# liuQuan98/GCL

Hardware: AMD Instinct MI355X
Metric: active voxels/sec thru ResUNetBN2C fwd+bwd+GCL loss, KITTI 0.3m (higher is better)
Workload: dtype f32; 1 GPU; configs[2]: GCL training step (finest_contrastive_loss), ResUNetBN2C-32 conv1 k=5, KITTI-shaped ray-cast clouds @0.3 m, bs=4 x 7 clouds per GPU, positive groups 'fixed16'; global_batch=4, parallelism=dp1

## Files before the change

### gcl_amd/MinkowskiEngine/native.py

```python
import ctypes
import os
import threading

import torch
from torch.autograd.function import once_differentiable

from .. import _lib

PLAN_ENABLED = os.environ.get("GCL_PLAN", "1") == "1"
AUX_STREAM = {"0": "", "1": "1", "low": "low", "high": "high"}[os.environ.get("GCL_PLAN_AUX", "low")]


def _addr(t):
    return t.data_ptr() if t is not None else 0


_SIDE_STREAMS = {}


def eval_side_stream(device, n_rows=None):
    if os.environ.get("GCL_EVAL_SPLIT_MAPS", "1") == "0":
        return None
    if n_rows is not None and n_rows < int(os.environ.get("GCL_EVAL_SPLIT_MIN_ROWS", "100000")):
        return None
# ... 253 lines not shown
        plan.covers_all_params = claimed == set(range(len(params)))
        return plan

    def _pointers(self):
        key = tuple(p.data_ptr() for p in self.params)
        if key != self._ptr_key:
            if any(p.dtype != torch.float32 or not p.is_contiguous() for p in self.params):
                raise ValueError("plan parameters must be contiguous fp32 tensors")
            self._ptr_key = key
            self._param_ptrs = (ctypes.c_void_p * len(key))(*key)
            bn = []
            for rm, rv in self.bn_buffers:
                bn += [rm.data_ptr(), rv.data_ptr()]
            self._bn_ptrs = (ctypes.c_void_p * max(1, len(bn)))(*bn)
        return self._param_ptrs, self._bn_ptrs

    def run(self, x_feats, maps):
        lib = _lib.require_gpu()
        if maps.keys != self.spec_keys:
            raise ValueError("the maps were built for a different map specification than the plan")
        self._check_input(x_feats, maps)
        x = x_feats.contiguous()
        dev = x.device
        need = lib.gcl_plan_arena_bytes(self.handle, ctypes.byref(maps.desc))
        if need < 0:
            raise RuntimeError("gcl_plan_arena_bytes: " + lib.gcl_last_error().decode())
        arena = torch.empty(int(need), dtype=torch.uint8, device=dev)
        self._ensure_state(lib, dev)
        pp, bp = self._pointers()
        if AUX_STREAM and self._aux is None:
            lo, _hi = torch.cuda.Stream.priority_range()
            pct = int(os.environ.get("GCL_AUX_CU_PCT", "0"))
            if 0 < pct < 100:
                h = ctypes.c_void_p()
                _lib.check(lib.gcl_stream_create_cu_share(pct, 1, ctypes.byref(h)), "gcl_stream_create_cu_share")
                self._aux = torch.cuda.ExternalStream(h.value, device=dev)
            else:
                self._aux = torch.cuda.Stream(device=dev, priority={"low": lo, "high": _hi}.get(AUX_STREAM, 0))
            lib.gcl_plan_set_aux_stream(self.handle, ctypes.c_void_p(self._aux.cuda_stream))
        if self.profile_next:
            lib.gcl_plan_profile(self.handle, 1)
        y_ptr = ctypes.c_void_p()
        held = None
        if self._touched is not None and not (torch.is_grad_enabled() and self.forward_list_ok()):
            held, cap = self._touched, self._touched_cap
            self.set_touched_rows(None, 0)
        try:
            _lib.check(lib.gcl_plan_forward(self.handle, ctypes.byref(maps.desc), _lib.ptr(x, torch.float32), pp, bp,
                                            _lib.ptr(self._state), _lib.ptr(arena), arena.numel(), ctypes.byref(y_ptr),
                                            _lib.stream()), "gcl_plan_forward")
        finally:
            if held is not None:
                self.set_touched_rows(held, cap)
        for m in self.bn_modules:
            m._pending_batches += 1
            m._train_forwards += 1
        n_out = int(maps.desc.n_rows[self.records[-1]["level_out"]])
        off = y_ptr.value - arena.data_ptr()
        y = arena[off:off + n_out * self.out_channels * 4].view(torch.float32).view(n_out, self.out_channels)
        if not torch.is_grad_enabled():
            lib.gcl_plan_release(self.handle, _lib.ptr(arena))
            return y
        run = _PlanRun()
        run.plan, run.arena, run.maps, run.y, run.x = self, arena, maps, y, x
        run.grad_targets, run.done = self.grad_targets, False
        run.touched = None
        if self._touched is not None and lib.gcl_plan_suffix_fwd_rows_used(self.handle) > 0:
            run.touched, self._touched, self._touched_cap = self._touched, None, 0
        run.segments = self._segments()
        if run.grad_targets is not None:
            if self._anchor is None or self._anchor.device != dev:
                self._anchor = torch.zeros(1, device=dev, requires_grad=True)
            return _PlanFn.apply(run, self._anchor)
        return _PlanFn.apply(run, *self.params)

    def _check_input(self, x_feats, maps):
        r0 = self.records[0]
        if x_feats.dim() != 2 or x_feats.shape[1] != r0["cin"]:
            raise ValueError(f"the plan was recorded for {r0['cin']} input channels, got a tensor of shape {tuple(x_feats.shape)}")
        if x_feats.shape[0] != int(maps.desc.n_rows[r0["level_in"]]):
            raise ValueError("features and coordinate maps differ in length")

    def _ensure_state(self, lib, dev):
        if self._state is None or self._state.device != dev:
            self._state = torch.empty(int(lib.gcl_plan_eval_state_bytes(self.handle)), dtype=torch.uint8, device=dev)
            self._eval_key = None

    def prepare_eval(self, dev):
        from . import ops
        lib = _lib.require_gpu()
        self._ensure_state(lib, dev)
        pp, _ = self._pointers()
        aff, ptrs = [], []
        for m in self.bn_modules:
            scale, shift = m.eval_affine()
            rstd = getattr(m, "_eval_rstd", None)
            if rstd is None or rstd[0] is not scale:
                with torch.no_grad():
                    rstd = m._eval_rstd = (scale, torch.rsqrt(m.bn.running_var.detach() + m.bn.eps).contiguous())
            aff.append((scale, shift, rstd[1]))
            ptrs += [scale.data_ptr(), shift.data_ptr(), m.bn.running_mean.data_ptr(), rstd[1].data_ptr()]
        bn = (ctypes.c_void_p * len(ptrs))(*ptrs)
        key = (tuple(p._version for p in self.params), tuple(p.data_ptr() for p in self.params), ops._AMAX_EPOCH)
        return pp, bn, aff, key, dev

    def run_eval(self, x_feats, maps, prepared=None):
        lib = _lib.require_gpu()
        if maps.keys != self.spec_keys:
            raise ValueError("the maps were built for a different map specification than the plan")
        self._check_input(x_feats, maps)
        x = x_feats.contiguous()
        dev = x.device
        if prepared is None or prepared[4] != dev:
            prepared = self.prepare_eval(dev)
        pp, bn, aff, key, _ = prepared
        need = lib.gcl_plan_eval_arena_bytes(self.handle, ctypes.byref(maps.desc))
        if need < 0:
            raise RuntimeError("gcl_plan_eval_arena_bytes: " + lib.gcl_last_error().decode())
        arena = torch.empty(int(need), dtype=torch.uint8, device=dev)
        repack = int(key != self._eval_key)
        y_ptr = ctypes.c_void_p()
        _lib.check(lib.gcl_plan_forward_eval(self.handle, ctypes.byref(maps.desc), _lib.ptr(x, torch.float32), pp, bn, repack,
                                             _lib.ptr(self._state), _lib.ptr(arena), arena.numel(), ctypes.byref(y_ptr),
                                             _lib.stream()), "gcl_plan_forward_eval")
        self._eval_key = key
        n_out = int(maps.desc.n_rows[self.records[-1]["level_out"]])
        off = y_ptr.value - arena.data_ptr()
        return arena[off:off + n_out * self.out_channels * 4].view(torch.float32).view(n_out, self.out_channels)

    def _segments(self):
        n = len(self.records)
        if self.bucket_of_param is None or self.on_bucket is None:
            return [(0, n, [])]
        lowest = {}
        for i, r in enumerate(self.records):
            for k in ("w", "bias", "bn_w", "bn_b"):
                p = r[k]
                if p >= 0 and p in self.bucket_of_param:
                    b = self.bucket_of_param[p]
                    lowest[b] = min(lowest.get(b, i), i)
        cuts = sorted(set(lowest.values()), reverse=True)
        segs, hi = [], n
        for c in cuts:
            segs.append((c, hi, sorted(b for b, i in lowest.items() if i == c)))
            hi = c
        if hi > 0:
            segs.append((0, hi, []))
        return segs

    def forward_list_ok(self):
        n, s = len(self.records), _lib.load().gcl_plan_touched_suffix(self.handle)
        return all(last <= s or (first <= s and last == n) for first, last, _ in self._segments())

    def output_rows(self, maps):
        return int(maps.desc.n_rows[self.records[-1]["level_out"]])

    def set_touched_rows(self, rows, cap):
        lib = _lib.load()
        self._touched = rows
        self._touched_cap = int(cap)
        _lib.check(lib.gcl_plan_set_touched_rows(self.handle, _lib.ptr(rows, torch.int32), int(cap)),
                   "gcl_plan_set_touched_rows")

    def touch_loss_rows(self, index, goff, sel, rows_a, rows_b, n_rows, cap):
        lib = _lib.load()
        dev = index.device
        scratch = torch.empty(int(lib.gcl_touched_rows_scratch_len(int(n_rows))), dtype=torch.int32, device=dev)
        out = torch.empty(int(cap) + 1, dtype=torch.int32, device=dev)
        rows, count = out[:cap], out[cap:]
        _lib.check(lib.gcl_touched_rows(_lib.ptr(index, torch.int64), index.shape[0], _lib.ptr(goff, torch.int64),
                                        goff.shape[0] - 1, _lib.ptr(sel, torch.int64), sel.shape[0],
                                        _lib.ptr(rows_a, torch.int64), rows_a.shape[0], _lib.ptr(rows_b, torch.int64),
                                        rows_b.shape[0], int(n_rows), _lib.ptr(scratch), _lib.ptr(rows), int(cap),
                                        _lib.ptr(count), _lib.stream()), "gcl_touched_rows")
        self.set_touched_rows(rows, cap)
        return rows, count

    def _backward(self, run, dy):
        lib = _lib.load()
        targets = run.grad_targets
        flat = None
        if targets is None:
            sizes = [p.numel() for p in self.params]
            flat = torch.empty(sum(sizes), dtype=torch.float32, device=dy.device)
            targets, off = [], 0
            for p, s in zip(self.params, sizes):
                targets.append(flat[off:off + s].view_as(p))
                off += s
        gp = (ctypes.c_void_p * len(targets))(*[t.data_ptr() for t in targets])
        st = _lib.stream()
        for first, last, buckets in run.segments:
            _lib.check(lib.gcl_plan_backward(self.handle, _lib.ptr(run.arena), _lib.ptr(dy, torch.float32), gp, first,
                                             last, st), "gcl_plan_backward")
            for b in buckets:
                self.on_bucket(b)
        self._touched = run.touched = None
        if self.profile_next:
            self.profile_next = False
            self._profile_pending = True
            lib.gcl_plan_profile(self.handle, 0)
        run.done = True
        run.arena = run.maps = run.y = run.x = None
        return None if flat is None else targets

    def profile_records(self):
        lib = _lib.load()
        buf = (ctypes.c_double * (8 * 1024))()
        n = lib.gcl_plan_profile_read(self.handle, buf, 1024)
        return [tuple(buf[8 * i + j] for j in range(8)) for i in range(max(0, n))]
```

### gcl_amd/_lib.py

```python
import ctypes
import os
import subprocess

import torch

_HERE = os.path.dirname(os.path.abspath(__file__))
CSRC = os.path.join(_HERE, "csrc")
LIB_PATH = os.environ.get("GCL_LIB_PATH", os.path.join(CSRC, "libgcl_hip.so"))
SOURCES = ["coords.hip", "conv.hip", "norm.hip", "loss.hip", "pairloss.hip", "data.hip", "sc2pcr.hip", "plan.hip", "match.hip", "ransac.hip", "regstats.hip", "fpfh.hip",
           "valpose.hip", "pairmatch.hip", "icp.hip", "instnorm.hip"]
HEADER = os.path.join(os.path.dirname(_HERE), "include", "gcl_amd.h")

_vp, _i32, _i64, _f32 = ctypes.c_void_p, ctypes.c_int32, ctypes.c_int64, ctypes.c_float
_f64 = ctypes.c_double

MAX_LEVELS, MAX_MAPS = 8, 16
MAPS_PINNED_BYTES = 512 * (MAX_MAPS + 1)
ERR_ARENA = -4


class MapSpec(ctypes.Structure):
    _fields_ = [("t_in", _i32), ("kernel_size", _i32), ("stride", _i32), ("tables", _i32), ("pairs", _i32)]


class MapDesc(ctypes.Structure):
    _fields_ = [("t_in", _i32), ("kernel_size", _i32), ("stride", _i32), ("K", _i32), ("level_in", _i32),
                ("level_out", _i32), ("n_in", _i64), ("n_out", _i64), ("n_pairs", _i64),
                ("nbr", _vp), ("nbr_t", _vp), ("counts", _vp),
                ("tbl_n", _vp), ("order_n", _vp), ("mask_n", _vp), ("tbl_t", _vp), ("order_t", _vp), ("mask_t", _vp),
                ("pair_in", _vp), ("pair_out", _vp), ("presence", _vp), ("dw_bounds", _vp), ("seg_off", _i64 * 128),
                ("counts_host", _i32 * 128)]


class MapsDesc(ctypes.Structure):
    _fields_ = [("n_levels", _i32), ("n_maps", _i32), ("n_rows", _i64 * MAX_LEVELS), ("coords", _vp * MAX_LEVELS),
                ("table", _vp * MAX_LEVELS), ("cap", _i64 * MAX_LEVELS), ("status", _i32 * 4), ("arena_used", _i64),
                ("ready_event", _vp), ("late_mask", _i32), ("reserved", _i32), ("maps", MapDesc * MAX_MAPS)]


class NnSearch(ctypes.Structure):
    _fields_ = [("a", _vp), ("rows_a", _vp), ("b", _vp), ("rows_b", _vp), ("dmin", _vp), ("argmin", _vp), ("pts_a", _vp),
                ("pts_b", _vp), ("src", _vp), ("tgt", _vp), ("bi_off", _i64), ("part_off", _i64), ("ma", _i32), ("mb", _i32)]


class MutualJob(ctypes.Structure):
    _fields_ = [("nn01", _vp), ("nn10", _vp), ("xyz0", _vp), ("xyz1", _vp), ("T", _vp), ("pairs", _vp), ("src", _vp),
                ("tgt", _vp), ("count", _vp), ("m0", _i32), ("m1", _i32)]


class PlanOp(ctypes.Structure):
    _fields_ = [("kind", _i32), ("x", _i32), ("x2", _i32), ("y", _i32), ("level_in", _i32), ("level_out", _i32),
                ("cin", _i32), ("cout", _i32), ("map", _i32), ("transpose", _i32), ("K", _i32), ("w", _i32),
                ("bias", _i32), ("bn_w", _i32), ("bn_b", _i32), ("bn", _i32), ("relu", _i32), ("momentum", _f32),
                ("eps", _f32)]


OP_CONVBN, OP_CONV, OP_RELU, OP_CAT, OP_ROWNORM = 1, 2, 3, 4, 5

SIGNATURES = {
    "gcl_last_error": (ctypes.c_char_p, []),
    "gcl_version": (_i32, []),
    "gcl_device_count": (_i32, []),
    "gcl_coords_insert": (_i32, [_vp, _i64, _vp, _i64, _vp, _vp]),
    "gcl_scan_scratch_len": (_i64, [_i64]),
    "gcl_stride_map": (_i32, [_vp, _i64, _vp, _i32, _vp, _i64, _vp, _vp, _vp, _vp, _vp]),
    "gcl_exclusive_scan_i32": (_i32, [_vp, _i64, _vp, _vp, _vp]),
    "gcl_voxel_coords": (_i32, [_vp, _i64, _f32, _i32, _vp, _vp]),
    "gcl_unique_coords": (_i32, [_vp, _i64, _vp, _i64, _vp, _vp, _vp, _vp, _vp, _vp]),
    "gcl_colocation_hits": (_i32, [_vp, _vp, _i64, _i32, ctypes.POINTER(ctypes.c_double), _vp, _i64, _f32,
                                    ctypes.c_double, _i32, _vp, _vp, _vp, _vp]),
    "gcl_colocation_emit": (_i32, [_vp, _vp, _vp, _i64, _i32, _i32, _vp, _vp, _vp, _vp, _vp, _vp]),
    "gcl_voxel_coords_multi": (_i32, [_vp, _i64, ctypes.POINTER(_i64), _i32, _f32, _vp, _vp]),
    "gcl_cloud_row_starts": (_i32, [_vp, _i64, _vp, _i32, _vp, _vp]),
    "gcl_loader_points": (_i32, [_vp, _vp, _vp, _i64, _vp, _vp, _vp, _vp, _vp]),
    "gcl_colocation_hits_at": (_i32, [_vp, _vp, _i64, _i64, _i32, _i32, ctypes.POINTER(ctypes.c_double), _vp, _i64, _f32,
                                       ctypes.c_double, _i32, _vp, _vp, _vp, _vp]),
    "gcl_cloud_centroids_scratch_len": (_i64, [_i64, _i32]),
    "gcl_cloud_centroids": (_i32, [_vp, _i64, ctypes.POINTER(_i64), _i32, _vp, _vp, _vp]),
    "gcl_cloud_affines": (_i32, [_vp, _vp, _i32, _vp, _vp]),
    "gcl_voxel_coords_aug": (_i32, [_vp, _i64, ctypes.POINTER(_i64), _i32, _f64, _vp, _vp, _i32, _vp, _vp]),
    "gcl_loader_points_aug": (_i32, [_vp, _vp, _vp, _i64, _vp, _vp, _vp, _vp, _i32, _vp, _vp, _vp]),
    "gcl_host_legacy_choice":(_i32, [_vp, _vp, _i64, _i64, _vp, _vp]),
    "gcl_kernel_map_bitmap_len": (_i64, []),
    "gcl_kernel_map_scratch_len": (_i64, [_i32, _i64]),
    "gcl_kernel_map": (_i32, [_vp, _i64, _vp, _i64, _i32, _i32, _i32, _vp, _vp, _vp, _vp, _i64, _vp, _vp]),
    "gcl_kernel_map_pairs": (_i32, [_vp, _i32, _i64, ctypes.POINTER(_i64), _vp, _vp, _vp, _vp]),
    "gcl_map_launch_shape": (_i32, [_i64, _i32, _i32, ctypes.POINTER(_i32)]),
    "gcl_pack_weights_bytes": (_i64, [_i32, _i32, _i32, _i32]),
    "gcl_amax": (_i32, [_vp, _i64, _vp, _i32, _vp]),
    "gcl_amax_multi": (_i32, [_vp, _vp, _i32, _vp, _vp]),
    "gcl_pack_weights_multi": (_i32, [_vp, _i32, _i64, _i32, _vp, _vp, _vp]),
    "gcl_conv_fwd_nb": (_i32, [_i64, _i32, _i32]),
    "gcl_pack_weights": (_i32, [_vp, _i32, _i32, _i32, _i32, _i32, _vp, _vp, _vp]),
    "gcl_table_sort_scratch_len": (_i64, [_i64]),
    "gcl_table_sort": (_i32, [_vp, _i32, _i64, _vp, _vp, _vp, _vp, _vp]),
    "gcl_table_sort_multi": (_i32, [_vp, _i32, _vp]),
    "gcl_conv_fwd_groups_scratch_len": (_i64, [_i64, _i32, _i32, _i32]),
    "gcl_conv_fwd_launch_shape": (_i32, [_i64, _i32, _i32, _i32, _i32, _i32, _i32, _i32, _i32, _i32, ctypes.POINTER(_i32)]),
    "gcl_conv_fwd_fused": (_i32, [_vp, _i64, _i32, _vp, _i32, _vp, _vp, _vp, _vp, _vp, _i64, _i32, _i32, _i32, _vp, _vp, _vp,
                                  _i32, _vp, _vp, _vp, _i32, _vp]),
    "gcl_conv_fwd_fused_ld": (_i32, [_vp, _i64, _i32, _vp, _i32, _vp, _vp, _vp, _vp, _vp, _i64, _i32, _i32, _i32, _vp, _vp, _vp,
                                     _i32, _i32, _vp, _vp, _vp, _i32, _vp]),
    "gcl_split_planes": (_i32, [_vp, _i64, _i32, _vp, _vp, _vp]),
    "gcl_conv_fwd": (_i32, [_vp, _i64, _i32, _vp, _i32, _vp, _vp, _vp, _vp, _vp, _i64, _i32, _i32, _i32, _vp, _vp, _vp, _i32,
                            _vp]),
    "gcl_conv_bwd_weight_scratch_len": (_i64, [_i32, _i32, _i32, _i64, _i64]),
    "gcl_conv_bwd_weight": (_i32, [_vp, _i64, _vp, _i64, _i32, _i32, _vp, _vp, ctypes.POINTER(_i64), _i32, _i32, _i32, _i32, _vp,
                                   _vp, _vp, _vp, _vp]),
    "gcl_conv_bwd_weight_bounds_len": (_i64, [_i32, _i64]),
    "gcl_conv_bwd_weight_bounds": (_i32, [_vp, ctypes.POINTER(_i64), _i32, _i64, _vp, _vp]),
    "gcl_conv_bwd_weight_rg": (_i32, [_vp, _i64, _vp, _i64, _i32, _i32, _vp, _vp, ctypes.POINTER(_i64), _i32, _i32, _i32, _i32, _vp,
                                      _vp, _vp, _vp, _vp, _vp]),
    "gcl_conv_bwd_weight_launch_shape": (_i32, [_i32, _i32, _i32, _i32, _i32, _i32, _i64, _i64, ctypes.POINTER(_i32)]),
    "gcl_conv_bwd_weight_rows_scratch_len": (_i64, [_i32, _i32, _i32, _i64]),
    "gcl_conv_bwd_weight_rows": (_i32, [_vp, _vp, _i64, _i32, _i32, _i32, _vp, _vp, _vp, _vp, _vp]),
    "gcl_presence_bits": (_i32, [_vp, _i32, _i64, _vp, _vp]),
    "gcl_kernel_map_3_from_5": (_i32, [_vp, _vp, _i64, _vp, _vp, _vp]),
    "gcl_not_ones_rows": (_i32, [_vp, _i32, _vp, _i64, _vp, _i32, _vp, _vp]),
    "gcl_stem_fwd": (_i32, [_vp, _vp, _vp, _i64, _i32, _i32, _i32, _vp, _vp, _vp, _vp]),
    "gcl_stem_bwd_weight_scratch_len": (_i64, [_i32, _i32, _i32, _i64]),
    "gcl_stem_bwd_weight": (_i32, [_vp, _vp, _vp, _i64, _i32, _i32, _i32, _vp, _vp, _vp, _vp, _vp]),
    "gcl_bn_scratch_len": (_i64, [_i64, _i32]),
    "gcl_bn_stats": (_i32, [_vp, _i64, _i32, _f32, _f32, _vp, _vp, _vp, _vp, _vp, _vp]),
    "gcl_bn_tiles_scratch_len": (_i64, [_i64, _i32]),
    "gcl_bn_stats_from_tiles_range": (_i32, [_vp, _i64, _i64, _i32, _f32, _f32, _vp, _vp, _vp, _vp, _vp, _vp, _vp, _i32, _vp, _vp, _vp,
                                             _vp]),
    "gcl_bn_apply_planes": (_i32, [_vp, _i64, _i32, _vp, _vp, _vp, _vp, _vp, _i32, _vp, _i32, _vp, _vp, _vp, _vp]),
    "gcl_bn_bwd_reduce_range": (_i32, [_vp, _vp, _i32, _vp, _vp, _i64, _i32, _vp, _vp, _i32, _vp, _vp, _vp, _vp, _vp, _vp, _vp]),
    "gcl_bn_bwd_apply_planes": (_i32, [_vp, _vp, _i32, _vp, _vp, _i64, _i32, _vp, _vp, _vp, _vp, _vp, _i32, _vp, _vp, _vp, _vp, _vp]),
    "gcl_bn_bwd_reduce_rows": (_i32, [_vp, _vp, _i32, _vp, _vp, _i64, _i32, _vp, _vp, _i32, _vp, _vp, _vp, _vp, _vp, _vp, _vp]),
    "gcl_bn_bwd_apply_rows": (_i32, [_vp, _vp, _i32, _vp, _vp, _i64, _i32, _vp, _vp, _vp, _vp, _vp, _i32, _vp, _vp, _vp, _vp, _vp]),
    "gcl_bn_stats_from_tiles": (_i32, [_vp, _i64, _i64, _i32, _f32, _f32, _vp, _vp, _vp, _vp, _vp, _vp]),
    "gcl_bn_apply": (_i32, [_vp, _i64, _i32, _vp, _vp, _vp, _vp, _vp, _i32, _vp, _vp, _vp, _vp]),
    "gcl_bn_apply_ld": (_i32, [_vp, _i64, _i32, _vp, _vp, _vp, _vp, _vp, _i32, _vp, _i32, _vp, _vp, _vp]),
    "gcl_bn_mask_len": (_i64, [_i64, _i32]),
    "gcl_bn_bwd_reduce": (_i32, [_vp, _vp, _vp, _vp, _i64, _i32, _vp, _vp, _i32, _vp, _vp, _vp, _vp]),
    "gcl_bn_bwd_apply": (_i32, [_vp, _vp, _vp, _vp, _i64, _i32, _vp, _vp, _vp, _vp, _vp, _i32, _vp, _vp, _vp, _vp]),
    "gcl_bn_bwd_reduce_ld": (_i32, [_vp, _vp, _i32, _vp, _vp, _i64, _i32, _vp, _vp, _i32, _vp, _vp, _vp, _vp]),
    "gcl_bn_bwd_apply_ld": (_i32, [_vp, _vp, _i32, _vp, _vp, _i64, _i32, _vp, _vp, _vp, _vp, _vp, _i32, _vp, _vp, _vp, _vp]),
    "gcl_in_scratch_len": (_i64, [_i64, _i32, _i32]),
    "gcl_in_fwd": (_i32, [_vp, _i64, _i32, _vp, _vp, _vp, _i32, _f32, _vp, _vp, _vp, _i32, _vp, _vp, _vp, _vp, _vp, _vp, _vp]),
    "gcl_in_bwd": (_i32, [_vp, _vp, _i64, _i32, _vp, _vp, _vp, _i32, _vp, _vp, _vp, _i32, _vp, _vp, _vp, _vp, _vp, _vp, _vp,
                          _vp]),
    "gcl_row_normalize_fwd": (_i32, [_vp, _i64, _i32, _vp, _vp, _vp]),
    "gcl_row_normalize_bwd": (_i32, [_vp, _vp, _vp, _i64, _i32, _vp, _vp, _vp]),
    "gcl_sgd_multi": (_i32, [_vp, _vp, _i32, _f32, _f32, _f32, _i32, _vp]),
    "gcl_col_sum": (_i32, [_vp, _i64, _i32, _vp, _vp, _vp]),
    "gcl_maps_arena_bytes": (_i64, [_i64, _vp, _i32, _i32]),
    "gcl_maps_build": (_i32, [_vp, _i64, _vp, _i32, _i32, _vp, _i64, _vp, _vp, _vp]),
    "gcl_maps_build_split": (_i32, [_vp, _i64, _vp, _i32, _i32, _vp, _i64, _vp, _vp, _vp, _vp]),
    "gcl_plan_create": (_vp, [_vp, _i32, _i32, _i32, _vp, _i32, _i32]),
    "gcl_plan_destroy": (None, [_vp]),
    "gcl_plan_state_bytes": (_i64, [_vp]),
    "gcl_plan_arena_bytes": (_i64, [_vp, _vp]),
    "gcl_plan_forward": (_i32, [_vp, _vp, _vp, _vp, _vp, _vp, _vp, _i64, _vp, _vp]),
    "gcl_plan_eval_state_bytes": (_i64, [_vp]),
    "gcl_plan_eval_arena_bytes": (_i64, [_vp, _vp]),
    "gcl_plan_forward_eval": (_i32, [_vp, _vp, _vp, _vp, _vp, _i32, _vp, _vp, _i64, _vp, _vp]),
    "gcl_plan_backward": (_i32, [_vp, _vp, _vp, _vp, _i32, _i32, _vp]),
    "gcl_plan_release": (_i32, [_vp, _vp]),
    "gcl_plan_set_aux_stream": (_i32, [_vp, _vp]),
    "gcl_plan_touched_suffix": (_i32, [_vp]),
    "gcl_plan_set_touched_rows": (_i32, [_vp, _vp, _i64]),
    "gcl_plan_suffix_rows_used": (_i64, [_vp]),
    "gcl_plan_suffix_fwd_rows_used": (_i64, [_vp]),
    "gcl_gather_rows": (_i32, [_vp, _i32, _i64, _vp, _i64, _i32, _f32, _vp, _vp]),
    "gcl_scatter_rows": (_i32, [_vp, _vp, _i64, _i32, _i64, _vp, _i32, _vp]),
    "gcl_scatter_add_rows": (_i32, [_vp, _i32, _vp, _i64, _i32, _i64, _vp, _i32, _vp]),
    "gcl_row_slots": (_i32, [_vp, _i64, _i64, _vp, _vp]),
    "gcl_touched_rows_scratch_len": (_i64, [_i64]),
    "gcl_touched_rows": (_i32, [_vp, _i64, _vp, _i64, _vp, _i32, _vp, _i32, _vp, _i32, _i64, _vp, _vp, _i64, _vp, _vp]),
    "gcl_stream_create_cu_share": (_i32, [_i32, _i32, ctypes.POINTER(ctypes.c_void_p)]),
    "gcl_stream_destroy": (_i32, [_vp]),
    "gcl_plan_profile": (_i32, [_vp, _i32]),
    "gcl_plan_profile_read": (_i32, [_vp, _vp, _i32]),
    "gcl_sc2_chunks": (_i32, []),
    "gcl_sc2_refine_partial_len": (_i32, []),
    "gcl_sc2_confidence": (_i32, [_vp, _vp, _i32, _f32, _i32, _vp, _vp, _vp, _vp]),
    "gcl_sc2_confidence_scratch_bytes": (_i64, [_i32]),
    "gcl_sc2_confidence_sparse": (_i32, [_vp, _vp, _i32, _f32, _i32, _vp, _vp, _vp, _vp, _vp]),
    "gcl_sc2_register_scratch_bytes": (_i64, [_i32]),
    "gcl_sc2_register": (_i32, [_vp, _vp, _i32, _f32, _i32, _f32, _i32, _i32, _i32, _f32, _f32, _i32, _vp, _vp, _vp, _vp, _vp,
                                _vp, _vp, _vp, _vp, _vp]),
    "gcl_sc2_register_batch_scratch_bytes": (_i64, [_i32, _i32]),
    "gcl_sc2_register_batch": (_i32, [_vp, _vp, _i32, _i32, _vp, _vp, _f32, _i32, _f32, _i32, _i32, _f32, _f32, _i32, _vp, _vp,
                                      _vp, _vp, _vp, _vp, _vp, _vp, _vp, _vp]),
    "gcl_sc2_local_max": (_i32, [_vp, _vp, _i32, _f32, _vp, _vp]),
    "gcl_sc2_seed_knn": (_i32, [_vp, _vp, _i32, _vp, _i32, _f32, _i32, _vp, _vp, _vp]),
    "gcl_sc2_seed_trans": (_i32, [_vp, _vp, _i32, _vp, _i32, _i32, _i32, _f32, _i32, _f32, _vp, _vp, _vp]),
    "gcl_sc2_refine": (_i32, [_vp, _vp, _i32, _f32, _i32, _vp, _vp, _vp, _vp]),
    "gcl_ransac_scratch_bytes": (_i64, [_i32, _i32]),
    "gcl_ransac_default_chunk": (_i32, []),
    "gcl_ransac_register": (_i32, [_vp, _vp, _i32, _i32, _f32, _f32, _f32, _i32, _f32, ctypes.c_uint64, _i32, _vp, _vp, _vp, _vp,
                                   _vp, _vp, _vp]),
    "gcl_ransac_batch_scratch_bytes": (_i64, [_i32, _i32, _i32]),
    "gcl_ransac_register_batch": (_i32, [_vp, _vp, _i32, _i32, _vp, _i32, _f32, _f32, _f32, _i32, _f32, _vp, _i32, _vp, _vp,
                                         _vp, _vp, _vp, _vp, _vp]),
    "gcl_registration_stats": (_i32, [_vp, _vp, _i32, _i32, _vp, _vp, _vp, _f32, _f32, _f32, _vp, _vp, _vp, _vp]),
    "gcl_group_loss_fwd": (_i32, [_vp, _i32, _vp, _vp, _vp, _vp, _i32, _f32, _f32, _i32, _vp, _vp, _vp, _vp]),
    "gcl_group_loss_bwd": (_i32, [_vp, _i32, _vp, _vp, _vp, _vp, _i32, _f32, _f32, _i32, _vp, _vp, _vp, _vp, _vp]),
    "gcl_circle_group_fwd": (_i32, [_vp, _i32, _vp, _vp, _vp, _vp, _i32, _f32, _f32, _f32, _i32, _vp, _vp, _vp, _vp, _vp]),
    "gcl_circle_group_bwd": (_i32, [_vp, _i32, _vp, _vp, _vp, _vp, _i32, _f32, _f32, _f32, _i32, _vp, _vp, _vp, _vp, _vp,
                                    _vp]),
    "gcl_nn_rowmin_scratch_len": (_i64, [_i32, _i32]),
    "gcl_nn_rowmin": (_i32, [_vp, _vp, _i32, _vp, _vp, _i32, _i32, _i32, _vp, _vp, _vp, _vp]),
    "gcl_nn_rowmin_any_scratch_len": (_i64, [_i32, _i32, _i32]),
    "gcl_nn_rowmin_any": (_i32, [_vp, _vp, _i32, _vp, _vp, _i32, _i32, _i32, _vp, _vp, _vp, _vp]),
    "gcl_nn3_scratch_len": (_i64, [_i32, _i32]),
    "gcl_nn3_rowmin": (_i32, [_vp, _i32, _vp, _i32, _vp, _i32, _vp, _vp, _vp, _vp, _vp]),
    "gcl_nn_rowmin_batch_scratch_len": (_i64, [_vp, _i32, _i32]),
    "gcl_nn_rowmin_batch": (_i32, [_vp, _vp, _i32, _i32, _i32, _vp, _vp]),
    "gcl_mutual_match_batch": (_i32, [_vp, _vp, _i32, _f32, _vp]),
    "gcl_mutual_correspondences_batch": (_i32, [_vp, _vp, _i32, _i32, _vp]),
    "gcl_mutual_match": (_i32, [_vp, _i32, _vp, _i32, _vp, _vp, _vp, _f32, _vp, _vp, _vp]),
    "gcl_mutual_correspondences": (_i32, [_vp, _i32, _vp, _i32, _vp, _vp, _i32, _vp, _vp, _vp, _vp]),
    "gcl_neg_mask": (_i32, [_vp, _vp, _vp, _i32, _vp, _vp, _i64, _i64, _vp, _i64, _vp, _vp]),
    "gcl_neg_loss_fwd": (_i32, [_vp, _vp, _i32, _f32, _vp, _vp]),
    "gcl_neg_loss_bwd": (_i32, [_vp, _i32, _vp, _vp, _vp, _vp, _vp, _i32, _f32, _vp, _vp, _vp, _vp]),
    "gcl_loss_combine": (_i32, [_vp, _vp, _i32, _vp, _f32, _f32, _f32, _vp, _vp]),
    "gcl_loss_seed": (_i32, [_vp, _f32, _f32, _f32, _i32, _vp, _vp, _vp, _vp]),
    "gcl_pair_key_table": (_i32, [_vp, _i64, _i64, _vp, _i64, _vp]),
    "gcl_pair_key_mask": (_i32, [_vp, _i32, _vp, _vp, _i64, _i32, _i64, _vp, _i64, _vp, _vp, _vp]),
    "gcl_triplet_scratch_len": (_i64, [_i32]),
    "gcl_triplet_fwd": (_i32, [_vp, _i64, _vp, _i64, _i32, _vp, _vp, _vp, _vp, _i32, _f32, _vp, _vp, _vp]),
    "gcl_triplet_bwd": (_i32, [_vp, _i64, _vp, _i64, _i32, _vp, _vp, _vp, _vp, _i32, _vp, _vp, _vp, _vp, _vp, _vp]),
    "gcl_pair_terms_scratch_len": (_i64, [_i32]),
    "gcl_pair_terms_fwd": (_i32, [_vp, _i64, _vp, _i64, _i32, _vp, _vp, _i32, _i32, _f32, _f32, _vp, _vp, _vp]),
    "gcl_pair_terms_bwd": (_i32, [_vp, _i64, _vp, _i64, _i32, _vp, _vp, _i32, _i32, _f32, _f32, _vp, _vp, _vp, _vp, _vp,
                                  _vp]),
    "gcl_fpfh_cell_keys": (_i32, [_vp, _i64, _vp, _i32, _f32, _vp, _vp]),
    "gcl_fpfh_neighbours": (_i32, [_vp, _i64, _vp, _i32, _vp, _vp, _f32, _i32, _vp, _vp, _vp]),
    "gcl_fpfh_normals": (_i32, [_vp, _i64, _vp, _vp, _i32, _vp, _vp, _i32, _vp, _vp]),
    "gcl_fpfh_spfh": (_i32, [_vp, _vp, _i64, _vp, _vp, _i32, _vp, _vp]),
    "gcl_fpfh_combine": (_i32, [_vp, _vp, _i64, _vp, _vp, _i32, _i32, _vp, _vp]),
    "gcl_irls_pose_scratch_len": (_i64, [_i64]),
    "gcl_irls_pose_batch": (_i32, [_vp, _vp, _i64, _vp, _i32, _vp, _i32, _f64, _i32, _vp, _vp, _vp, _vp]),
    "gcl_val_stats_batch": (_i32, [_vp, _vp, _i64, _vp, _vp, _i64, _vp, _i32, _vp, _vp, _vp, _f64, _f64, _vp, _vp]),
    "gcl_pair_matches_scratch_len": (_i64, [_i64]),
    "gcl_pair_matches_count": (_i32, [_vp, _i64, _vp, _vp, _i64, _vp, _vp, _i32, _vp, _i64, _i32, _i32, _f32, _vp, _vp, _f64, _i32,
                                       _vp, _vp, _vp, _vp]),
    "gcl_pair_matches_emit": (_i32, [_vp, _i64, _vp, _vp, _i64, _vp, _vp, _i32, _vp, _i64, _i32, _i32, _f32, _vp, _vp, _f64, _i32,
                                      _i32, _vp, _vp, _vp, _i64, _vp]),
    "gcl_icp_scratch_bytes": (_i64, [_i64, _i64, _i32]),
    "gcl_icp_register_batch": (_i32, [_vp, ctypes.POINTER(_i64), _vp, _vp, ctypes.POINTER(_i64), _vp, _i32, _vp, _vp, _f64, _vp,
                                      _i32, _f64, _f64, _vp, _vp, _vp, _vp, _vp, _vp]),
}

PAIR_CHUNK = 128
TRIPLET_OUT = 20
PAIR_SQ, PAIR_SQ_POS, PAIR_NEG, PAIR_DIST = 0, 1, 2, 3
FPFH_MAX_NN, FPFH_MAX_CLOUDS, FPFH_BINS = 128, 32767, 33

_lib = None


TRAINING_STEP_SOURCES = ("coords.hip", "conv.hip", "norm.hip", "plan.hip")


def source_hash():
    import hashlib
    h = hashlib.sha256()
    for path in [os.path.join(CSRC, s) for s in TRAINING_STEP_SOURCES] + [os.path.join(CSRC, "common.h")]:
        with open(path, "rb") as fh:
            h.update(fh.read())
    return h.hexdigest()[:16]


def build(force=False, verbose=False):
    srcs = [os.path.join(CSRC, s) for s in SOURCES]
    hdrs = [os.path.join(CSRC, "common.h"), os.path.join(CSRC, "kabsch.h"), os.path.join(CSRC, "fpgrid.h"), HEADER]
    deps = srcs + hdrs
    if not force and os.path.exists(LIB_PATH) and all(os.path.getmtime(LIB_PATH) >= os.path.getmtime(d) for d in deps):
        return LIB_PATH
    hdr_time = max(os.path.getmtime(h) for h in hdrs)
    objs, jobs = [], []
    for s in srcs:
        o = s[:-4] + ".o"
        objs.append(o)
        if force or not os.path.exists(o) or os.path.getmtime(o) < max(os.path.getmtime(s), hdr_time):
            cmd = ["hipcc", "--offload-arch=gfx950", "-O3", "-std=c++17", "-fPIC", "-c", s, "-o", o]
            if verbose:
                print(" ".join(cmd))
            jobs.append((cmd, subprocess.Popen(cmd)))
    for cmd, p in jobs:
        if p.wait() != 0:
            raise subprocess.CalledProcessError(p.returncode, cmd)
    cmd = ["hipcc", "--offload-arch=gfx950", "-fPIC", "-shared", "-o", LIB_PATH] + objs
    if verbose:
        print(" ".join(cmd))
    subprocess.run(cmd, check=True)
    return LIB_PATH


def load():
    global _lib
    if _lib is not None:
        return _lib
    if not os.path.exists(LIB_PATH):
        raise RuntimeError(
            f"{LIB_PATH} is missing: run `python -c 'import __graft_entry__ as g; g.build()'` "
            "(gcl_amd has no CPU fallback; the HIP library is the only product path)")
    lib = ctypes.CDLL(LIB_PATH)
    for name, (res, args) in SIGNATURES.items():
        fn = getattr(lib, name)
        fn.restype = res
        fn.argtypes = args
    _lib = lib
    return lib


_gpu_ok = False


def require_gpu():
# ... 39 lines not shown
```

### gcl_amd/csrc/norm.hip

```cpp
#include "common.h"

namespace gcl {

static inline int bn_rows_per_wg(long long n, int c) {
  int rows = 1024;
  while (rows > 64 && n / rows < 1024) rows >>= 1;
  (void)c;
  return rows;
}

__device__ __forceinline__ float4 mask_as_y(const unsigned long long* __restrict__ mask, long long e) {
  const unsigned long long* m = mask + (e >> 6) * 4;
  const int b = (int)(e & 63);
  return make_float4((float)((m[0] >> b) & 1), (float)((m[1] >> b) & 1), (float)((m[2] >> b) & 1),
                     (float)((m[3] >> b) & 1));
}

__device__ __forceinline__ void relu_gate(float4& g, const float4& yv) {
  g.x = yv.x > 0.f ? g.x : 0.f; g.y = yv.y > 0.f ? g.y : 0.f;
  g.z = yv.z > 0.f ? g.z : 0.f; g.w = yv.w > 0.f ? g.w : 0.f;
}

__device__ __forceinline__ void bn_reduce_partials(double (&red)[2][256][4], const double (&s0)[4], const double (&s1)[4],
                                                   const float (&gm)[4], int c, bool gmax, double* partial) {
// ... 243 lines not shown
};
__global__ void __launch_bounds__(256) k_bn_stats_direct(const float* __restrict__ partial, int n_part, long long n, int c,
                                                         float eps, float momentum, float* running_mean,
                                                         float* running_var, float* mean, float* rstd, BnRange rg) {
  const int ch = blockIdx.x;
  double s, ss;
  reduce_runs(partial + (long long)ch * n_part, partial + ((long long)c + ch) * n_part, n_part, s, ss);
  float xlo = 0.f, xhi = 0.f;
  if (rg.y_amax)
    reduce_min_max(partial + ((long long)2 * c + ch) * n_part, partial + ((long long)3 * c + ch) * n_part, n_part, xlo, xhi);
  if (threadIdx.x != 0) return;
  double m = s / (double)n;
  double var = ss / (double)n - m * m;
  if (var < 0) var = 0;
  const float mu = (float)m, rs = (float)(1.0 / sqrt(var + (double)eps));
  mean[ch] = mu;
  rstd[ch] = rs;
  if (running_mean) {
    double unb = (n > 1) ? var * (double)n / (double)(n - 1) : var;
    running_mean[ch] = (float)((1.0 - momentum) * running_mean[ch] + momentum * m);
    running_var[ch] = (float)((1.0 - momentum) * running_var[ch] + momentum * unb);
  }
  if (rg.y_amax) {
    if (rg.xrange) {
      rg.xrange[ch] = xlo;
      rg.xrange[c + ch] = xhi;
    }
    const float w = rg.weight[ch], b = rg.bias[ch];
    const float f_lo = (xlo - mu) * rs * w + b, f_hi = (xhi - mu) * rs * w + b;
    float bound = rg.relu ? fmaxf(fmaxf(f_lo, f_hi), 0.f) : fmaxf(fabsf(f_lo), fabsf(f_hi));
    if (rg.add_amax) bound += __int_as_float(amax_slot_bits(rg.add_amax));
    if (rg.max_with) bound = fmaxf(bound, __int_as_float(amax_slot_bits(rg.max_with)));
    amax_slot_publish(rg.y_amax, __float_as_int(bound), (unsigned)ch);
  }
}

struct BnBwdRange {
  const float* xrange;
  const float* mean;
  const float* rstd;
  const float* weight;
  long long n;
  int* dx_amax;
};
__global__ void __launch_bounds__(256) k_bn_bwd_final(const double* __restrict__ partial, int nwg, int c,
                                                      float* sum_g, float* sum_gx, BnBwdRange rg) {
  const int ch = blockIdx.x;
  double s, ss;
  reduce_runs(partial + (long long)ch * nwg, partial + ((long long)c + ch) * nwg, nwg, s, ss);
  double gmax = 0;
  if (rg.dx_amax) {
    __shared__ double gm[256];
    double a = 0;
    const double* p3 = partial + ((long long)2 * c + ch) * nwg;
    for (int w = threadIdx.x; w < nwg; w += 256) a = fmax(a, p3[w]);
    gm[threadIdx.x] = a;
    __syncthreads();
    for (int o = 128; o > 0; o >>= 1) {
      if ((int)threadIdx.x < o) gm[threadIdx.x] = fmax(gm[threadIdx.x], gm[threadIdx.x + o]);
      __syncthreads();
    }
    gmax = gm[0];
  }
  if (threadIdx.x != 0) return;
  sum_g[ch] = (float)s;
  sum_gx[ch] = (float)ss;
  if (rg.dx_amax) {
    const float mu = rg.mean[ch], rs = rg.rstd[ch], inv_n = 1.0f / (float)rg.n;
    const float xh = fmaxf(fabsf(rg.xrange[ch] - mu), fabsf(rg.xrange[c + ch] - mu)) * rs;
    const float bound = fabsf(rg.weight[ch] * rs) * ((float)gmax + fabsf((float)s) * inv_n + xh * fabsf((float)ss) * inv_n);
    amax_slot_publish(rg.dx_amax, __float_as_int(bound * 1.0000153f), (unsigned)ch);
  }
}

__device__ __forceinline__ void publish_amax(float m, int* amax_bits) {
#pragma unroll
  for (int o = 32; o > 0; o >>= 1) m = fmaxf(m, __shfl_xor(m, o));
  __shared__ float wm[4];
  if ((threadIdx.x & 63) == 0) wm[threadIdx.x >> 6] = m;
  __syncthreads();
  if (threadIdx.x == 0) {
    amax_slot_publish(amax_bits, __float_as_int(fmaxf(fmaxf(wm[0], wm[1]), fmaxf(wm[2], wm[3]))), blockIdx.x);
  }
}
__device__ __forceinline__ float amax4(float m, const float4& v) {
  return fmaxf(m, fmaxf(fmaxf(fabsf(v.x), fabsf(v.y)), fmaxf(fabsf(v.z), fabsf(v.w))));
}

struct BnFwdC { float4 mu, rs, wv, bv; };
__device__ __forceinline__ BnFwdC bn_fwd_c(const float* mean, const float* rstd, const float* weight, const float* bias, int cq) {
  BnFwdC k;
  k.mu = reinterpret_cast<const float4*>(mean)[cq]; k.rs = reinterpret_cast<const float4*>(rstd)[cq];
  k.wv = reinterpret_cast<const float4*>(weight)[cq]; k.bv = reinterpret_cast<const float4*>(bias)[cq];
  return k;
}
__device__ __forceinline__ float4 bn_fwd_one(const float4& xv, const float4& rv, bool has_res, int relu, const BnFwdC& k) {
  float4 o;
  o.x = (xv.x - k.mu.x) * k.rs.x * k.wv.x + k.bv.x;
  o.y = (xv.y - k.mu.y) * k.rs.y * k.wv.y + k.bv.y;
  o.z = (xv.z - k.mu.z) * k.rs.z * k.wv.z + k.bv.z;
  o.w = (xv.w - k.mu.w) * k.rs.w * k.wv.w + k.bv.w;
  if (has_res) { o.x += rv.x; o.y += rv.y; o.z += rv.z; o.w += rv.w; }
  if (relu) { o.x = fmaxf(o.x, 0.f); o.y = fmaxf(o.y, 0.f); o.z = fmaxf(o.z, 0.f); o.w = fmaxf(o.w, 0.f); }
  return o;
}
__device__ __forceinline__ void bn_mask_store(unsigned long long* __restrict__ mask, long long e, const float4& o, bool ok) {
  unsigned long long b0 = __ballot(ok && o.x > 0.f), b1 = __ballot(ok && o.y > 0.f), b2 = __ballot(ok && o.z > 0.f),
                     b3 = __ballot(ok && o.w > 0.f);
  if (ok && (threadIdx.x & 63) == 0) {
    unsigned long long* m = mask + (e >> 6) * 4;
    m[0] = b0; m[1] = b1; m[2] = b2; m[3] = b3;
  }
}

template <bool HOIST>
__global__ void __launch_bounds__(256) k_bn_apply(const float* __restrict__ x, long long total4, int c,
                                                  const float* __restrict__ mean, const float* __restrict__ rstd,
                                                  const float* __restrict__ weight, const float* __restrict__ bias,
                                                  const float* __restrict__ residual, int relu,
                                                  float* __restrict__ y, unsigned long long* __restrict__ mask,
                                                  int* amax_bits, int y_ld = 0, unsigned short* __restrict__ planes = nullptr,
                                                  const int* __restrict__ planes_amax = nullptr) {
  const float pscale = planes ? amax_scale(planes_amax) : 1.f;
  const int cq_n = c >> 2;
  const long long S = (long long)gridDim.x * blockDim.x;
  const long long e0 = (long long)blockIdx.x * blockDim.x + threadIdx.x;
  const long long yld4 = (y_ld ? y_ld : c) >> 2;
  const long long rstep = HOIST ? S / cq_n : 0;
  long long row_e = e0 / cq_n;
  const int q0 = (int)(e0 % cq_n);
#define BN_Y(E, ROW) (y_ld ? (HOIST ? reinterpret_cast<float4*>(y)[(ROW)*yld4 + q0]                        \
                                    : reinterpret_cast<float4*>(y)[((E) / cq_n) * yld4 + ((E) % cq_n)])   \
                           : reinterpret_cast<float4*>(y)[E])
  const float4 z4 = make_float4(0, 0, 0, 0);
  float am = 0.f;
  BnFwdC ka, kb;
  if (HOIST) ka = kb = bn_fwd_c(mean, rstd, weight, bias, (int)(e0 % cq_n));
  for (long long e = e0; e - (threadIdx.x & 63) < total4; e += 2 * S) {
    const long long f = e + S;
    const bool oka = e < total4, okb = f < total4;
    if (!HOIST) {
      ka = bn_fwd_c(mean, rstd, weight, bias, (int)((oka ? e : 0) % cq_n));
      kb = bn_fwd_c(mean, rstd, weight, bias, (int)((okb ? f : 0) % cq_n));
    }
    float4 xa = z4, xb = z4, ra = z4, rb = z4;
    if (oka) xa = reinterpret_cast<const float4*>(x)[e];
    if (okb) xb = reinterpret_cast<const float4*>(x)[f];
    if (residual) {
      if (oka) ra = reinterpret_cast<const float4*>(residual)[e];
      if (okb) rb = reinterpret_cast<const float4*>(residual)[f];
    }
    const float4 oa = bn_fwd_one(xa, ra, residual != nullptr, relu, ka);
    const float4 ob = bn_fwd_one(xb, rb, residual != nullptr, relu, kb);
    if (oka) { BN_Y(e, row_e) = oa; am = amax4(am, oa); }
    if (okb) { BN_Y(f, row_e + rstep) = ob; am = amax4(am, ob); }
    if (planes) {
      const long long pld = yld4 * 4;
      if (oka) store_planes4(planes, HOIST ? row_e : e / cq_n, pld, HOIST ? q0 * 4 : (int)(e % cq_n) * 4, oa, pscale);
      if (okb) store_planes4(planes, HOIST ? row_e + rstep : f / cq_n, pld, HOIST ? q0 * 4 : (int)(f % cq_n) * 4, ob, pscale);
    }
    row_e += 2 * rstep;
    if (mask) {
      bn_mask_store(mask, e, oa, oka);
      if (f - (threadIdx.x & 63) < total4) bn_mask_store(mask, f, ob, okb);
    }
  }
#undef BN_Y
  if (amax_bits && !planes) publish_amax(am, amax_bits);
}

struct BnBwdC { float4 mu, rs, wv, sg, sx; };
__device__ __forceinline__ BnBwdC bn_bwd_c(const float* mean, const float* rstd, const float* weight, const float* sum_g,
                                           const float* sum_gx, int cq) {
  BnBwdC k;
  k.mu = reinterpret_cast<const float4*>(mean)[cq]; k.rs = reinterpret_cast<const float4*>(rstd)[cq];
  k.wv = reinterpret_cast<const float4*>(weight)[cq];
  k.sg = reinterpret_cast<const float4*>(sum_g)[cq]; k.sx = reinterpret_cast<const float4*>(sum_gx)[cq];
  return k;
}
__device__ __forceinline__ float4 bn_bwd_one(const float4& xv, const float4& g, float inv_n, const BnBwdC& k) {
  float4 o;
  o.x = k.wv.x * k.rs.x * (g.x - k.sg.x * inv_n - (xv.x - k.mu.x) * k.rs.x * k.sx.x * inv_n);
  o.y = k.wv.y * k.rs.y * (g.y - k.sg.y * inv_n - (xv.y - k.mu.y) * k.rs.y * k.sx.y * inv_n);
  o.z = k.wv.z * k.rs.z * (g.z - k.sg.z * inv_n - (xv.z - k.mu.z) * k.rs.z * k.sx.z * inv_n);
  o.w = k.wv.w * k.rs.w * (g.w - k.sg.w * inv_n - (xv.w - k.mu.w) * k.rs.w * k.sx.w * inv_n);
  return o;
}

template <bool HOIST, bool ROWS>
__global__ void __launch_bounds__(256) k_bn_bwd_apply(const float* __restrict__ x, const float* __restrict__ dy,
                                                      const float* __restrict__ y, long long total4, int c,
                                                      float inv_n, const float* __restrict__ mean,
                                                      const float* __restrict__ rstd,
                                                      const float* __restrict__ weight,
                                                      const float* __restrict__ sum_g,
                                                      const float* __restrict__ sum_gx, int relu,
                                                      const unsigned long long* __restrict__ mask,
                                                      float* __restrict__ dx, float* __restrict__ dres,
                                                      int* amax_bits, int dy_ld = 0,
                                                      unsigned short* __restrict__ planes = nullptr,
                                                      const int* __restrict__ planes_amax = nullptr,
                                                      const int* __restrict__ slots = nullptr) {
  const float pscale = planes ? amax_scale(planes_amax) : 1.f;
  const int cq_n = c >> 2;
  const long long S = (long long)gridDim.x * blockDim.x;
  const long long e0 = (long long)blockIdx.x * blockDim.x + threadIdx.x;
  const long long gld4 = (dy_ld ? dy_ld : c) >> 2;
  const long long rstep = HOIST ? S / cq_n : 0;
  long long row_e = e0 / cq_n;
  const int q0 = (int)(e0 % cq_n);
#define BN_DY(E, ROW) (dy_ld ? (HOIST ? reinterpret_cast<const float4*>(dy)[(ROW)*gld4 + q0]                       \
                                      : reinterpret_cast<const float4*>(dy)[((E) / cq_n) * gld4 + ((E) % cq_n)])  \
                             : reinterpret_cast<const float4*>(dy)[E])
#define BN_SLOT(E, ROW) slots[HOIST ? (ROW) : (E) / cq_n]
#define BN_DY_ROWS(G, E, SLOT) \
  if ((SLOT) >= 0) G = reinterpret_cast<const float4*>(dy)[(SLOT)*gld4 + (HOIST ? q0 : (int)((E) % cq_n))];
#define BN_DRES(E, SLOT, G)                                                                                       \
  if (dres) {                                                                                                     \
    if (!ROWS) reinterpret_cast<float4*>(dres)[E] = G;                                                            \
    else if ((SLOT) >= 0) reinterpret_cast<float4*>(dres)[(SLOT)*cq_n + (HOIST ? q0 : (int)((E) % cq_n))] = G;    \
  }
  const float4 z4 = make_float4(0, 0, 0, 0);
  float am = 0.f;
  BnBwdC ka, kb;
  if (HOIST) ka = kb = bn_bwd_c(mean, rstd, weight, sum_g, sum_gx, (int)(e0 % cq_n));
  for (long long e = e0; e < total4; e += 2 * S) {
    const long long f = e + S;
    const bool okb = f < total4;
    if (!HOIST) {
      ka = bn_bwd_c(mean, rstd, weight, sum_g, sum_gx, (int)(e % cq_n));
      kb = bn_bwd_c(mean, rstd, weight, sum_g, sum_gx, (int)((okb ? f : 0) % cq_n));
    }
    long long sa = -1, sb = -1;
    if (ROWS) {
      sa = BN_SLOT(e, row_e);
      if (okb) sb = BN_SLOT(f, row_e + rstep);
    }
    float4 xa = reinterpret_cast<const float4*>(x)[e], ga = z4;
    if (ROWS) { BN_DY_ROWS(ga, e, sa) } else ga = BN_DY(e, row_e);
    float4 xb = z4, gb = z4, ya = z4, yb = z4;
    if (okb) {
      xb = reinterpret_cast<const float4*>(x)[f];
      if (ROWS) { BN_DY_ROWS(gb, f, sb) } else gb = BN_DY(f, row_e + rstep);
    }
    row_e += 2 * rstep;
    if (relu) {
      ya = mask ? mask_as_y(mask, e) : reinterpret_cast<const float4*>(y)[e];
      if (okb) yb = mask ? mask_as_y(mask, f) : reinterpret_cast<const float4*>(y)[f];
      relu_gate(ga, ya);
      relu_gate(gb, yb);
    }
    const float4 oa = bn_bwd_one(xa, ga, inv_n, ka);
    reinterpret_cast<float4*>(dx)[e] = oa;
    am = amax4(am, oa);
    if (planes) store_planes4(planes, e / cq_n, c, (int)(e % cq_n) * 4, oa, pscale);
    BN_DRES(e, sa, ga)
    if (okb) {
      const float4 ob = bn_bwd_one(xb, gb, inv_n, kb);
      reinterpret_cast<float4*>(dx)[f] = ob;
      am = amax4(am, ob);
      if (planes) store_planes4(planes, f / cq_n, c, (int)(f % cq_n) * 4, ob, pscale);
      BN_DRES(f, sb, gb)
    }
  }
#undef BN_DY
#undef BN_SLOT
#undef BN_DY_ROWS
#undef BN_DRES
  if (amax_bits && !planes) publish_amax(am, amax_bits);
}

template <bool BWD>
__global__ void __launch_bounds__(256) k_row_normalize(const float* __restrict__ a, const float* __restrict__ dy,
                                                       const float* __restrict__ norm_in, long long n, int c,
                                                       float* __restrict__ out, float* __restrict__ norm_out,
                                                       int* out_amax) {
  const int lpr = c >> 2;
  const long long e = (long long)blockIdx.x * blockDim.x + threadIdx.x;
  const long long row = e / lpr;
  const bool ok = row < n;
  float4 v = make_float4(0, 0, 0, 0), g = make_float4(0, 0, 0, 0);
  if (ok) {
    v = reinterpret_cast<const float4*>(a)[e];
    if (BWD) g = reinterpret_cast<const float4*>(dy)[e];
  }
  float s = BWD ? (v.x * g.x + v.y * g.y + v.z * g.z + v.w * g.w) : (v.x * v.x + v.y * v.y + v.z * v.z + v.w * v.w);
  for (int o = 1; o < lpr; o <<= 1) s += __shfl_xor(s, o);
  float m = 0.f;
  if (ok) {
    float4 o4;
    if (!BWD) {
      const float nr = sqrtf(s);
      o4 = make_float4(v.x / nr, v.y / nr, v.z / nr, v.w / nr);
      if ((e % lpr) == 0) norm_out[row] = nr;
    } else {
      const float nr = norm_in[row];
      o4 = make_float4((g.x - v.x * s) / nr, (g.y - v.y * s) / nr, (g.z - v.z * s) / nr, (g.w - v.w * s) / nr);
    }
    reinterpret_cast<float4*>(out)[e] = o4;
    m = amax4(m, o4);
  }
  if (out_amax) publish_amax(m, out_amax);
}

struct SgdPtrs { float* p; const float* g; float* buf; };
__global__ void __launch_bounds__(256) k_sgd_multi(const SgdPtrs* __restrict__ table, const long long* __restrict__ sizes,
                                                   float lr, float momentum, float wd, int first) {
  const SgdPtrs t = table[blockIdx.y];
  const long long n = sizes[blockIdx.y];
  const bool vec = ((((unsigned long long)t.p) | ((unsigned long long)t.g) | ((unsigned long long)t.buf)) & 15ull) == 0;
  const long long n4 = vec ? n / 4 : 0;
  for (long long e = (long long)blockIdx.x * blockDim.x + threadIdx.x; e < n4; e += (long long)gridDim.x * blockDim.x) {
    float4 p = reinterpret_cast<const float4*>(t.p)[e];
    const float4 g = reinterpret_cast<const float4*>(t.g)[e];
    float4 b = make_float4(0, 0, 0, 0);
    if (!first) b = reinterpret_cast<const float4*>(t.buf)[e];
    const float d0 = g.x + wd * p.x, d1 = g.y + wd * p.y, d2 = g.z + wd * p.z, d3 = g.w + wd * p.w;
    b.x = first ? d0 : momentum * b.x + d0;
    b.y = first ? d1 : momentum * b.y + d1;
    b.z = first ? d2 : momentum * b.z + d2;
    b.w = first ? d3 : momentum * b.w + d3;
    reinterpret_cast<float4*>(t.buf)[e] = b;
    p.x -= lr * b.x;
    p.y -= lr * b.y;
    p.z -= lr * b.z;
    p.w -= lr * b.w;
    reinterpret_cast<float4*>(t.p)[e] = p;
  }
  for (long long e = n4 * 4 + (long long)blockIdx.x * blockDim.x + threadIdx.x; e < n; e += (long long)gridDim.x * blockDim.x) {
    const float p = t.p[e];
    const float d = t.g[e] + wd * p;
    const float b = first ? d : momentum * t.buf[e] + d;
    t.buf[e] = b;
    t.p[e] = p - lr * b;
  }
}

static bool bn_c_ok(int c) { return c >= 4 && c % 4 == 0 && (256 % (c / 4)) == 0; }

__global__ void __launch_bounds__(256) k_col_sum_final(const double* __restrict__ partial, int nwg, int c, float* out) {
  const int ch = blockIdx.x;
  double s, ss;
  reduce_runs(partial + (long long)ch * nwg, partial + ((long long)c + ch) * nwg, nwg, s, ss);
  if (threadIdx.x != 0) return;
  out[ch] = (float)s;
}

}

using namespace gcl;

extern "C" {

int64_t gcl_bn_scratch_len(int64_t n, int32_t c) { return cdiv(n, bn_rows_per_wg(n, c)) * 3 * c; }

int gcl_bn_stats(const float* x, int64_t n, int32_t c, float eps, float momentum, float* running_mean,
                 float* running_var, double* scratch, float* mean, float* rstd, void* stream) {
  GCL_CHECK_ARG(x && scratch && mean && rstd, "gcl_bn_stats: null pointer");
  GCL_CHECK_ARG(n > 0 && bn_c_ok(c), "gcl_bn_stats: unsupported shape n=%lld c=%d (c/4 must divide 256)", (long long)n, c);
  hipStream_t st = (hipStream_t)stream;
  const int rows = bn_rows_per_wg(n, c);
  int nwg = (int)cdiv(n, rows);
  hipLaunchKernelGGL(k_bn_reduce<false>, dim3(nwg), dim3(256), 0, st, x, (const float*)nullptr,
                     (const float*)nullptr, (long long)n, c, (const float*)nullptr, (const float*)nullptr, 0,
                     (const unsigned long long*)nullptr, rows, scratch);
  hipLaunchKernelGGL(k_bn_stats_final, dim3((unsigned)c), dim3(256), 0, st, (const double*)scratch, nwg,
                     (long long)n, c, eps, momentum, running_mean, running_var, mean, rstd);
  GCL_CHECK_LAUNCH();
  return GCL_OK;
}

int64_t gcl_bn_tiles_scratch_len(int64_t n_tiles, int32_t c) { (void)n_tiles; return 2 * (int64_t)c; }

int gcl_bn_stats_from_tiles(const float* partial, int64_t n_tiles, int64_t n, int32_t c, float eps, float momentum,
                            float* running_mean, float* running_var, double* scratch, float* mean, float* rstd,
                            void* stream) {
  (void)scratch;
  return gcl_bn_stats_from_tiles_range(partial, n_tiles, n, c, eps, momentum, running_mean, running_var, mean, rstd, nullptr,
                                       nullptr, nullptr, 0, nullptr, nullptr, nullptr, stream);
}

int gcl_bn_stats_from_tiles_range(const float* partial, int64_t n_tiles, int64_t n, int32_t c, float eps, float momentum,
                                  float* running_mean, float* running_var, float* mean, float* rstd, float* xrange,
                                  const float* weight, const float* bias, int32_t relu, const int32_t* add_amax,
                                  const int32_t* max_with, int32_t* y_amax, void* stream) {
  GCL_CHECK_ARG(partial && mean && rstd, "gcl_bn_stats_from_tiles: null pointer");
  GCL_CHECK_ARG(n > 0 && n_tiles > 0 && n_tiles <= BN_DIRECT_MAX && c > 0, "gcl_bn_stats_from_tiles: bad sizes");
  GCL_CHECK_ARG(!y_amax || (weight && bias), "gcl_bn_stats_from_tiles_range: the bound of max|y| needs the BatchNorm's weight and bias");
  const BnRange rg{xrange, weight, bias, relu, (const int*)add_amax, (const int*)max_with, (int*)y_amax};
  hipLaunchKernelGGL(k_bn_stats_direct, dim3((unsigned)c), dim3(256), 0, (hipStream_t)stream, partial, (int)n_tiles,
                     (long long)n, c, eps, momentum, running_mean, running_var, mean, rstd, rg);
  GCL_CHECK_LAUNCH();
  return GCL_OK;
}

int gcl_bn_apply(const float* x, int64_t n, int32_t c, const float* mean, const float* rstd, const float* weight,
                 const float* bias, const float* residual, int32_t relu, float* y, uint64_t* relu_mask,
                 int32_t* y_amax, void* stream) {
  return gcl_bn_apply_ld(x, n, c, mean, rstd, weight, bias, residual, relu, y, 0, relu_mask, y_amax, stream);
}

int gcl_bn_apply_ld(const float* x, int64_t n, int32_t c, const float* mean, const float* rstd, const float* weight,
                    const float* bias, const float* residual, int32_t relu, float* y, int32_t y_ld, uint64_t* relu_mask,
                    int32_t* y_amax, void* stream) {
  return gcl_bn_apply_planes(x, n, c, mean, rstd, weight, bias, residual, relu, y, y_ld, relu_mask, y_amax, nullptr, stream);
}

int gcl_bn_apply_planes(const float* x, int64_t n, int32_t c, const float* mean, const float* rstd, const float* weight,
                        const float* bias, const float* residual, int32_t relu, float* y, int32_t y_ld, uint64_t* relu_mask,
                        int32_t* y_amax, void* planes, void* stream) {
  GCL_CHECK_ARG(x && mean && rstd && weight && bias && y, "gcl_bn_apply: null pointer");
  GCL_CHECK_ARG(n > 0 && c >= 4 && c % 4 == 0, "gcl_bn_apply: unsupported shape");
  GCL_CHECK_ARG(y_ld == 0 || (y_ld >= c && y_ld % 4 == 0), "gcl_bn_apply_ld: y_ld must be 0 or a multiple of 4 >= c");
  GCL_CHECK_ARG(!planes || (y_amax && c % 32 == 0 && (y_ld % 32) == 0),
                "gcl_bn_apply_planes: a plane image needs the slot that holds the bound of max|y| and widths that are multiples of 32");
  long long total4 = n * (c / 4);
  long long g = cdiv(total4, 256);
  if (g > 4096) g = 4096;
  if ((g * 256) % (c / 4) == 0)
    hipLaunchKernelGGL(k_bn_apply<true>, dim3((unsigned)g), dim3(256), 0, (hipStream_t)stream, x, total4, c, mean, rstd,
                       weight, bias, residual, relu, y, (unsigned long long*)(relu ? relu_mask : nullptr), y_amax, y_ld,
                       (unsigned short*)planes, (const int*)y_amax);
  else
    hipLaunchKernelGGL(k_bn_apply<false>, dim3((unsigned)g), dim3(256), 0, (hipStream_t)stream, x, total4, c, mean, rstd,
                       weight, bias, residual, relu, y, (unsigned long long*)(relu ? relu_mask : nullptr), y_amax, y_ld,
                       (unsigned short*)planes, (const int*)y_amax);
  GCL_CHECK_LAUNCH();
  return GCL_OK;
}

int64_t gcl_bn_mask_len(int64_t n, int32_t c) { return cdiv(n * (c / 4), 64) * 4; }

int gcl_bn_bwd_reduce(const float* x, const float* dy, const float* y, const uint64_t* relu_mask, int64_t n,
                      int32_t c, const float* mean, const float* rstd, int32_t relu, double* scratch, float* sum_g,
                      float* sum_gx, void* stream) {
  return gcl_bn_bwd_reduce_ld(x, dy, 0, y, relu_mask, n, c, mean, rstd, relu, scratch, sum_g, sum_gx, stream);
}

int gcl_bn_bwd_reduce_ld(const float* x, const float* dy, int32_t dy_ld, const float* y, const uint64_t* relu_mask, int64_t n,
                         int32_t c, const float* mean, const float* rstd, int32_t relu, double* scratch, float* sum_g,
                         float* sum_gx, void* stream) {
  return gcl_bn_bwd_reduce_range(x, dy, dy_ld, y, relu_mask, n, c, mean, rstd, relu, scratch, sum_g, sum_gx, nullptr, nullptr,
                                 nullptr, stream);
}

int gcl_bn_bwd_reduce_range(const float* x, const float* dy, int32_t dy_ld, const float* y, const uint64_t* relu_mask,
                            int64_t n, int32_t c, const float* mean, const float* rstd, int32_t relu, double* scratch,
                            float* sum_g, float* sum_gx, const float* xrange, const float* weight, int32_t* dx_amax,
                            void* stream) {
  GCL_CHECK_ARG(dy_ld == 0 || (dy_ld >= c && dy_ld % 4 == 0), "gcl_bn_bwd_reduce: dy_ld must be 0 or a multiple of 4 >= c");
  GCL_CHECK_ARG(x && dy && mean && rstd && scratch && sum_g && sum_gx, "gcl_bn_bwd_reduce: null pointer");
  GCL_CHECK_ARG(!relu || y || relu_mask, "gcl_bn_bwd_reduce: y or relu_mask is required when relu is set");
  GCL_CHECK_ARG(n > 0 && bn_c_ok(c), "gcl_bn_bwd_reduce: unsupported shape n=%lld c=%d", (long long)n, c);
  GCL_CHECK_ARG(!dx_amax || (xrange && weight), "gcl_bn_bwd_reduce_range: the bound of max|dx| needs xrange (forward pass) and the weight");
  hipStream_t st = (hipStream_t)stream;
  const int rows = bn_rows_per_wg(n, c);
  int nwg = (int)cdiv(n, rows);
  hipLaunchKernelGGL(k_bn_reduce<true>, dim3(nwg), dim3(256), 0, st, x, dy, y, (long long)n, c, mean, rstd, relu,
                     (const unsigned long long*)relu_mask, rows, scratch, dy_ld, dx_amax ? 1 : 0);
  const BnBwdRange rg{xrange, mean, rstd, weight, (long long)n, (int*)dx_amax};
  hipLaunchKernelGGL(k_bn_bwd_final, dim3((unsigned)c), dim3(256), 0, st, (const double*)scratch, nwg, c,
                     sum_g, sum_gx, rg);
  GCL_CHECK_LAUNCH();
  return GCL_OK;
}

int gcl_bn_bwd_apply(const float* x, const float* dy, const float* y, const uint64_t* relu_mask, int64_t n, int32_t c,
                     const float* mean, const float* rstd, const float* weight, const float* sum_g,
                     const float* sum_gx, int32_t relu, float* dx, float* dres, int32_t* dx_amax, void* stream) {
  return gcl_bn_bwd_apply_ld(x, dy, 0, y, relu_mask, n, c, mean, rstd, weight, sum_g, sum_gx, relu, dx, dres, dx_amax, stream);
}

int gcl_bn_bwd_apply_ld(const float* x, const float* dy, int32_t dy_ld, const float* y, const uint64_t* relu_mask, int64_t n,
                        int32_t c, const float* mean, const float* rstd, const float* weight, const float* sum_g,
                        const float* sum_gx, int32_t relu, float* dx, float* dres, int32_t* dx_amax, void* stream) {
  return gcl_bn_bwd_apply_planes(x, dy, dy_ld, y, relu_mask, n, c, mean, rstd, weight, sum_g, sum_gx, relu, dx, dres, dx_amax,
                                 nullptr, stream);
}

int gcl_bn_bwd_apply_planes(const float* x, const float* dy, int32_t dy_ld, const float* y, const uint64_t* relu_mask, int64_t n,
                            int32_t c, const float* mean, const float* rstd, const float* weight, const float* sum_g,
                            const float* sum_gx, int32_t relu, float* dx, float* dres, int32_t* dx_amax, void* planes,
                            void* stream) {
  GCL_CHECK_ARG(dy_ld == 0 || (dy_ld >= c && dy_ld % 4 == 0), "gcl_bn_bwd_apply: dy_ld must be 0 or a multiple of 4 >= c");
  GCL_CHECK_ARG(x && dy && mean && rstd && weight && sum_g && sum_gx && dx, "gcl_bn_bwd_apply: null pointer");
  GCL_CHECK_ARG(!relu || y || relu_mask, "gcl_bn_bwd_apply: y or relu_mask is required when relu is set");
  GCL_CHECK_ARG(n > 0 && c >= 4 && c % 4 == 0, "gcl_bn_bwd_apply: unsupported shape");
  GCL_CHECK_ARG(!planes || (dx_amax && c % 32 == 0),
                "gcl_bn_bwd_apply_planes: a plane image needs the slot that holds the bound of max|dx| and c a multiple of 32");
  long long total4 = n * (c / 4);
  long long g = cdiv(total4, 256);
  if (g > 4096) g = 4096;
  if ((g * 256) % (c / 4) == 0)
    hipLaunchKernelGGL((k_bn_bwd_apply<true, false>), dim3((unsigned)g), dim3(256), 0, (hipStream_t)stream, x, dy, y, total4, c,
                       1.0f / (float)n, mean, rstd, weight, sum_g, sum_gx, relu, (const unsigned long long*)relu_mask, dx,
                       dres, dx_amax, dy_ld, (unsigned short*)planes, (const int*)dx_amax);
  else
    hipLaunchKernelGGL((k_bn_bwd_apply<false, false>), dim3((unsigned)g), dim3(256), 0, (hipStream_t)stream, x, dy, y, total4, c,
                       1.0f / (float)n, mean, rstd, weight, sum_g, sum_gx, relu, (const unsigned long long*)relu_mask, dx,
                       dres, dx_amax, dy_ld, (unsigned short*)planes, (const int*)dx_amax);
  GCL_CHECK_LAUNCH();
  return GCL_OK;
}

int gcl_bn_bwd_reduce_rows(const float* x, const float* g, int32_t g_ld, const int32_t* slots, const uint64_t* relu_mask,
                           int64_t n, int32_t c, const float* mean, const float* rstd, int32_t relu, double* scratch,
                           float* sum_g, float* sum_gx, const float* xrange, const float* weight, int32_t* dx_amax,
                           void* stream) {
  GCL_CHECK_ARG(g_ld == 0 || (g_ld >= c && g_ld % 4 == 0), "gcl_bn_bwd_reduce_rows: g_ld must be 0 or a multiple of 4 >= c");
  GCL_CHECK_ARG(x && g && slots && mean && rstd && scratch && sum_g && sum_gx, "gcl_bn_bwd_reduce_rows: null pointer");
  GCL_CHECK_ARG(!relu || relu_mask, "gcl_bn_bwd_reduce_rows: relu_mask is required when relu is set");
  GCL_CHECK_ARG(n > 0 && bn_c_ok(c), "gcl_bn_bwd_reduce_rows: unsupported shape n=%lld c=%d", (long long)n, c);
  GCL_CHECK_ARG(!dx_amax || (xrange && weight), "gcl_bn_bwd_reduce_rows: the bound of max|dx| needs xrange (forward pass) and the weight");
  hipStream_t st = (hipStream_t)stream;
  const int per_wg = bn_rows_per_wg(n, c);
  const int nwg = (int)cdiv(n, per_wg);
  hipLaunchKernelGGL(k_bn_reduce_rows, dim3(nwg), dim3(256), 0, st, x, g, (const int*)slots, (long long)n, c, mean, rstd,
                     (const unsigned long long*)(relu ? relu_mask : nullptr), per_wg, scratch, g_ld, dx_amax ? 1 : 0);
  const BnBwdRange rg{xrange, mean, rstd, weight, (long long)n, (int*)dx_amax};
  hipLaunchKernelGGL(k_bn_bwd_final, dim3((unsigned)c), dim3(256), 0, st, (const double*)scratch, nwg, c, sum_g, sum_gx, rg);
  GCL_CHECK_LAUNCH();
  return GCL_OK;
}

int gcl_bn_bwd_apply_rows(const float* x, const float* g, int32_t g_ld, const int32_t* slots, const uint64_t* relu_mask,
                          int64_t n, int32_t c, const float* mean, const float* rstd, const float* weight, const float* sum_g,
                          const float* sum_gx, int32_t relu, float* dx, float* dres, int32_t* dx_amax, void* planes,
                          void* stream) {
  GCL_CHECK_ARG(g_ld == 0 || (g_ld >= c && g_ld % 4 == 0), "gcl_bn_bwd_apply_rows: g_ld must be 0 or a multiple of 4 >= c");
  GCL_CHECK_ARG(x && g && slots && mean && rstd && weight && sum_g && sum_gx && dx, "gcl_bn_bwd_apply_rows: null pointer");
  GCL_CHECK_ARG(!relu || relu_mask, "gcl_bn_bwd_apply_rows: relu_mask is required when relu is set");
  GCL_CHECK_ARG(n > 0 && c >= 4 && c % 4 == 0, "gcl_bn_bwd_apply_rows: unsupported shape");
  GCL_CHECK_ARG(!planes || (dx_amax && c % 32 == 0),
                "gcl_bn_bwd_apply_rows: a plane image needs the slot that holds the bound of max|dx| and c a multiple of 32");
  long long total4 = n * (c / 4);
  long long grid = cdiv(total4, 256);
  if (grid > 4096) grid = 4096;
  if ((grid * 256) % (c / 4) == 0)
    hipLaunchKernelGGL((k_bn_bwd_apply<true, true>), dim3((unsigned)grid), dim3(256), 0, (hipStream_t)stream, x, g,
                       (const float*)nullptr, total4, c, 1.0f / (float)n, mean, rstd, weight, sum_g, sum_gx, relu,
                       (const unsigned long long*)relu_mask, dx, dres, dx_amax, g_ld, (unsigned short*)planes,
                       (const int*)dx_amax, (const int*)slots);
  else
    hipLaunchKernelGGL((k_bn_bwd_apply<false, true>), dim3((unsigned)grid), dim3(256), 0, (hipStream_t)stream, x, g,
                       (const float*)nullptr, total4, c, 1.0f / (float)n, mean, rstd, weight, sum_g, sum_gx, relu,
                       (const unsigned long long*)relu_mask, dx, dres, dx_amax, g_ld, (unsigned short*)planes,
                       (const int*)dx_amax, (const int*)slots);
  GCL_CHECK_LAUNCH();
  return GCL_OK;
}

static bool rownorm_c_ok(int c) { return c >= 4 && c <= 256 && (c & (c - 1)) == 0; }

int gcl_row_normalize_fwd(const float* x, int64_t n, int32_t c, float* y, float* norm, void* stream) {
  GCL_CHECK_ARG(x && y && norm, "gcl_row_normalize_fwd: null pointer");
  GCL_CHECK_ARG(n > 0 && rownorm_c_ok(c), "gcl_row_normalize_fwd: c must be a power of two in [4, 256] (got %d)", c);
  long long total = n * (c / 4);
  hipLaunchKernelGGL(k_row_normalize<false>, dim3((unsigned)cdiv(total, 256)), dim3(256), 0, (hipStream_t)stream, x,
                     (const float*)nullptr, (const float*)nullptr, (long long)n, c, y, norm, (int*)nullptr);
  GCL_CHECK_LAUNCH();
  return GCL_OK;
}

int gcl_row_normalize_bwd(const float* y, const float* dy, const float* norm, int64_t n, int32_t c, float* dx,
                          int32_t* dx_amax, void* stream) {
  GCL_CHECK_ARG(y && dy && norm && dx, "gcl_row_normalize_bwd: null pointer");
  GCL_CHECK_ARG(n > 0 && rownorm_c_ok(c), "gcl_row_normalize_bwd: c must be a power of two in [4, 256] (got %d)", c);
  long long total = n * (c / 4);
  hipLaunchKernelGGL(k_row_normalize<true>, dim3((unsigned)cdiv(total, 256)), dim3(256), 0, (hipStream_t)stream, y, dy,
                     norm, (long long)n, c, dx, (float*)nullptr, dx_amax);
  GCL_CHECK_LAUNCH();
  return GCL_OK;
}

int gcl_col_sum(const float* x, int64_t n, int32_t c, double* scratch, float* out, void* stream) {
  GCL_CHECK_ARG(x && scratch && out, "gcl_col_sum: null pointer");
  GCL_CHECK_ARG(n > 0 && bn_c_ok(c), "gcl_col_sum: unsupported shape n=%lld c=%d (c/4 must divide 256)", (long long)n, c);
  hipStream_t st = (hipStream_t)stream;
  const int rows = bn_rows_per_wg(n, c);
  int nwg = (int)cdiv(n, rows);
  hipLaunchKernelGGL(k_bn_reduce<false>, dim3(nwg), dim3(256), 0, st, x, (const float*)nullptr,
                     (const float*)nullptr, (long long)n, c, (const float*)nullptr, (const float*)nullptr, 0,
                     (const unsigned long long*)nullptr, rows, scratch);
  hipLaunchKernelGGL(k_col_sum_final, dim3((unsigned)c), dim3(256), 0, st, (const double*)scratch, nwg, c, out);
  GCL_CHECK_LAUNCH();
  return GCL_OK;
}

int gcl_sgd_multi(const void* table, const int64_t* sizes, int32_t n_tensors, float lr, float momentum,
                  float weight_decay, int32_t first, void* stream) {
  GCL_CHECK_ARG(table && sizes && n_tensors > 0 && n_tensors <= 65535, "gcl_sgd_multi: bad argument");
  hipLaunchKernelGGL(k_sgd_multi, dim3(128, (unsigned)n_tensors), dim3(256), 0, (hipStream_t)stream,
                     (const SgdPtrs*)table, (const long long*)sizes, lr, momentum, weight_decay, first);
  GCL_CHECK_LAUNCH();
  return GCL_OK;
}

}
```

### gcl_amd/csrc/plan.hip

```cpp
#include "common.h"

#include <string.h>

#include <new>
#include <utility>
#include <vector>

namespace gcl {

__device__ __forceinline__ float amax4p(float m, const float4& v) {
  return fmaxf(m, fmaxf(fmaxf(fabsf(v.x), fabsf(v.y)), fmaxf(fabsf(v.z), fabsf(v.w))));
}
__device__ __forceinline__ void publish_amax_wg(float m, int* slot) {
#pragma unroll
  for (int o = 32; o > 0; o >>= 1) m = fmaxf(m, __shfl_xor(m, o));
  __shared__ float wm[4];
  if ((threadIdx.x & 63) == 0) wm[threadIdx.x >> 6] = m;
  __syncthreads();
  if (threadIdx.x == 0)
    amax_slot_publish(slot, __float_as_int(fmaxf(fmaxf(wm[0], wm[1]), fmaxf(wm[2], wm[3]))), blockIdx.x);
}

__global__ void __launch_bounds__(256) k_relu_fwd(const float4* __restrict__ x, long long n4, float4* __restrict__ y,
                                                  int* amax) {
// ... 283 lines not shown
  for (int s = 0; s < n_specs; ++s) any_pairs = any_pairs || (specs[s].pairs != 0 && specs[s].kernel_size > 1);
  const bool split = (side != nullptr || A.dry) && !any_pairs;
  auto on_side = [&](const gcl_map_spec& sp) { return split && !(sp.t_in == 1 && sp.stride == 1); };
  struct MapLaunch { int s, src5, flags; int32_t *bitmap, *scratch; void* stream; };
  MapLaunch launches[GCL_MAX_MAPS];
  int n_launches = 0;
  const MapShape mshape = map_launch_shape(n, 1, 0);
  const bool prefill = !A.dry && !side && mshape.prefill;
  char* fill_lo = nullptr;
  for (int s = 0; s < n_specs; ++s) {
    const gcl_map_spec& sp = specs[s];
    gcl_map_desc& d = out->maps[s];
    d.t_in = sp.t_in;
    d.kernel_size = sp.kernel_size;
    d.stride = sp.stride;
    d.K = sp.kernel_size * sp.kernel_size * sp.kernel_size;
    d.level_in = level_of(sp.t_in);
    d.level_out = level_of(sp.t_in * sp.stride);
    GCL_CHECK_ARG(d.level_in >= 0 && d.level_out >= 0 && d.level_out < n_levels && (sp.stride == 1 || sp.stride == 2),
                  "gcl_maps_build: map %d (t_in %d, stride %d) is outside the %d levels built", s, sp.t_in, sp.stride, n_levels);
    GCL_CHECK_ARG(sp.kernel_size == 1 || sp.kernel_size == 3 || sp.kernel_size == 5, "gcl_maps_build: kernel size 1, 3 or 5");
    d.n_in = out->n_rows[d.level_in];
    d.n_out = out->n_rows[d.level_out];
    if (sp.kernel_size == 1) {
      GCL_CHECK_ARG(sp.stride == 1, "gcl_maps_build: kernel_size 1 with stride > 1");
      continue;
    }
    const int sd = on_side(sp) ? 1 : 0;
    void* mstream = (sd && side) ? (void*)side : stream;
    if (sd) out->late_mask |= 1 << s;
    d.nbr = A.take_n<int32_t>((long long)d.K * d.n_out);
    if (!fill_lo) fill_lo = (char*)d.nbr;
    const bool same = sp.stride == 1;
    d.nbr_t = same ? nullptr : A.take_n<int32_t>((long long)d.K * d.n_in);
    d.counts = counts_all + 128 * s;
    int src5 = -1;
    for (int q = 0; q < s && same && sp.kernel_size == 3; ++q)
      if (specs[q].t_in == sp.t_in && specs[q].kernel_size == 5 && specs[q].stride == 1 && out->maps[q].nbr) src5 = q;
    if (src5 >= 0) {
      launches[n_launches++] = MapLaunch{s, src5, 0, nullptr, nullptr, mstream};
      continue;
    }
    const bool use_bitmap = A.dry || mshape.use_bitmap;
    const bool bitmap_valid = use_bitmap && bitmap[sd][d.level_in] != nullptr;
    if (use_bitmap && !bitmap_valid) bitmap[sd][d.level_in] = A.take_n<int32_t>(gcl_kernel_map_bitmap_len());
    int32_t* scratch = A.take_n<int32_t>(gcl_kernel_map_scratch_len(sp.kernel_size, d.n_out));
    launches[n_launches++] = MapLaunch{s, -1, (same ? 1 : 0) | (bitmap_valid ? 2 : 0) | 4 | (prefill ? 8 : 0),
                                       use_bitmap ? bitmap[sd][d.level_in] : nullptr, scratch, mstream};
  }
  if (prefill && fill_lo) fill32(fill_lo, (long long)((A.base + A.off) - fill_lo) / 4, 0xFFFFFFFFu, st);
  for (int q = 0; q < n_launches; ++q) {
    const MapLaunch& L = launches[q];
    const gcl_map_spec& sp = specs[L.s];
    gcl_map_desc& d = out->maps[L.s];
    if (L.src5 >= 0)
      PLAN_CALL(gcl_kernel_map_3_from_5(out->maps[L.src5].nbr, out->maps[L.src5].counts, d.n_out, d.nbr, d.counts, L.stream));
    else
      PLAN_CALL(gcl_kernel_map(out->coords[d.level_out], d.n_out, out->table[d.level_in], out->cap[d.level_in],
                               sp.kernel_size, sp.t_in, L.flags, L.bitmap, L.scratch, d.nbr, d.nbr_t, d.n_in, d.counts, L.stream));
    if (!A.dry && any_pairs)
      GCL_CHECK_HIP(hipMemcpyAsync(pinned + 128 * (L.s + 1), d.counts, sizeof(int32_t) * d.K, hipMemcpyDeviceToHost, st));
  }
  gcl_sort_job jobs[2][2 * GCL_MAX_MAPS];
  int n_jobs[2] = {0, 0};
  for (int s = 0; s < n_specs; ++s) {
    const gcl_map_spec& sp = specs[s];
    gcl_map_desc& d = out->maps[s];
    if (sp.kernel_size == 1) continue;
    for (int tr = 0; tr < 2; ++tr) {
      if (!(sp.tables & (1 << tr))) continue;
      const int32_t* tbl = tr ? d.nbr_t : d.nbr;
      GCL_CHECK_ARG(tbl, "gcl_maps_build: map %d has no transposed table (stride 1)", s);
      const long long rows = tr ? d.n_in : d.n_out;
      GCL_CHECK_ARG(d.K == 27, "gcl_maps_build: sorted tables are built for 3^3 kernels");
      int32_t* scratch = A.take_n<int32_t>(gcl_table_sort_scratch_len(rows));
      int32_t* order = A.take_n<int32_t>(rows);
      int32_t* sorted = A.take_n<int32_t>((long long)d.K * rows);
      int32_t* mask = A.take_n<int32_t>(cdiv(rows, 32));
      const int sd = on_side(sp) ? 1 : 0;
      jobs[sd][n_jobs[sd]++] = gcl_sort_job{tbl, d.K, rows, scratch, order, sorted, mask, d.counts};
      if (tr) { d.tbl_t = sorted; d.order_t = order; d.mask_t = mask; }
      else { d.tbl_n = sorted; d.order_n = order; d.mask_n = mask; }
    }
  }
  for (int s = 0; s < n_specs; ++s) {
    if (!(specs[s].tables & 4) || specs[s].kernel_size == 1) continue;
    gcl_map_desc& d = out->maps[s];
    d.presence = A.take_n<uint32_t>(d.n_out * ((d.K + 31) / 32));
    PLAN_CALL(gcl_presence_bits(d.nbr, d.K, d.n_out, d.presence, (on_side(specs[s]) && side) ? (void*)side : stream));
  }
  for (int sd = 0; sd < 2; ++sd) {
    void* sstream = (sd && side) ? (void*)side : stream;
    if (n_jobs[sd]) PLAN_CALL(gcl_table_sort_multi(jobs[sd], n_jobs[sd], sstream));
  }
  if (!side) out->late_mask = 0;
  if (!A.dry && any_pairs) GCL_CHECK_HIP(hipStreamSynchronize(st));
  for (int s = 0; s < n_specs; ++s) {
    const gcl_map_spec& sp = specs[s];
    gcl_map_desc& d = out->maps[s];
    if (sp.kernel_size == 1) {
      if (!sp.pairs) continue;
      const long long total = cdiv(d.n_in, GCL_PAIR_CHUNK) * GCL_PAIR_CHUNK;
      d.pair_in = d.pair_out = A.take_n<int32_t>(total);
      d.seg_off[0] = 0;
      d.seg_off[1] = total;
      d.n_pairs = d.n_in;
      d.counts_host[0] = (int32_t)d.n_in;
      if (!A.dry) {
        hipLaunchKernelGGL(k_identity_pairs, dim3((unsigned)cdiv(total, 256)), dim3(256), 0, st, d.pair_in, (long long)d.n_in,
                           total);
        GCL_CHECK_LAUNCH();
      }
      continue;
    }
    if (!any_pairs && !A.dry) continue;
    long long total = 0;
    d.seg_off[0] = 0;
    for (int k = 0; k < d.K; ++k) {
      const long long c = A.dry ? d.n_out : (long long)pinned[128 * (s + 1) + k];
      d.counts_host[k] = (int32_t)c;
      d.n_pairs += c;
      total += cdiv(c, GCL_PAIR_CHUNK) * GCL_PAIR_CHUNK;
      d.seg_off[k + 1] = total;
    }
    if (!sp.pairs) continue;
    const long long len = total > 0 ? total : 1;
    int32_t* both = A.take_n<int32_t>(2 * len);
    d.pair_in = both;
    d.pair_out = both + len;
    int32_t* scratch = A.take_n<int32_t>((long long)d.K * cdiv(d.n_out, 1024) + d.K + 1);
    PLAN_CALL(gcl_kernel_map_pairs(d.nbr, d.K, d.n_out, d.seg_off, scratch, d.pair_in, d.pair_out, stream));
    const long long nb = !A.dry ? gcl_conv_bwd_weight_bounds_len(d.K, d.n_out)
                                : (d.n_out >= 32768 && d.K > 1 && d.K <= 27 ? (long long)d.K * (cdiv(d.n_out, 512) + 1) : 0);
    if (nb > 0 && total > 0) {
      d.dw_bounds = A.take_n<int32_t>(nb);
      PLAN_CALL(gcl_conv_bwd_weight_bounds(d.pair_out, d.seg_off, d.K, d.n_out, d.dw_bounds, stream));
    }
  }
  out->arena_used = A.off;
  if (!A.fits()) {
    set_error("gcl_maps_build: arena too small (%lld bytes needed, %lld given)", A.off, A.size);
    return GCL_ERR_ARENA;
  }
  return GCL_OK;
}

struct RowView;
struct TState {
  float* ptr = nullptr;
  RowView* rv = nullptr;
  int32_t* amax = nullptr;
  void* planes = nullptr;
  int ld = 0;
};

struct OpSaved {
  float* conv_out = nullptr;
  unsigned long long* mask = nullptr;
  float *mean = nullptr, *rstd = nullptr;
  float* xrange = nullptr;
  int32_t* x_amax = nullptr;
  float* norm = nullptr;
};

struct ProfRec {
  hipEvent_t e0, e1;
  double kind, pairs, cin, cout, n_in, n_out, K;
};

struct PassState {
  const gcl_maps_desc* maps = nullptr;
  gcl_maps_desc maps_copy;
  std::vector<TState> t, g;
  std::vector<OpSaved> saved;
  std::vector<void*> params;
  Arena A{DRY_BASE, 0, 0, true};
  int32_t* slot_pool = nullptr;
  long long n_slots = 0, next_slot = 0;
  bool slots_exhausted = false;
  int32_t* w_amax = nullptr;
  unsigned char *pack_fwd = nullptr, *pack_bwd = nullptr;
  void* state = nullptr;
  bool forward_done = false, bwd_packed = false;
  std::vector<char> relu_masked;
  hipEvent_t fwd_packs = nullptr;
  bool fwd_packs_pending = false;
  int32_t* not_ones = nullptr;
  void* key = nullptr;
  const int32_t* fwd_rows = nullptr;
  long long fwd_cap = 0;
};

struct Plan : PassState {
  std::vector<PassState*> passes;
  std::vector<gcl_plan_op> ops;
  int n_tensors = 0, n_params = 0, n_bn = 0, presplit = 128;
  std::vector<int> worder;
  std::vector<int> widx;
  std::vector<int> wmode;
  std::vector<long long> wK, wcin, wcout, off_fwd, off_bwd;
  long long bytes_fwd = 0, bytes_bwd = 0, wgs_fwd = 0, wgs_bwd = 0;
  int n_bwd = 0;
  std::vector<char> made;
  std::vector<char> fuse_relu;
  std::vector<int> cat_left;
  std::vector<int> mask_from;
  std::vector<long long> host_tables, uploaded;
  bool eval = false;
  void* const* bn_eval = nullptr;
  bool eval_repack = true;
  hipStream_t aux = nullptr;
  std::vector<hipEvent_t> events;
  size_t events_used = 0;
  bool aux_dirty = false;
  int suffix_first = 0;
  bool suffix_rows_ok = false;
  const int32_t* touched = nullptr;
  long long touched_cap = 0;
  long long suffix_rows_used = 0;
  long long suffix_fwd_rows_used = 0;
  bool profile = false;
  std::vector<ProfRec> prof;
  size_t prof_used = 0;
};

static long long state_words(const Plan& P) { return (long long)P.worder.size() * (2 + 8 + 8); }

static int32_t* new_slot(Plan& P) {
  if (P.next_slot >= P.n_slots) {
    P.slots_exhausted = true;
    return P.slot_pool;
  }
  return P.slot_pool + (P.next_slot++) * GCL_AMAX_WORDS;
}

static int ensure_amax(Plan& P, TState& ts, long long numel, hipStream_t st) {
  Arena& A = P.A;
  if (ts.amax) return GCL_OK;
  ts.amax = new_slot(P);
  PLAN_CALL(gcl_amax(ts.ptr, numel, ts.amax, 1, (void*)st));
  return GCL_OK;
}

static int ensure_planes(Plan& P, TState& ts, long long n, int c, hipStream_t st) {
  Arena& A = P.A;
  if (ts.planes) return GCL_OK;
  ts.planes = A.take(n * c * 4);
  PLAN_CALL(gcl_split_planes(ts.ptr, n, c, ts.amax, ts.planes, (void*)st));
  return GCL_OK;
}

static hipStream_t fork_aux(Plan& P, hipStream_t st) {
  if (!P.aux || P.A.dry) return st;
  if (P.events_used == P.events.size()) {
    hipEvent_t e;
    if (hipEventCreateWithFlags(&e, hipEventDisableTiming) != hipSuccess) return st;
    P.events.push_back(e);
  }
  hipEvent_t e = P.events[P.events_used++];
  if (hipEventRecord(e, st) != hipSuccess || hipStreamWaitEvent(P.aux, e, 0) != hipSuccess) return st;
  P.aux_dirty = true;
  return P.aux;
}

static int join_aux(Plan& P, hipStream_t st) {
  if (!P.aux || !P.aux_dirty || P.A.dry) return GCL_OK;
  if (P.events_used == P.events.size()) {
    hipEvent_t e;
    GCL_CHECK_HIP(hipEventCreateWithFlags(&e, hipEventDisableTiming));
    P.events.push_back(e);
  }
  hipEvent_t e = P.events[P.events_used++];
  GCL_CHECK_HIP(hipEventRecord(e, P.aux));
  GCL_CHECK_HIP(hipStreamWaitEvent(st, e, 0));
  P.aux_dirty = false;
  return GCL_OK;
}

struct ProfScope {
  Plan& P;
  hipStream_t st;
  ProfRec* r = nullptr;
  ProfScope(Plan& P_, hipStream_t st_, int kind, double pairs, int cin, int cout, long long n_in, long long n_out, int K)
      : P(P_), st(st_) {
    if (!P.profile || P.A.dry) return;
    if (P.prof_used == P.prof.size()) {
      ProfRec nr{};
      if (hipEventCreate(&nr.e0) != hipSuccess || hipEventCreate(&nr.e1) != hipSuccess) return;
      P.prof.push_back(nr);
    }
    r = &P.prof[P.prof_used++];
    r->kind = kind; r->pairs = pairs; r->cin = cin; r->cout = cout; r->n_in = (double)n_in; r->n_out = (double)n_out; r->K = K;
    (void)hipEventRecord(r->e0, st);
  }
  ~ProfScope() { if (r) (void)hipEventRecord(r->e1, st); }
};

static bool is_stem(const gcl_plan_op& op, const gcl_map_desc& m) {
  return op.cin <= 4 && (op.cout % 32) == 0 && !op.transpose && m.kernel_size > 1 && op.bias < 0;
}

static int stem_flag(Plan& P, const gcl_plan_op& op, const gcl_map_desc& m, const TState& x, long long n_in, hipStream_t st) {
  Arena& A = P.A;
  if (!m.presence || P.not_ones) return GCL_OK;
  constexpr int CLOUD_FLAGS = 4096;
  int32_t* cloud = A.take_n<int32_t>(CLOUD_FLAGS);
  P.not_ones = A.take_n<int32_t>(n_in);
  PLAN_CALL(gcl_not_ones_rows(x.ptr, op.cin, P.maps->coords[op.level_in], n_in, cloud, CLOUD_FLAGS, P.not_ones, (void*)st));
  return GCL_OK;
}

struct SortedTable {
  const int32_t *tbl = nullptr, *order = nullptr, *mask = nullptr;
};
static SortedTable sorted_table(const gcl_map_desc& m, bool transposed) {
  if (m.kernel_size == 1) return SortedTable();
  return transposed ? SortedTable{m.tbl_t, m.order_t, m.mask_t} : SortedTable{m.tbl_n, m.order_n, m.mask_n};
}

static int conv_forward(Plan& P, int i, float** y_out, float** stats_out, hipStream_t st, int32_t** relu_amax_out,
                        long long rows = 0) {
  Arena& A = P.A;
  const gcl_plan_op& op = P.ops[i];
  const gcl_maps_desc& M = *P.maps;
  const gcl_map_desc& m = M.maps[op.map];
  const long long n_in = rows > 0 ? rows : M.n_rows[op.level_in], n_out = rows > 0 ? rows : M.n_rows[op.level_out];
  TState& x = P.t[op.x];
  float* y = A.take_n<float>(n_out * op.cout);
  *y_out = y;
  *stats_out = nullptr;
  *relu_amax_out = nullptr;
  const float* W = (const float*)P.params[op.w];
  if (is_stem(op, m)) {
    int rcs = stem_flag(P, op, m, x, n_in, st);
    if (rcs) return rcs;
    PLAN_CALL(gcl_stem_fwd(x.ptr, W, m.nbr, n_out, op.K, op.cin, op.cout, y, m.presence, m.presence ? P.not_ones : nullptr,
                           (void*)st));
    return GCL_OK;
  }
  const int wi = P.widx[op.w];
  if (P.fwd_packs_pending && !A.dry) {
    GCL_CHECK_HIP(hipStreamWaitEvent(st, P.fwd_packs, 0));
    P.fwd_packs_pending = false;
  }
  int rc = ensure_amax(P, x, n_in * op.cin, st);
  if (rc) return rc;
  P.saved[i].x_amax = x.amax;
  const bool pl = op.cin >= P.presplit;
  if (pl && (rc = ensure_planes(P, x, n_in, op.cin, st))) return rc;
  float* stats = nullptr;
  if (op.kind == GCL_OP_CONVBN) stats = A.take_n<float>(cdiv(n_out, 128) * 4 * op.cout);
  *stats_out = stats;
  const SortedTable T = sorted_table(m, op.transpose);
  GCL_CHECK_ARG(A.dry || m.kernel_size == 1 || T.tbl, "gcl_plan_forward: record %d needs a sorted table the maps do not carry", i);
  const float* bias = op.bias >= 0 ? (const float*)P.params[op.bias] : nullptr;
  ProfScope ps(P, st, 0, (double)(m.kernel_size > 1 ? m.n_pairs : n_out), op.cin, op.cout, n_in, n_out, op.K);
  int32_t* relu_amax = (op.kind == GCL_OP_CONV && P.fuse_relu[i]) ? new_slot(P) : nullptr;
  *relu_amax_out = relu_amax;
  PLAN_CALL(gcl_conv_fwd_fused(pl ? (const float*)x.planes : x.ptr, n_in, pl ? 1 : 0, P.pack_fwd + P.off_fwd[wi], 4, x.amax,
                               P.w_amax + (long long)wi * GCL_AMAX_WORDS, T.tbl, T.order, T.mask, n_out, op.K, op.cin, op.cout,
                               bias, nullptr, nullptr, relu_amax ? 1 : 0, relu_amax, y, stats, 0, (void*)st));
  return GCL_OK;
}

static int upload_tables(Plan& P, hipStream_t st) {
  const size_t n = P.worder.size();
  std::vector<long long>& h = P.host_tables;
  h.assign((size_t)state_words(P), 0);
  long long wg = 0;
  for (size_t q = 0; q < n; ++q) {
    h[q] = (long long)(uintptr_t)P.params[P.worder[q]];
    h[n + q] = P.wK[q] * P.wcin[q] * P.wcout[q];
    long long* d = &h[2 * n + 8 * q];
    d[0] = h[q]; d[1] = P.wK[q]; d[2] = P.wcin[q]; d[3] = P.wcout[q]; d[4] = 0; d[5] = (long long)q; d[6] = P.off_fwd[q]; d[7] = wg;
    wg += cdiv(h[n + q], 256);
  }
  P.wgs_fwd = wg;
  wg = 0;
  size_t row = 0;
  for (size_t q = 0; q < n; ++q) {
    if (!P.wmode[q]) continue;
    long long* d = &h[2 * n + 8 * n + 8 * row++];
    d[0] = h[q]; d[1] = P.wK[q]; d[2] = P.wcin[q]; d[3] = P.wcout[q]; d[4] = P.wmode[q]; d[5] = (long long)q; d[6] = P.off_bwd[q]; d[7] = wg;
    wg += cdiv(h[n + q], 256);
  }
  P.wgs_bwd = wg;
  if (h != P.uploaded) {
    GCL_CHECK_HIP(hipMemcpyAsync(P.state, h.data(), h.size() * sizeof(long long), hipMemcpyHostToDevice, st));
    GCL_CHECK_HIP(hipStreamSynchronize(st));
    P.uploaded = h;
  }
  return GCL_OK;
}

static int spread_rows(Plan& P, float* src, float* norm, const int32_t* rows, long long cap, int c, long long n, float** out,
                       hipStream_t st) {
  Arena& A = P.A;
  float* dst = A.take_n<float>(n * c);
  *out = dst;
  if (A.dry) return GCL_OK;
  GCL_CHECK_HIP(hipMemsetAsync(dst, 0, (size_t)(n * c) * sizeof(float), st));
  if (!norm) return gcl_scatter_rows(src, rows, cap, c, n, dst, c, (void*)st);
  hipLaunchKernelGGL(k_scatter_rows_inert, dim3(grid_for(cap * c / 4)), dim3(256), 0, st, (float4*)src, norm, (const int*)rows,
                     cap, c / 4, n, dst, c);
  GCL_CHECK_LAUNCH();
  return GCL_OK;
}

static int plan_forward(Plan& P, const float* x_in, void* const* bn_stats, float** y_out, hipStream_t st) {
  Arena& A = P.A;
  const gcl_maps_desc& M = *P.maps;
  const size_t nw = P.worder.size();
  P.t.assign(P.n_tensors, TState());
  P.g.assign(P.n_tensors, TState());
  P.saved.assign(P.ops.size(), OpSaved());
  if (P.profile && !A.dry) P.prof_used = 0;
  if (!A.dry) P.events_used = 0;
  P.n_slots = 4 * (long long)P.n_tensors + 2 * (long long)P.ops.size() + 16;
  P.next_slot = 0;
  P.slots_exhausted = false;
  P.not_ones = nullptr;
  P.fwd_packs_pending = false;
  P.slot_pool = A.take_n<int32_t>(P.n_slots * GCL_AMAX_WORDS);
  if (!A.dry) GCL_CHECK_HIP(hipMemsetAsync(P.slot_pool, 0, (size_t)P.n_slots * GCL_AMAX_WORDS * sizeof(int32_t), st));
  if (P.eval) {
    char* base = (char*)P.state + ((state_words(P) * 8 + 255) & ~255ll);
    P.w_amax = (int32_t*)base;
    P.pack_fwd = (unsigned char*)(base + (((long long)nw * GCL_AMAX_WORDS * 4 + 255) & ~255ll));
  } else {
    P.w_amax = A.take_n<int32_t>((long long)nw * GCL_AMAX_WORDS);
    P.pack_fwd = (unsigned char*)A.take(P.bytes_fwd);
  }
  P.bwd_packed = false;
  if (nw && !A.dry) {
    int rc = upload_tables(P, st);
    if (rc) return rc;
    if (!P.eval || P.eval_repack) {
      const long long* tab = (const long long*)P.state;
      hipStream_t ps = st;
      if (!P.eval && P.aux && P.n_bwd) ps = fork_aux(P, st);
      PLAN_CALL(gcl_amax_multi((const float* const*)tab, (const int64_t*)(tab + nw), (int32_t)nw, P.w_amax, (void*)ps));
      PLAN_CALL(gcl_pack_weights_multi((const int64_t*)(tab + 2 * nw), (int32_t)nw, P.wgs_fwd, 4, P.w_amax, P.pack_fwd, (void*)ps));
      if (ps != st) {
        if (P.events_used == P.events.size()) {
          hipEvent_t e;
          GCL_CHECK_HIP(hipEventCreateWithFlags(&e, hipEventDisableTiming));
          P.events.push_back(e);
        }
        P.fwd_packs = P.events[P.events_used++];
        GCL_CHECK_HIP(hipEventRecord(P.fwd_packs, ps));
        P.fwd_packs_pending = true;
      }
    }
  }
  if (!P.eval && P.aux && P.n_bwd) {
    P.pack_bwd = (unsigned char*)A.take(P.bytes_bwd);
    if (!A.dry) {
      hipStream_t ws = fork_aux(P, st);
      const long long* tab = (const long long*)P.state;
      PLAN_CALL(gcl_pack_weights_multi((const int64_t*)(tab + 2 * nw + 8 * nw), P.n_bwd, P.wgs_bwd, 4, P.w_amax, P.pack_bwd,
                                       (void*)ws));
    }
    P.bwd_packed = true;
  }
  P.t[0].ptr = (float*)x_in;
  bool late_pending = !A.dry && M.ready_event && M.late_mask;
  for (size_t i = 0; i < P.ops.size(); ++i) {
    const gcl_plan_op& op = P.ops[i];
    const bool compact = P.fwd_cap > 0 && (int)i >= P.suffix_first;
    const long long n_out = compact ? P.fwd_cap : M.n_rows[op.level_out];
    if (compact && (int)i == P.suffix_first) {
      TState& xs = P.t[op.x];
      float* cx = A.take_n<float>(P.fwd_cap * op.cin);
      PLAN_CALL(gcl_gather_rows(xs.ptr, xs.ld ? xs.ld : op.cin, M.n_rows[op.level_in], P.fwd_rows, P.fwd_cap, op.cin, 0.f, cx,
                                (void*)st));
      int32_t* slot = xs.amax;
      xs = TState();
      xs.ptr = cx;
      xs.amax = slot;
    }
    if (late_pending && (op.kind == GCL_OP_CONVBN || op.kind == GCL_OP_CONV) && ((M.late_mask >> op.map) & 1)) {
      GCL_CHECK_HIP(hipStreamWaitEvent(st, (hipEvent_t)M.ready_event, 0));
      late_pending = false;
    }
    TState& y = P.t[op.y];
    int rc;
    switch (op.kind) {
      case GCL_OP_CONVBN: {
        if (P.eval) {
          const gcl_map_desc& m = M.maps[op.map];
          const long long n_in = M.n_rows[op.level_in];
          TState& x = P.t[op.x];
          const int c = op.cout;
          const float* res = op.x2 >= 0 ? P.t[op.x2].ptr : nullptr;
          y.ptr = A.take_n<float>(n_out * c);
          y.amax = new_slot(P);
          void* const* be = P.bn_eval ? P.bn_eval + 4 * op.bn : nullptr;
          if (is_stem(op, m)) {
            float* cy = A.take_n<float>(n_out * c);
            unsigned long long* mask = op.relu ? A.take_n<unsigned long long>(gcl_bn_mask_len(n_out, c)) : nullptr;
            if ((rc = stem_flag(P, op, m, x, n_in, st))) return rc;
            PLAN_CALL(gcl_stem_fwd(x.ptr, (const float*)P.params[op.w], m.nbr, n_out, op.K, op.cin, c, cy, m.presence,
                                   m.presence ? P.not_ones : nullptr, (void*)st));
            PLAN_CALL(gcl_bn_apply(cy, n_out, c, (const float*)be[2], (const float*)be[3], (const float*)P.params[op.bn_w],
                                   (const float*)P.params[op.bn_b], res, op.relu, y.ptr, (uint64_t*)mask, y.amax, (void*)st));
            break;
          }
          const int wi = P.widx[op.w];
          if ((rc = ensure_amax(P, x, n_in * op.cin, st))) return rc;
          const SortedTable T = sorted_table(m, op.transpose);
          GCL_CHECK_ARG(A.dry || m.kernel_size == 1 || T.tbl,
                        "gcl_plan_forward_eval: record %d needs a sorted table the maps do not carry", (int)i);
          const long long gs_len = T.tbl ? gcl_conv_fwd_groups_scratch_len(n_out, op.K, op.cin, c) : 0;
          float* gscratch = gs_len > 0 ? A.take_n<float>(gs_len) : nullptr;
          ProfScope ps(P, st, 0, (double)(m.kernel_size > 1 ? m.n_pairs : n_out), op.cin, c, n_in, n_out, op.K);
          PLAN_CALL(gcl_conv_fwd_fused(x.ptr, n_in, 0, P.pack_fwd + P.off_fwd[wi], 4, x.amax,
                                       P.w_amax + (long long)wi * GCL_AMAX_WORDS, T.tbl, T.order, T.mask, n_out, op.K, op.cin, c,
                                       (const float*)be[1], (const float*)be[0], res, op.relu, y.amax, y.ptr, gscratch,
                                       GCL_CONV_TALL, (void*)st));
          break;
        }
        float *cy, *stats;
        int32_t* unused_slot;
        if ((rc = conv_forward(P, (int)i, &cy, &stats, st, &unused_slot))) return rc;
        OpSaved& sv = P.saved[i];
        sv.conv_out = cy;
        const int c = op.cout;
        float* mr = A.take_n<float>(2 * c);
        sv.mean = mr;
        sv.rstd = mr + c;
        float* rm = (float*)bn_stats[2 * op.bn];
        float* rv = (float*)bn_stats[2 * op.bn + 1];
        const int32_t* res_amax = op.x2 >= 0 ? P.t[op.x2].amax : nullptr;
        const int32_t* cat_amax = P.cat_left[i] >= 0 ? P.t[P.ops[P.cat_left[i]].x2].amax : nullptr;
        const bool bound = stats && c >= P.presplit && (c % 32) == 0 && (op.x2 < 0 || res_amax) &&
                           (P.cat_left[i] < 0 || (cat_amax && (P.ops[P.cat_left[i]].cout % 32) == 0));
        int32_t* bound_slot = bound ? new_slot(P) : nullptr;
        if (stats) {
          const long long nt = cdiv(n_out, 128);
          if (bound) sv.xrange = A.take_n<float>(2 * c);
          PLAN_CALL(gcl_bn_stats_from_tiles_range(stats, nt, n_out, c, op.eps, op.momentum, rm, rv, sv.mean, sv.rstd, sv.xrange,
                                                  (const float*)P.params[op.bn_w], (const float*)P.params[op.bn_b], op.relu,
                                                  res_amax, cat_amax, bound_slot, (void*)st));
        } else {
          double* scratch = A.take_n<double>(gcl_bn_scratch_len(n_out, c));
          PLAN_CALL(gcl_bn_stats(cy, n_out, c, op.eps, op.momentum, rm, rv, scratch, sv.mean, sv.rstd, (void*)st));
        }
        if (P.cat_left[i] >= 0) {
          const gcl_plan_op& cat = P.ops[P.cat_left[i]];
          TState& cty = P.t[cat.y];
          cty = TState();
          cty.ptr = A.take_n<float>(n_out * cat.cout);
          cty.amax = bound ? bound_slot : new_slot(P);
          if (bound) cty.planes = A.take(n_out * cat.cout * 4);
          y.ptr = cty.ptr;
          y.ld = cat.cout;
          y.amax = cty.amax;
          y.planes = nullptr;
        } else {
          y.ptr = A.take_n<float>(n_out * c);
          y.ld = 0;
          y.amax = bound ? bound_slot : new_slot(P);
          if (bound) y.planes = A.take(n_out * c * 4);
        }
        if (op.relu) sv.mask = A.take_n<unsigned long long>(gcl_bn_mask_len(n_out, c));
        const float* res = op.x2 >= 0 ? P.t[op.x2].ptr : nullptr;
        void* img = !bound ? nullptr : (P.cat_left[i] >= 0 ? P.t[P.ops[P.cat_left[i]].y].planes : y.planes);
        PLAN_CALL(gcl_bn_apply_planes(cy, n_out, c, sv.mean, sv.rstd, (const float*)P.params[op.bn_w],
                                      (const float*)P.params[op.bn_b], res, op.relu, y.ptr, y.ld, (uint64_t*)sv.mask, y.amax,
                                      img, (void*)st));
        break;
      }
      case GCL_OP_CONV: {
        float *cy, *stats;
        int32_t* relu_amax;
        if ((rc = conv_forward(P, (int)i, &cy, &stats, st, &relu_amax, compact ? P.fwd_cap : 0))) return rc;
        y.ptr = cy;
        if (relu_amax) {
          y.amax = relu_amax;
          P.t[P.ops[i + 1].y] = y;
        }
        break;
      }
      case GCL_OP_RELU: {
        if (i > 0 && P.fuse_relu[i - 1]) {
          if (compact) y = P.t[op.x];
          break;
        }
        const long long n4 = n_out * op.cout / 4;
        y.ptr = A.take_n<float>(n_out * op.cout);
        y.amax = new_slot(P);
        if (!A.dry) {
          hipLaunchKernelGGL(k_relu_fwd, dim3(grid_for(n4)), dim3(256), 0, st, (const float4*)P.t[op.x].ptr, n4, (float4*)y.ptr,
                             y.amax);
          GCL_CHECK_LAUNCH();
        }
        break;
      }
      case GCL_OP_CAT: {
        const int ca = op.cin, cb = op.cout - op.cin;
        if (P.t[op.x].ld == op.cout && P.t[op.x].ptr == y.ptr && y.ptr) {
          if (!A.dry) {
            hipLaunchKernelGGL(k_cat_right, dim3(grid_for(n_out * cb / 4)), dim3(256), 0, st, (const float4*)P.t[op.x2].ptr,
                               cb / 4, n_out, ca / 4, (float4*)y.ptr, y.amax, (unsigned short*)y.planes);
            GCL_CHECK_LAUNCH();
          }
          break;
        }
        y.ptr = A.take_n<float>(n_out * op.cout);
        y.amax = new_slot(P);
        const int32_t *sa = P.t[op.x].amax, *sb = P.t[op.x2].amax;
        if (!A.dry) {
          const bool both = sa && sb;
          hipLaunchKernelGGL(k_cat2, dim3(grid_for(n_out * op.cout / 4)), dim3(256), 0, st, (const float4*)P.t[op.x].ptr, ca / 4,
                             (const float4*)P.t[op.x2].ptr, cb / 4, n_out, (float4*)y.ptr, y.amax, both ? (const int*)sa : nullptr,
                             both ? (const int*)sb : nullptr);
          GCL_CHECK_LAUNCH();
        }
        break;
      }
      case GCL_OP_ROWNORM: {
        y.ptr = A.take_n<float>(n_out * op.cout);
        P.saved[i].norm = A.take_n<float>(n_out);
        PLAN_CALL(gcl_row_normalize_fwd(P.t[op.x].ptr, n_out, op.cout, y.ptr, P.saved[i].norm, (void*)st));
        break;
      }
      default:
        set_error("gcl_plan_forward: unknown record kind %d", op.kind);
        return GCL_ERR_ARG;
    }
  }
  if (late_pending) GCL_CHECK_HIP(hipStreamWaitEvent(st, (hipEvent_t)M.ready_event, 0));
  *y_out = P.t[P.ops.back().y].ptr;
  if (P.fwd_cap > 0) {
    const gcl_plan_op& last = P.ops.back();
    return spread_rows(P, *y_out, last.kind == GCL_OP_ROWNORM ? P.saved[P.ops.size() - 1].norm : nullptr, P.fwd_rows, P.fwd_cap,
                       last.cout, M.n_rows[last.level_out], y_out, st);
  }
  return GCL_OK;
}

struct RowView {
  const int32_t* rows = nullptr;
  long long cap = 0, n = 0;
  bool parked = false;
  std::vector<std::pair<const float*, float*>> gathered;
  int32_t* slots = nullptr;
  long long n_rows(const gcl_maps_desc& M, int level) const { return cap > 0 ? cap : M.n_rows[level]; }
};

static int contiguous(Plan& P, TState& g, long long rows, int c, hipStream_t st);

static int densify(Plan& P, TState& g, int c, hipStream_t st) {
  if (!g.rv || !g.ptr) return GCL_OK;
  const RowView& V = *g.rv;
  int rc;
  if ((rc = contiguous(P, g, V.cap, c, st))) return rc;
  float* dense;
  if ((rc = spread_rows(P, g.ptr, nullptr, V.rows, V.cap, c, V.n, &dense, st))) return rc;
  g = TState();
  g.ptr = dense;
  return GCL_OK;
}

static int give(Plan& P, int tensor, float* gptr, long long numel, hipStream_t st, int32_t* amax = nullptr, int ld = 0,
                int c = 0, RowView* rv = nullptr) {
  Arena& A = P.A;
  if (tensor < 0 || !P.made[tensor] || !gptr) return GCL_OK;
  TState& g = P.g[tensor];
  if (!g.ptr) {
    g = TState();
    g.ptr = gptr;
    g.ld = ld;
    g.rv = rv;
    g.amax = amax;
    return GCL_OK;
  }
  if (g.rv || rv) {
    GCL_CHECK_ARG(c > 0 && c % 4 == 0, "gcl_plan_backward: a compact gradient needs its channel count");
    TState in;
    in.ptr = gptr;
    in.ld = ld;
    in.rv = rv;
    numel = (g.rv ? g.rv : rv)->n * c;
    int rc;
    if ((rc = densify(P, g, c, st)) || (rc = densify(P, in, c, st))) return rc;
    gptr = in.ptr;
    ld = in.ld;
  }
  float* sum = A.take_n<float>(numel);
  if (!A.dry) {
    if (g.ld || ld) {
      GCL_CHECK_ARG(c > 0 && c % 4 == 0, "gcl_plan_backward: a sliced gradient needs its channel count");
      hipLaunchKernelGGL(k_add2_ld, dim3(grid_for(numel / 4)), dim3(256), 0, st, (const float*)g.ptr, g.ld ? g.ld : c,
                         (const float*)gptr, ld ? ld : c, numel / c, c / 4, (float4*)sum);
    } else {
      hipLaunchKernelGGL(k_add2, dim3(grid_for(numel / 4)), dim3(256), 0, st, (const float4*)g.ptr, (const float4*)gptr,
                         numel / 4, (float4*)sum);
    }
    GCL_CHECK_LAUNCH();
  }
  g = TState();
  g.ptr = sum;
  return GCL_OK;
}

static int contiguous(Plan& P, TState& g, long long rows, int c, hipStream_t st) {
  if (!g.ld || !g.ptr) return GCL_OK;
  Arena& A = P.A;
  float* out = A.take_n<float>(rows * c);
  if (!A.dry) {
    hipLaunchKernelGGL(k_add2_ld, dim3(grid_for(rows * c / 4)), dim3(256), 0, st, (const float*)g.ptr, g.ld, (const float*)nullptr,
                       0, rows, c / 4, (float4*)out);
    GCL_CHECK_LAUNCH();
  }
  g = TState();
  g.ptr = out;
  return GCL_OK;
}

static int saved_rows(Plan& P, RowView& V, const float* src, int ld, int c, float pad, hipStream_t st, const float** out) {
  Arena& A = P.A;
  *out = src;
  if (V.cap <= 0 || V.parked) return GCL_OK;
  for (auto& e : V.gathered)
    if (e.first == src) {
      *out = e.second;
      return GCL_OK;
    }
  float* rows = A.take_n<float>(V.cap * c);
  PLAN_CALL(gcl_gather_rows(src, ld, V.n, V.rows, V.cap, c, pad, rows, (void*)st));
  V.gathered.push_back({src, rows});
  *out = rows;
  return GCL_OK;
}
static int saved_rows(Plan& P, RowView& V, const TState& t, int c, hipStream_t st, const float** out) {
  return saved_rows(P, V, t.ptr, t.ld ? t.ld : c, c, 0.f, st, out);
}

static int row_slots(Plan& P, RowView& V, hipStream_t st) {
  Arena& A = P.A;
  if (V.slots) return GCL_OK;
  V.slots = A.take_n<int32_t>(V.n);
  PLAN_CALL(gcl_row_slots(V.rows, V.cap, V.n, V.slots, (void*)st));
  return GCL_OK;
}

static int conv_backward(Plan& P, int i, TState dy, RowView& V, void* const* grads, hipStream_t st) {
  Arena& A = P.A;
  const gcl_plan_op& op = P.ops[i];
  const gcl_maps_desc& M = *P.maps;
  const gcl_map_desc& m = M.maps[op.map];
  const long long n_in = V.n_rows(M, op.level_in), n_out = V.n_rows(M, op.level_out);
  TState& x = P.t[op.x];
  float* dW = (float*)grads[op.w];
  int rc;
  if (is_stem(op, m)) {
    float* scratch = A.take_n<float>(gcl_stem_bwd_weight_scratch_len(op.K, op.cin, op.cout, n_out));
    hipStream_t ws = fork_aux(P, st);
    ProfScope ps(P, ws, 2, (double)m.n_pairs, op.cin, op.cout, n_in, n_out, op.K);
    PLAN_CALL(gcl_stem_bwd_weight(x.ptr, dy.ptr, m.nbr, n_out, op.K, op.cin, op.cout, scratch, dW, m.presence,
                                  m.presence ? P.not_ones : nullptr, (void*)ws));
    return GCL_OK;
  }
  const int wi = P.widx[op.w];
  if ((rc = ensure_amax(P, dy, n_out * op.cout, st))) return rc;
  const int32_t* w_amax = P.w_amax + (long long)wi * GCL_AMAX_WORDS;
  const double pairs = (double)(m.kernel_size > 1 ? m.n_pairs : n_out);
  const long long rows_len = m.kernel_size == 1 ? gcl_conv_bwd_weight_rows_scratch_len(op.cin, op.cout, 4, n_in) : 0;
  const bool pl_w = rows_len <= 0 && op.cin >= P.presplit && op.cout >= P.presplit;
  const bool pl_x = op.cout >= P.presplit;
  if ((pl_w || (pl_x && P.made[op.x])) && (rc = ensure_planes(P, dy, n_out, op.cout, st))) return rc;
  if (pl_w) {
    x.amax = P.saved[i].x_amax;
    if ((rc = ensure_planes(P, x, n_in, op.cin, st))) return rc;
  }
  const float* xr;
  if ((rc = saved_rows(P, V, x, op.cin, st, &xr))) return rc;
  hipStream_t ws = fork_aux(P, st);
  if (P.made[op.x]) {
    const int mode = (m.kernel_size > 1 && !op.transpose && m.stride == 1) ? 2 : 1;
    const SortedTable T = sorted_table(m, !op.transpose && m.stride != 1);
    const int32_t *tbl = T.tbl, *order = T.order, *mask = T.mask;
    GCL_CHECK_ARG(mode == P.wmode[wi], "gcl_plan_backward: record %d: input-gradient pack mode mismatch", i);
    GCL_CHECK_ARG(A.dry || m.kernel_size == 1 || tbl, "gcl_plan_backward: record %d needs a sorted table the maps do not carry", i);
    const bool pl = pl_x;
    float* acc = P.g[op.x].ptr;
    const int acc_ld = P.g[op.x].ld;
    const RowView* acc_rows = P.g[op.x].rv;
    GCL_CHECK_ARG(!acc_rows || (V.cap <= 0 && acc_rows->n == n_in && op.cin % 4 == 0),
                  "gcl_plan_backward: record %d: a compact gradient waits at an input of another shape", i);
    float* dx = A.take_n<float>(n_in * op.cin);
    int32_t* dx_amax = nullptr;
    {
      ProfScope ps(P, st, acc && !acc_rows ? 1 : 0, pairs, op.cout, op.cin, n_out, n_in, op.K);
      if (acc && !acc_rows)
        PLAN_CALL(gcl_conv_fwd_fused_ld(pl ? (const float*)dy.planes : dy.ptr, n_out, pl ? 1 : 0, P.pack_bwd + P.off_bwd[wi], 4,
                                        dy.amax, w_amax, tbl, order, mask, n_in, op.K, op.cout, op.cin, nullptr, nullptr, acc,
                                        acc_ld, 0, nullptr, dx, nullptr, 0, (void*)st));
      else if (!acc && P.mask_from[i] >= 0) {
        dx_amax = new_slot(P);
        PLAN_CALL(gcl_conv_fwd_fused(pl ? (const float*)dy.planes : dy.ptr, n_out, pl ? 1 : 0, P.pack_bwd + P.off_bwd[wi], 4,
                                     dy.amax, w_amax, tbl, order, mask, n_in, op.K, op.cout, op.cin, nullptr, nullptr, xr, 2,
                                     dx_amax, dx, nullptr, 0, (void*)st));
        if (P.relu_masked.size() != P.ops.size()) P.relu_masked.assign(P.ops.size(), 0);
        P.relu_masked[P.mask_from[i]] = 1;
      } else
        PLAN_CALL(gcl_conv_fwd(pl ? (const float*)dy.planes : dy.ptr, n_out, pl ? 1 : 0, P.pack_bwd + P.off_bwd[wi], 4, dy.amax,
                               w_amax, tbl, order, mask, n_in, op.K, op.cout, op.cin, nullptr, dx, nullptr, 0, (void*)st));
    }
    if (acc_rows)
      PLAN_CALL(gcl_scatter_add_rows(acc, acc_ld ? acc_ld : op.cin, acc_rows->rows, acc_rows->cap, op.cin, n_in, dx, op.cin,
                                     (void*)st));
    P.g[op.x] = TState();
    P.g[op.x].ptr = dx;
    P.g[op.x].amax = dx_amax;
  }
  if (rows_len > 0) {
    float* scratch = A.take_n<float>(rows_len);
    ProfScope ps(P, ws, 3, pairs, op.cin, op.cout, n_in, n_out, op.K);
    PLAN_CALL(gcl_conv_bwd_weight_rows(xr, dy.ptr, n_in, op.cin, op.cout, 4, P.saved[i].x_amax, dy.amax, scratch, dW,
                                       (void*)ws));
  } else {
    GCL_CHECK_ARG(V.cap <= 0, "gcl_plan_backward: record %d: the pair-list weight gradient does not run on a row list", i);
    const int32_t *pa = m.pair_in, *pb = m.pair_out;
    if (op.transpose) { pa = m.pair_out; pb = m.pair_in; }
    GCL_CHECK_ARG(A.dry || (pa && pb), "gcl_plan_backward: record %d needs pair lists the maps do not carry", i);
    const int sorted_side = m.kernel_size == 1 ? 0 : (op.transpose ? 1 : 2);
    const long long n_sorted = sorted_side == 1 ? n_in : (sorted_side == 2 ? n_out : 0);
    float* scratch = A.take_n<float>(gcl_conv_bwd_weight_scratch_len(op.K, op.cin, op.cout, m.seg_off[op.K], n_sorted));
    const bool pl = pl_w;
    ProfScope ps(P, ws, 2, pairs, op.cin, op.cout, n_in, n_out, op.K);
    const int32_t* rgb = (sorted_side != 0 && n_sorted == m.n_out) ? m.dw_bounds : nullptr;
    PLAN_CALL(gcl_conv_bwd_weight_rg(pl ? (const float*)x.planes : x.ptr, n_in, pl ? (const float*)dy.planes : dy.ptr, n_out,
                                     pl ? 1 : 0, sorted_side, pa, pb, m.seg_off, op.K, op.cin, op.cout, 4, P.saved[i].x_amax,
                                     dy.amax, scratch, dW, rgb, (void*)ws));
  }
  if (op.bias >= 0) {
    double* scratch = A.take_n<double>(gcl_bn_scratch_len(n_out, op.cout));
    PLAN_CALL(gcl_col_sum(dy.ptr, n_out, op.cout, scratch, (float*)grads[op.bias], (void*)ws));
  }
  return GCL_OK;
}

static int backward_record(Plan& P, int i, RowView& V, void* const* grads, hipStream_t st) {
  Arena& A = P.A;
  const gcl_maps_desc& M = *P.maps;
  const gcl_plan_op& op = P.ops[i];
  const long long n_out = V.n_rows(M, op.level_out), n_in = V.n_rows(M, op.level_in);
  TState g = P.g[op.y];
  P.g[op.y] = TState();
  if (!g.ptr) return GCL_OK;
  int rc;
  const bool rows_ok = g.rv && V.cap <= 0 && g.rv->n == n_out &&
                       (op.kind == GCL_OP_CAT || (op.kind == GCL_OP_CONVBN && (!op.relu || P.saved[i].mask)));
  if (g.rv && !rows_ok && (rc = densify(P, g, op.cout, st))) return rc;
  RowView* const rv = g.rv;
  switch (op.kind) {
    case GCL_OP_CONVBN: {
      const OpSaved& sv = P.saved[i];
      const int c = op.cout;
      float* sum_g = (float*)grads[op.bn_b];
      float* sum_gx = (float*)grads[op.bn_w];
      double* scratch = A.take_n<double>(gcl_bn_scratch_len(n_out, c));
      const bool bound = sv.xrange && c >= P.presplit && !is_stem(op, M.maps[op.map]);
      TState d;
      d.ptr = A.take_n<float>(n_out * c);
      d.amax = new_slot(P);
      if (rv) {
        if ((rc = row_slots(P, *rv, st))) return rc;
        PLAN_CALL(gcl_bn_bwd_reduce_rows(sv.conv_out, g.ptr, g.ld, rv->slots, (const uint64_t*)sv.mask, n_out, c, sv.mean, sv.rstd,
                                         op.relu, scratch, sum_g, sum_gx, sv.xrange, (const float*)P.params[op.bn_w],
                                         bound ? d.amax : nullptr, (void*)st));
      } else {
        PLAN_CALL(gcl_bn_bwd_reduce_range(sv.conv_out, g.ptr, g.ld, nullptr, (const uint64_t*)sv.mask, n_out, c, sv.mean, sv.rstd,
                                          op.relu, scratch, sum_g, sum_gx, sv.xrange, (const float*)P.params[op.bn_w],
                                          bound ? d.amax : nullptr, (void*)st));
      }
      if (bound) d.planes = A.take(n_out * c * 4);
      const long long res_rows = rv ? rv->cap : n_out;
      float* dres = op.x2 >= 0 ? A.take_n<float>(res_rows * c) : nullptr;
      if (rv)
        PLAN_CALL(gcl_bn_bwd_apply_rows(sv.conv_out, g.ptr, g.ld, rv->slots, (const uint64_t*)sv.mask, n_out, c, sv.mean, sv.rstd,
                                        (const float*)P.params[op.bn_w], sum_g, sum_gx, op.relu, d.ptr, dres, d.amax, d.planes,
                                        (void*)st));
      else
        PLAN_CALL(gcl_bn_bwd_apply_planes(sv.conv_out, g.ptr, g.ld, nullptr, (const uint64_t*)sv.mask, n_out, c, sv.mean,
                                          sv.rstd, (const float*)P.params[op.bn_w], sum_g, sum_gx, op.relu, d.ptr, dres,
                                          d.amax, d.planes, (void*)st));
      if ((rc = conv_backward(P, i, d, V, grads, st))) return rc;
      return give(P, op.x2, dres, res_rows * c, st, nullptr, 0, c, rv);
    }
    case GCL_OP_CONV:
      if ((rc = contiguous(P, g, n_out, op.cout, st))) return rc;
      return conv_backward(P, i, g, V, grads, st);
    case GCL_OP_RELU: {
      if ((size_t)i < P.relu_masked.size() && P.relu_masked[i]) {
        P.relu_masked[i] = 0;
        return give(P, op.x, g.ptr, n_out * op.cout, st, g.amax, g.ld, op.cout);
      }
      if ((rc = contiguous(P, g, n_out, op.cout, st))) return rc;
      const float* y;
      if ((rc = saved_rows(P, V, P.t[op.y], op.cout, st, &y))) return rc;
      const long long numel = n_out * op.cout;
      float* gx = A.take_n<float>(numel);
      int32_t* slot = new_slot(P);
      if (!A.dry) {
        hipLaunchKernelGGL(k_relu_bwd, dim3(grid_for(numel / 4)), dim3(256), 0, st, (const float4*)g.ptr, (const float4*)y,
                           numel / 4, (float4*)gx, slot);
        GCL_CHECK_LAUNCH();
      }
      return give(P, op.x, gx, numel, st, slot, 0, op.cout);
    }
    case GCL_OP_CAT: {
      const int ca = op.cin, cb = op.cout - op.cin;
      const long long rows = rv ? rv->cap : n_out;
      if ((rc = contiguous(P, g, rows, op.cout, st))) return rc;
      if ((rc = give(P, op.x, g.ptr, rows * ca, st, nullptr, op.cout, ca, rv))) return rc;
      return give(P, op.x2, g.ptr + ca, rows * cb, st, nullptr, op.cout, cb, rv);
    }
    case GCL_OP_ROWNORM: {
      if ((rc = contiguous(P, g, n_out, op.cout, st))) return rc;
      const float *y, *norm;
      if ((rc = saved_rows(P, V, P.t[op.y], op.cout, st, &y))) return rc;
      if ((rc = saved_rows(P, V, P.saved[i].norm, 1, 1, 1.f, st, &norm))) return rc;
      float* dx = A.take_n<float>(n_in * op.cin);
      int32_t* slot = new_slot(P);
      PLAN_CALL(gcl_row_normalize_bwd(y, g.ptr, norm, n_out, op.cout, dx, slot, (void*)st));
      return give(P, op.x, dx, n_in * op.cin, st, slot, 0, op.cin);
    }
    default:
      set_error("gcl_plan_backward: unknown record kind %d", op.kind);
      return GCL_ERR_ARG;
  }
}

static int suffix_backward(Plan& P, const float* dy, void* const* grads, RowView& V, hipStream_t st) {
  Arena& A = P.A;
  const gcl_plan_op &head = P.ops[P.suffix_first], &tail = P.ops.back();
  V.n = P.maps->n_rows[head.level_in];
  V.parked = P.fwd_cap > 0;
  float* dyc = A.take_n<float>(V.cap * tail.cout);
  PLAN_CALL(gcl_gather_rows(dy, tail.cout, V.n, V.rows, V.cap, tail.cout, 0.f, dyc, (void*)st));
  P.g[tail.y] = TState();
  P.g[tail.y].ptr = dyc;
  int rc;
  for (int i = (int)P.ops.size() - 1; i >= P.suffix_first; --i)
    if ((rc = backward_record(P, i, V, grads, st))) return rc;
  const TState g = P.g[head.x];
  P.g[head.x] = TState();
  A.take_n<float>(V.n * head.cin);
  if (!g.ptr) return GCL_OK;
  return give(P, head.x, g.ptr, V.cap * head.cin, st, nullptr, 0, head.cin, &V);
}

static int tensor_width(const Plan& P, int tensor) {
  for (const gcl_plan_op& op : P.ops)
    if (op.y == tensor) return op.cout;
  return 0;
}

static int plan_backward(Plan& P, const float* dy, void* const* grads, int first, int last, hipStream_t st,
                         const int32_t* rows = nullptr, long long cap = 0) {
  Arena& A = P.A;
  const gcl_maps_desc& M = *P.maps;
  const size_t nw = P.worder.size();
  const int n_ops = (int)P.ops.size();
  if (last == (int)P.ops.size()) {
    P.g[P.ops.back().y] = TState();
    P.g[P.ops.back().y].ptr = (float*)dy;
  }
  if (P.bwd_packed && last == (int)P.ops.size()) {
    int rcj = join_aux(P, st);
    if (rcj) return rcj;
  }
  if (!P.bwd_packed) {
    P.pack_bwd = (unsigned char*)A.take(P.bytes_bwd);
    if (P.n_bwd && !A.dry) {
      const long long* tab = (const long long*)P.state;
      PLAN_CALL(gcl_pack_weights_multi((const int64_t*)(tab + 2 * nw + 8 * nw), P.n_bwd, P.wgs_bwd, 4, P.w_amax, P.pack_bwd,
                                       (void*)st));
    }
    P.bwd_packed = true;
  }
  int top = last - 1, rc;
  long long reserve_to = 0;
  RowView list;
  if (last == n_ops && !A.dry) P.suffix_rows_used = 0;
  if (last == n_ops && P.suffix_first < n_ops && P.suffix_rows_ok && first <= P.suffix_first) {
    const long long n = M.n_rows[P.ops[P.suffix_first].level_in];
    auto run = [&](const int32_t* r, long long c, bool counted, long long* end) {
      RowView scratch_view;
      RowView& V = counted ? scratch_view : list;
      V.rows = r;
      V.cap = c;
      const Arena a0 = A;
      const long long slot0 = P.next_slot;
      std::vector<TState> g0;
      std::vector<char> masked0;
      if (counted) {
        g0 = P.g;
        masked0 = P.relu_masked;
        A.dry = true;
      }
      const int rcs = suffix_backward(P, dy, grads, V, st);
      *end = A.off;
      if (counted) {
        A = a0;
        P.next_slot = slot0;
        P.g = g0;
        P.relu_masked = masked0;
      }
      return rcs;
    };
    long long end = 0;
    if (P.fwd_cap > 0) {
      rows = P.fwd_rows;
      cap = P.fwd_cap;
    } else if (A.dry) {
      cap = 0;
      if ((n - 1) / 2 > 0 && (rc = run(nullptr, (n - 1) / 2, true, &reserve_to))) return rc;
    } else if (!rows || cap <= 0 || 2 * cap >= n || run(rows, cap, true, &end) != GCL_OK || end > A.size) {
      cap = 0;
    }
    if (cap > 0) {
      if ((rc = run(rows, cap, false, &end))) return rc;
      top = P.suffix_first - 1;
      if (!A.dry) P.suffix_rows_used = cap;
    }
  }
  RowView dense;
  for (int i = top; i >= first; --i) {
    if (reserve_to && i == P.suffix_first - 1 && A.off < reserve_to) A.off = reserve_to;
    if ((rc = backward_record(P, i, dense, grads, st))) return rc;
  }
  if (reserve_to && A.off < reserve_to) A.off = reserve_to;
  for (size_t t = 0; t < P.g.size(); ++t)
    if (P.g[t].rv && (rc = densify(P, P.g[t], tensor_width(P, (int)t), st))) return rc;
  return join_aux(P, st);
}

static int check_maps(const Plan& P, const gcl_maps_desc* M) {
  GCL_CHECK_ARG(M && M->n_levels >= 1 && M->n_levels <= GCL_MAX_LEVELS && M->n_maps >= 0 && M->n_maps <= GCL_MAX_MAPS,
                "gcl_plan: bad maps descriptor");
  for (size_t i = 0; i < P.ops.size(); ++i) {
    const gcl_plan_op& op = P.ops[i];
    GCL_CHECK_ARG(op.level_in < M->n_levels && op.level_out < M->n_levels, "gcl_plan: record %d uses a level the maps lack", (int)i);
    if (op.kind == GCL_OP_CONVBN || op.kind == GCL_OP_CONV) {
      GCL_CHECK_ARG(op.map >= 0 && op.map < M->n_maps, "gcl_plan: record %d names map %d of %d", (int)i, op.map, M->n_maps);
      const gcl_map_desc& m = M->maps[op.map];
      GCL_CHECK_ARG(m.K == op.K, "gcl_plan: record %d expects K = %d, map %d has %d", (int)i, op.K, op.map, m.K);
      const int lin = op.transpose ? m.level_out : m.level_in, lout = op.transpose ? m.level_in : m.level_out;
      GCL_CHECK_ARG(lin == op.level_in && lout == op.level_out, "gcl_plan: record %d and map %d disagree on the levels", (int)i, op.map);
    }
  }
  return GCL_OK;
}

}

using namespace gcl;

extern "C" {

static int dry_pass(Plan& P, const float* x, void* const* bn_stats, bool backward, long long* need) {
  std::vector<void*> nulls(2 * (P.n_bn > 0 ? P.n_bn : 1), nullptr), gn(P.n_params, nullptr);
  const Arena real = P.A;
  const bool prof = P.profile;
  P.A = Arena{DRY_BASE, 0, 0, true};
  P.profile = false;
  float* y = nullptr;
  int rc = plan_forward(P, x, bn_stats ? bn_stats : nulls.data(), &y, nullptr);
  if (rc == GCL_OK && backward) rc = plan_backward(P, (const float*)DRY_BASE, gn.data(), 0, (int)P.ops.size(), nullptr);
  *need = P.A.off;
  P.A = real;
  P.profile = prof;
  P.relu_masked.clear();
  return rc;
}

static void park(Plan& P, PassState* slot) {
  *slot = std::move(static_cast<PassState&>(P));
  slot->maps = &slot->maps_copy;
  static_cast<PassState&>(P) = PassState();
}
static void unpark(Plan& P, PassState* slot) {
  static_cast<PassState&>(P) = std::move(*slot);
  P.maps = &P.maps_copy;
}

int64_t gcl_maps_arena_bytes(int64_t n, const gcl_map_spec* specs_host, int32_t n_specs, int32_t n_levels) {
  if (n <= 0 || !specs_host || n_specs < 0 || n_specs > GCL_MAX_MAPS || n_levels < 1 || n_levels > GCL_MAX_LEVELS) return -1;
  Arena A{DRY_BASE, 0, 0, true};
  gcl_maps_desc d;
  if (maps_build(nullptr, n, specs_host, n_specs, n_levels, A, nullptr, &d, nullptr) != GCL_OK) return -1;
  return A.off + 4096;
}

int gcl_maps_build_split(const int32_t* coords, int64_t n, const gcl_map_spec* specs_host, int32_t n_specs, int32_t n_levels,
                         void* arena, int64_t arena_bytes, void* pinned_host, gcl_maps_desc* out_host, void* stream,
                         void* side_stream) {
  GCL_CHECK_ARG(coords && specs_host && arena && pinned_host && out_host, "gcl_maps_build: null pointer");
  GCL_CHECK_ARG(side_stream != stream || !side_stream, "gcl_maps_build_split: the side stream must differ from the stream");
  GCL_CHECK_ARG(n > 0, "gcl_maps_build: empty SparseTensor");
  GCL_CHECK_ARG(n_specs >= 0 && n_specs <= GCL_MAX_MAPS && n_levels >= 1 && n_levels <= GCL_MAX_LEVELS,
                "gcl_maps_build: at most %d maps and %d levels", GCL_MAX_MAPS, GCL_MAX_LEVELS);
  const int64_t need = gcl_maps_arena_bytes(n, specs_host, n_specs, n_levels);
  GCL_CHECK_ARG(need >= 0, "gcl_maps_build: bad map specification");
  if (arena_bytes < need) {
    set_error("gcl_maps_build: arena too small (%lld bytes needed, %lld given)", (long long)need, (long long)arena_bytes);
    return GCL_ERR_ARENA;
  }
  Arena A{(char*)arena, arena_bytes, 0, false};
  return maps_build(coords, n, specs_host, n_specs, n_levels, A, (int32_t*)pinned_host, out_host, (hipStream_t)stream,
                    (hipStream_t)side_stream);
}

int gcl_maps_build(const int32_t* coords, int64_t n, const gcl_map_spec* specs_host, int32_t n_specs, int32_t n_levels,
                   void* arena, int64_t arena_bytes, void* pinned_host, gcl_maps_desc* out_host, void* stream) {
  return gcl_maps_build_split(coords, n, specs_host, n_specs, n_levels, arena, arena_bytes, pinned_host, out_host, stream, nullptr);
}

void* gcl_plan_create(const gcl_plan_op* ops_host, int32_t n_ops, int32_t n_tensors, int32_t n_params,
                      const int32_t* weight_order_host, int32_t n_weights, int32_t presplit_min_c) {
  if (!ops_host || n_ops <= 0 || n_tensors <= 1 || n_params <= 0 || n_weights < 0 || (n_weights && !weight_order_host)) {
    set_error("gcl_plan_create: bad argument");
    return nullptr;
  }
  Plan* P = new (std::nothrow) Plan();
  if (!P) {
    set_error("gcl_plan_create: out of host memory");
    return nullptr;
  }
  P->ops.assign(ops_host, ops_host + n_ops);
  P->n_tensors = n_tensors;
  P->n_params = n_params;
  P->presplit = presplit_min_c > 0 ? presplit_min_c : 128;
  P->worder.assign(weight_order_host, weight_order_host + n_weights);
  P->widx.assign(n_params, -1);
  P->made.assign(n_tensors, 0);
  const size_t nw = (size_t)n_weights;
  P->wmode.assign(nw, 0);
  P->wK.assign(nw, 0);
  P->wcin.assign(nw, 0);
  P->wcout.assign(nw, 0);
  P->off_fwd.assign(nw, 0);
  P->off_bwd.assign(nw, 0);
  bool ok = true;
  for (int q = 0; q < n_weights && ok; ++q) {
    const int p = weight_order_host[q];
    ok = p >= 0 && p < n_params && P->widx[p] < 0;
    if (ok) P->widx[p] = q;
  }
  std::vector<char> seen_param(n_params, 0);
  for (int i = 0; i < n_ops && ok; ++i) {
    const gcl_plan_op& op = P->ops[i];
    auto tensor_ok = [&](int t) { return t >= 0 && t < n_tensors; };
    ok = tensor_ok(op.x) && tensor_ok(op.y) && op.y != 0 && !P->made[op.y] && (op.x == 0 || P->made[op.x]) &&
         op.level_in >= 0 && op.level_in < GCL_MAX_LEVELS && op.level_out >= 0 && op.level_out < GCL_MAX_LEVELS &&
         op.cin > 0 && op.cout > 0;
    if (!ok) break;
    if (op.x2 >= 0) ok = tensor_ok(op.x2) && P->made[op.x2];
    if (!ok) break;
    auto claim = [&](int p) {
      if (p < 0 || p >= n_params || seen_param[p]) return false;
      seen_param[p] = 1;
      return true;
    };
    if (op.kind == GCL_OP_CONVBN || op.kind == GCL_OP_CONV) {
      ok = claim(op.w) && op.map >= 0 && op.map < GCL_MAX_MAPS && op.K >= 1 && op.K <= 125;
      if (ok && op.bias >= 0) ok = claim(op.bias) && op.kind == GCL_OP_CONV;
      if (ok && op.kind == GCL_OP_CONVBN) ok = claim(op.bn_w) && claim(op.bn_b) && op.bn >= 0 && op.cout % 4 == 0;
      if (ok && op.kind == GCL_OP_CONVBN) P->n_bn = op.bn + 1 > P->n_bn ? op.bn + 1 : P->n_bn;
      if (!ok) break;
      const bool stem_shape = op.cin <= 4 && (op.cout % 32) == 0 && !op.transpose && op.K > 1 && op.bias < 0;
      if (!stem_shape) {
        ok = (op.cin % 32) == 0 && (op.cout % 32) == 0 && op.K <= 27 && P->widx[op.w] >= 0;
        if (!ok) break;
        const int q = P->widx[op.w];
        P->wK[q] = op.K; P->wcin[q] = op.cin; P->wcout[q] = op.cout;
        if (op.x != 0) P->wmode[q] = (op.K > 1 && !op.transpose && op.level_in == op.level_out) ? 2 : 1;
      } else {
        ok = op.x == 0;
      }
    } else if (op.kind == GCL_OP_CAT) {
      ok = op.x2 >= 0 && op.cin % 4 == 0 && (op.cout - op.cin) > 0 && (op.cout - op.cin) % 4 == 0 && op.level_in == op.level_out;
    } else if (op.kind == GCL_OP_RELU || op.kind == GCL_OP_ROWNORM) {
      ok = op.cin == op.cout && op.cout % 4 == 0 && op.level_in == op.level_out;
    } else {
      ok = false;
    }
    P->made[op.y] = 1;
  }
  P->fuse_relu.assign(P->ops.size(), 0);
  for (size_t i = 0; ok && i + 1 < P->ops.size(); ++i) {
    const gcl_plan_op &a = P->ops[i], &b = P->ops[i + 1];
    if (a.kind != GCL_OP_CONV || b.kind != GCL_OP_RELU || b.x != a.y || a.cin <= 4) continue;
    bool other = a.y == P->ops.back().y;
    for (size_t j = 0; j < P->ops.size(); ++j)
      if (j != i + 1 && (P->ops[j].x == a.y || P->ops[j].x2 == a.y)) other = true;
    if (!other) P->fuse_relu[i] = 1;
  }
  P->cat_left.assign(P->ops.size(), -1);
  for (size_t i = 0; ok && i < P->ops.size(); ++i) {
    const gcl_plan_op& a = P->ops[i];
    if (a.kind != GCL_OP_CONVBN || a.cin <= 4 || a.y == P->ops.back().y) continue;
    int cat = -1, consumers = 0;
    for (size_t j = 0; j < P->ops.size(); ++j) {
      if (P->ops[j].kind == GCL_OP_CAT && P->ops[j].x == a.y && P->ops[j].x2 != a.y && j > i) cat = (int)j;
      consumers += (P->ops[j].x == a.y) + (P->ops[j].x2 == a.y);
    }
    if (cat >= 0 && consumers == 1) P->cat_left[i] = cat;
  }
  P->mask_from.assign(P->ops.size(), -1);
  for (size_t i = 0; ok && i < P->ops.size(); ++i) {
    const gcl_plan_op& a = P->ops[i];
    if ((a.kind != GCL_OP_CONV && a.kind != GCL_OP_CONVBN) || a.cin <= 4 || a.x == 0) continue;
    int r = -1, consumers = 0;
    for (size_t j = 0; j < P->ops.size(); ++j) {
      if (P->ops[j].kind == GCL_OP_RELU && P->ops[j].y == a.x) r = (int)j;
      consumers += (P->ops[j].x == a.x) + (P->ops[j].x2 == a.x);
    }
    if (r >= 0 && consumers == 1 && a.x != P->ops.back().y) P->mask_from[i] = r;
  }
  if (!ok) {
    set_error("gcl_plan_create: malformed or unsupported operator records");
    delete P;
    return nullptr;
  }
  {
    auto consumers = [&](int t) {
      int c = 0;
      for (const gcl_plan_op& o : P->ops) c += (o.x == t) + (o.x2 == t);
      return c;
    };
    auto row_local = [](const gcl_plan_op& o) {
      return o.kind == GCL_OP_ROWNORM || o.kind == GCL_OP_RELU ||
             (o.kind == GCL_OP_CONV && o.K == 1 && !o.transpose && o.level_in == o.level_out && o.cin > 4);
    };
    int s = n_ops;
    while (s > 0 && row_local(P->ops[s - 1]) &&
           (s == n_ops || (P->ops[s].x == P->ops[s - 1].y && consumers(P->ops[s - 1].y) == 1)))
      --s;
    while (s < n_ops && consumers(P->ops[s].x) != 1) ++s;
    P->suffix_first = s;
    P->suffix_rows_ok = true;
    for (int i = s; i < n_ops; ++i)
      if (P->ops[i].kind == GCL_OP_CONV && gcl_conv_bwd_weight_rows_scratch_len(P->ops[i].cin, P->ops[i].cout, 4, 128) <= 0)
        P->suffix_rows_ok = false;
  }
  for (size_t q = 0; q < nw; ++q) {
    if (!P->wK[q]) {
      set_error("gcl_plan_create: weight_order names a parameter no record uses");
      delete P;
      return nullptr;
    }
    const long long bytes = (gcl_pack_weights_bytes((int)P->wK[q], (int)P->wcin[q], (int)P->wcout[q], 4) + 255) / 256 * 256;
    P->off_fwd[q] = P->bytes_fwd;
    P->bytes_fwd += bytes;
    if (P->wmode[q]) {
      P->off_bwd[q] = P->bytes_bwd;
      P->bytes_bwd += bytes;
      ++P->n_bwd;
    }
  }
  return P;
}

void gcl_plan_destroy(void* plan) {
  Plan* P = (Plan*)plan;
  if (!P) return;
  for (ProfRec& r : P->prof) {
    (void)hipEventDestroy(r.e0);
    (void)hipEventDestroy(r.e1);
  }
  for (PassState* q : P->passes) delete q;
  for (hipEvent_t e : P->events) (void)hipEventDestroy(e);
  delete P;
}

int64_t gcl_plan_state_bytes(const void* plan) {
  if (!plan) return -1;
  return state_words(*(const Plan*)plan) * 8 + 256;
}

int64_t gcl_plan_arena_bytes(void* plan, const gcl_maps_desc* maps_host) {
  Plan* P = (Plan*)plan;
  if (!P || check_maps(*P, maps_host) != GCL_OK) return -1;
  P->maps = maps_host;
  P->params.assign(P->n_params, nullptr);
  long long need = 0;
  const int rc = dry_pass(*P, nullptr, nullptr, true, &need);
  P->forward_done = false;
  return rc == GCL_OK ? need + 4096 : -1;
}

int gcl_plan_forward(void* plan, const gcl_maps_desc* maps_host, const float* x, void* const* params_host,
                     void* const* bn_stats_host, void* state, void* arena, int64_t arena_bytes, float** y_out_host,
                     void* stream) {
  Plan* P = (Plan*)plan;
  GCL_CHECK_ARG(P && maps_host && x && params_host && bn_stats_host && state && arena && y_out_host, "gcl_plan_forward: null pointer");
  int rc = check_maps(*P, maps_host);
  if (rc) return rc;
  P->maps_copy = *maps_host;
  P->maps = &P->maps_copy;
  P->params.assign(params_host, params_host + P->n_params);
  P->state = state;
  P->A = Arena{(char*)arena, arena_bytes, 0, false};
  P->forward_done = false;
  long long need = 0;
  if ((rc = dry_pass(*P, x, bn_stats_host, true, &need))) return rc;
  if (need > arena_bytes) {
    set_error("gcl_plan_forward: arena too small (%lld bytes needed, %lld given)", need, (long long)arena_bytes);
    return GCL_ERR_ARENA;
  }
  const int n_ops = (int)P->ops.size();
  P->suffix_fwd_rows_used = 0;
  if (P->touched && P->touched_cap > 0 && P->suffix_first < n_ops && P->suffix_rows_ok && P->ops.back().cout % 4 == 0 &&
      2 * P->touched_cap < maps_host->n_rows[P->ops[P->suffix_first].level_in]) {
    P->fwd_rows = P->touched;
    P->fwd_cap = P->touched_cap;
    if (dry_pass(*P, x, bn_stats_host, true, &need) != GCL_OK || need > arena_bytes) {
      P->fwd_rows = nullptr;
      P->fwd_cap = 0;
    }
  }
  rc = plan_forward(*P, x, bn_stats_host, y_out_host, (hipStream_t)stream);
  P->forward_done = rc == GCL_OK;
  if (rc != GCL_OK) {
    P->fwd_rows = nullptr;
    P->fwd_cap = 0;
    return rc;
  }
  if (P->fwd_cap > 0) {
    P->suffix_fwd_rows_used = P->fwd_cap;
    P->touched = nullptr;
    P->touched_cap = 0;
  }
  PassState* slot = nullptr;
  for (PassState* q : P->passes)
    if (!q->forward_done || q->key == arena) slot = q;
  if (!slot) {
    slot = new (std::nothrow) PassState();
    GCL_CHECK_ARG(slot, "gcl_plan_forward: out of host memory");
    P->passes.push_back(slot);
  }
  P->key = arena;
  park(*P, slot);
  return GCL_OK;
}

int64_t gcl_plan_eval_state_bytes(const void* plan) {
  if (!plan) return -1;
  const Plan& P = *(const Plan*)plan;
  return ((state_words(P) * 8 + 255) & ~255ll) + (((long long)P.worder.size() * GCL_AMAX_WORDS * 4 + 255) & ~255ll) +
         P.bytes_fwd + 256;
}

int64_t gcl_plan_eval_arena_bytes(void* plan, const gcl_maps_desc* maps_host) {
  Plan* P = (Plan*)plan;
  if (!P || check_maps(*P, maps_host) != GCL_OK) return -1;
  P->maps = maps_host;
  P->params.assign(P->n_params, nullptr);
  P->eval = true;
  P->bn_eval = nullptr;
  P->state = DRY_BASE;
  long long need = 0;
  const int rc = dry_pass(*P, nullptr, nullptr, false, &need);
  P->eval = false;
  P->forward_done = false;
  return rc == GCL_OK ? need + 4096 : -1;
}

int gcl_plan_forward_eval(void* plan, const gcl_maps_desc* maps_host, const float* x, void* const* params_host,
                          void* const* bn_eval_host, int32_t repack, void* state, void* arena, int64_t arena_bytes,
                          float** y_out_host, void* stream) {
  Plan* P = (Plan*)plan;
  GCL_CHECK_ARG(P && maps_host && x && params_host && bn_eval_host && state && arena && y_out_host,
                "gcl_plan_forward_eval: null pointer");
  int rc = check_maps(*P, maps_host);
  if (rc) return rc;
  P->maps_copy = *maps_host;
  P->maps = &P->maps_copy;
  P->params.assign(params_host, params_host + P->n_params);
  P->state = state;
  P->eval = true;
  P->bn_eval = bn_eval_host;
  P->eval_repack = repack != 0;
  std::vector<void*> nulls(2 * (P->n_bn > 0 ? P->n_bn : 1), nullptr);
  long long need = 0;
  rc = dry_pass(*P, x, nulls.data(), false, &need);
  if (rc == GCL_OK && need > arena_bytes) {
    set_error("gcl_plan_forward_eval: arena too small (%lld bytes needed, %lld given)", need, (long long)arena_bytes);
    rc = GCL_ERR_ARENA;
  }
  if (rc == GCL_OK) {
    P->A = Arena{(char*)arena, arena_bytes, 0, false};
    rc = plan_forward(*P, x, nulls.data(), y_out_host, (hipStream_t)stream);
  }
  if (rc == GCL_OK && P->slots_exhausted) {
    set_error("gcl_plan_forward_eval: amax slot pool exhausted");
    rc = GCL_ERR_ARG;
  }
  P->eval = false;
  P->bn_eval = nullptr;
  P->forward_done = false;
  static_cast<PassState&>(*P) = PassState();
  return rc;
}

int gcl_plan_release(void* plan, void* arena) {
  Plan* P = (Plan*)plan;
  GCL_CHECK_ARG(P, "gcl_plan_release: null plan");
  bool found = false;
  for (PassState* q : P->passes)
    if (q->forward_done && q->key == arena) found = true;
  if (found && P->aux && P->aux_dirty) {
    GCL_CHECK_HIP(hipStreamSynchronize(P->aux));
    P->aux_dirty = false;
  }
  for (PassState* q : P->passes)
    if (q->forward_done && q->key == arena) *q = PassState();
  return GCL_OK;
}

int gcl_plan_backward(void* plan, void* arena, const float* dy, void* const* grads_host, int32_t first_op,
                      int32_t last_op, void* stream) {
  Plan* P = (Plan*)plan;
  GCL_CHECK_ARG(P, "gcl_plan_backward: null pointer");
  const int32_t* rows = P->touched;
  const long long cap = P->touched_cap;
  P->touched = nullptr;
  P->touched_cap = 0;
  GCL_CHECK_ARG(grads_host, "gcl_plan_backward: null pointer");
  PassState* slot = nullptr;
  for (PassState* q : P->passes)
    if (q->forward_done && q->key == arena) slot = q;
  GCL_CHECK_ARG(slot, "gcl_plan_backward: no forward pass to differentiate in this arena");
  GCL_CHECK_ARG(first_op >= 0 && first_op < last_op && last_op <= (int)P->ops.size(), "gcl_plan_backward: bad record range");
  GCL_CHECK_ARG(last_op != (int)P->ops.size() || dy, "gcl_plan_backward: the last segment needs dy");
  if (slot->fwd_cap > 0) {
    GCL_CHECK_ARG(!rows || (rows == slot->fwd_rows && cap == slot->fwd_cap),
                  "gcl_plan_backward: the forward pass of this arena ran the touched-row suffix on another list");
    GCL_CHECK_ARG(last_op <= P->suffix_first || (first_op <= P->suffix_first && last_op == (int)P->ops.size()),
                  "gcl_plan_backward: the record range [%d, %d) cuts the touched-row suffix [%d, %d), which the forward pass "
                  "ran on the rows of a list: there are no dense operands to fall back to",
                  (int)first_op, (int)last_op, P->suffix_first, (int)P->ops.size());
  }
  unpark(*P, slot);
  int rc = plan_backward(*P, dy, grads_host, first_op, last_op, (hipStream_t)stream, rows, cap);
  if (rc == GCL_OK && !P->A.fits()) {
    set_error("gcl_plan_backward: arena overrun");
    rc = GCL_ERR_ARENA;
  }
  if (rc == GCL_OK && P->slots_exhausted) {
    set_error("gcl_plan_backward: amax slot pool exhausted");
    rc = GCL_ERR_ARG;
  }
  if (first_op == 0 || rc != GCL_OK) P->forward_done = false;
  park(*P, slot);
  return rc;
}

int gcl_plan_set_aux_stream(void* plan, void* stream) {
  Plan* P = (Plan*)plan;
  GCL_CHECK_ARG(P, "gcl_plan_set_aux_stream: null plan");
  P->aux = (hipStream_t)stream;
  return GCL_OK;
}

int gcl_plan_touched_suffix(const void* plan) {
  if (!plan) return -1;
  return ((const Plan*)plan)->suffix_first;
}

int gcl_gather_rows(const float* src, int32_t ld, int64_t n_src, const int32_t* rows, int64_t cap, int32_t c, float pad,
                    float* out, void* stream) {
  GCL_CHECK_ARG(src && rows && out && n_src > 0 && cap > 0 && c > 0 && ld >= c, "gcl_gather_rows: bad argument");
  const bool vec = c % 4 == 0 && ld % 4 == 0 && (((uintptr_t)src | (uintptr_t)out) & 15) == 0;
  if (vec)
    hipLaunchKernelGGL(k_gather_rows<float4>, dim3(grid_for(cap * c / 4)), dim3(256), 0, (hipStream_t)stream, src, ld,
                       (long long)n_src, (const int*)rows, (long long)cap, c / 4, pad, (float4*)out);
  else
    hipLaunchKernelGGL(k_gather_rows<float>, dim3(grid_for(cap * c)), dim3(256), 0, (hipStream_t)stream, src, ld,
                       (long long)n_src, (const int*)rows, (long long)cap, c, pad, out);
  GCL_CHECK_LAUNCH();
  return GCL_OK;
}

int gcl_scatter_rows(const float* src, const int32_t* rows, int64_t cap, int32_t c, int64_t n_dst, float* dst, int32_t ld,
                     void* stream) {
  GCL_CHECK_ARG(src && rows && dst && n_dst > 0 && cap > 0, "gcl_scatter_rows: bad argument");
  GCL_CHECK_ARG(c > 0 && c % 4 == 0 && ld >= c && ld % 4 == 0 && (((uintptr_t)src | (uintptr_t)dst) & 15) == 0,
                "gcl_scatter_rows: channel count and row pitch must be multiples of 4, the tensors 16-byte aligned");
  hipLaunchKernelGGL(k_scatter_rows, dim3(grid_for(cap * c / 4)), dim3(256), 0, (hipStream_t)stream, (const float4*)src,
                     (const int*)rows, (long long)cap, c / 4, (long long)n_dst, dst, ld);
  GCL_CHECK_LAUNCH();
  return GCL_OK;
}

int gcl_scatter_add_rows(const float* src, int32_t src_ld, const int32_t* rows, int64_t cap, int32_t c, int64_t n_dst,
                         float* dst, int32_t ld, void* stream) {
  GCL_CHECK_ARG(src && rows && dst && n_dst > 0 && cap > 0, "gcl_scatter_add_rows: bad argument");
  GCL_CHECK_ARG(c > 0 && c % 4 == 0 && ld >= c && ld % 4 == 0 && src_ld >= c && src_ld % 4 == 0 &&
                    (((uintptr_t)src | (uintptr_t)dst) & 15) == 0,
                "gcl_scatter_add_rows: channel count and row pitches must be multiples of 4, the tensors 16-byte aligned");
  hipLaunchKernelGGL(k_scatter_add_rows, dim3(grid_for(cap * c / 4)), dim3(256), 0, (hipStream_t)stream, src, src_ld,
                     (const int*)rows, (long long)cap, c / 4, (long long)n_dst, dst, ld);
  GCL_CHECK_LAUNCH();
  return GCL_OK;
}

int gcl_row_slots(const int32_t* rows, int64_t cap, int64_t n, int32_t* slots, void* stream) {
  GCL_CHECK_ARG(rows && slots && n > 0 && cap > 0 && cap < (1ll << 31), "gcl_row_slots: bad argument");
  GCL_CHECK_HIP(hipMemsetAsync(slots, 0xff, (size_t)n * sizeof(int32_t), (hipStream_t)stream));
  hipLaunchKernelGGL(k_row_slots, dim3((unsigned)cdiv(cap, 256)), dim3(256), 0, (hipStream_t)stream, (const int*)rows,
                     (long long)cap, (long long)n, slots);
  GCL_CHECK_LAUNCH();
  return GCL_OK;
}

int64_t gcl_plan_suffix_rows_used(const void* plan) {
  if (!plan) return -1;
  return ((const Plan*)plan)->suffix_rows_used;
}

int64_t gcl_plan_suffix_fwd_rows_used(const void* plan) {
  if (!plan) return -1;
  return ((const Plan*)plan)->suffix_fwd_rows_used;
}

int gcl_plan_set_touched_rows(void* plan, const int32_t* rows, int64_t cap) {
  Plan* P = (Plan*)plan;
  GCL_CHECK_ARG(P, "gcl_plan_set_touched_rows: null plan");
  GCL_CHECK_ARG((rows && cap > 0) || (!rows && cap == 0), "gcl_plan_set_touched_rows: a list needs a positive length");
  P->touched = rows;
  P->touched_cap = cap;
  return GCL_OK;
}

int64_t gcl_touched_rows_scratch_len(int64_t n_rows) { return n_rows > 0 ? gcl_scan_scratch_len(n_rows) : 0; }

int gcl_touched_rows(const int64_t* index, int64_t n_index, const int64_t* goff, int64_t n_groups, const int64_t* sel,
                     int32_t n_sel, const int64_t* rows_a, int32_t n_a, const int64_t* rows_b, int32_t n_b, int64_t n_rows,
                     int32_t* scratch, int32_t* rows, int64_t cap, int32_t* n_touched, void* stream) {
  GCL_CHECK_ARG(scratch && rows && n_touched && n_rows > 0 && n_rows < (1ll << 31) && cap > 0,
                "gcl_touched_rows: bad argument");
  GCL_CHECK_ARG(n_sel >= 0 && n_a >= 0 && n_b >= 0 && n_index >= 0 && n_groups >= 0, "gcl_touched_rows: negative count");
  GCL_CHECK_ARG(n_sel == 0 || (index && goff && sel), "gcl_touched_rows: group selections need index, goff and sel");
  GCL_CHECK_ARG((n_a == 0 || rows_a) && (n_b == 0 || rows_b), "gcl_touched_rows: null row array");
  hipStream_t st = (hipStream_t)stream;
  int32_t *flag = scratch, *pos = scratch + n_rows, *bs = scratch + 2 * n_rows;
  GCL_CHECK_HIP(hipMemsetAsync(flag, 0, (size_t)n_rows * sizeof(int32_t), st));
  if (n_sel)
    hipLaunchKernelGGL(k_touch_groups, dim3((unsigned)n_sel), dim3(64), 0, st, (const long long*)index, (long long)n_index,
                       (const long long*)goff, (long long)n_groups, (const long long*)sel, (long long)n_rows, flag);
  if (n_a)
    hipLaunchKernelGGL(k_touch_rows, dim3((unsigned)cdiv(n_a, 256)), dim3(256), 0, st, (const long long*)rows_a, (long long)n_a,
                       (long long)n_rows, flag);
  if (n_b)
    hipLaunchKernelGGL(k_touch_rows, dim3((unsigned)cdiv(n_b, 256)), dim3(256), 0, st, (const long long*)rows_b, (long long)n_b,
                       (long long)n_rows, flag);
  GCL_CHECK_LAUNCH();
  int rc = gcl_exclusive_scan_i32(flag, n_rows, pos, bs, stream);
  if (rc) return rc;
  const long long items = n_rows > cap ? n_rows : cap;
  hipLaunchKernelGGL(k_touch_emit, dim3((unsigned)cdiv(items, 256)), dim3(256), 0, st, (const int*)flag, (const int*)pos,
                     (long long)n_rows, rows, (long long)cap, n_touched);
  GCL_CHECK_LAUNCH();
  return GCL_OK;
}

int gcl_stream_create_cu_share(int32_t percent, int32_t low_priority, void** stream_out) {
  GCL_CHECK_ARG(stream_out && percent >= 1 && percent <= 100, "gcl_stream_create_cu_share: percent must be 1..100");
  int dev = 0;
  hipDeviceProp_t prop;
  GCL_CHECK_HIP(hipGetDevice(&dev));
  GCL_CHECK_HIP(hipGetDeviceProperties(&prop, dev));
  const int n_cu = prop.multiProcessorCount, words = (n_cu + 31) / 32;
  int on = (int)((long long)n_cu * percent / 100);
  if (on < 8) on = 8;
  std::vector<uint32_t> mask((size_t)words, 0u);
  for (int i = 0; i < on && i < n_cu; ++i) mask[(size_t)i >> 5] |= 1u << (i & 31);
  hipStream_t st = nullptr;
  GCL_CHECK_HIP(hipExtStreamCreateWithCUMask(&st, (uint32_t)words, mask.data()));
  (void)low_priority;
  *stream_out = (void*)st;
  return GCL_OK;
}

int gcl_stream_destroy(void* stream) {
  if (stream) GCL_CHECK_HIP(hipStreamDestroy((hipStream_t)stream));
  return GCL_OK;
}

int gcl_plan_profile(void* plan, int32_t enable) {
  Plan* P = (Plan*)plan;
  GCL_CHECK_ARG(P, "gcl_plan_profile: null plan");
  P->profile = enable != 0;
  return GCL_OK;
}

int gcl_plan_profile_read(void* plan, double* records_host, int32_t max_records) {
  Plan* P = (Plan*)plan;
  if (!P || !records_host) return GCL_ERR_ARG;
  int n = 0;
  for (size_t i = 0; i < P->prof_used && n < max_records; ++i) {
    const ProfRec& r = P->prof[i];
    float ms = 0.f;
    if (hipEventElapsedTime(&ms, r.e0, r.e1) != hipSuccess) continue;
    double* o = records_host + 8 * n++;
    o[0] = r.kind; o[1] = ms; o[2] = r.pairs; o[3] = r.cin; o[4] = r.cout; o[5] = r.n_in; o[6] = r.n_out; o[7] = r.K;
  }
  return n;
}

}
```

### include/gcl_amd.h

```cpp
#ifndef GCL_AMD_H
#define GCL_AMD_H

#include <stdint.h>

#ifdef __cplusplus
extern "C" {
#endif

#define GCL_OK 0
#define GCL_ERR_ARG (-1)
#define GCL_ERR_HIP (-2)
#define GCL_ERR_NO_DEVICE (-3)

#define GCL_PAIR_CHUNK 128

const char* gcl_last_error(void);
int gcl_version(void);
int gcl_device_count(void);

int gcl_coords_insert(const int32_t* coords, int64_t n, int64_t* table, int64_t cap,
                      int32_t* status, void* stream);

int64_t gcl_scan_scratch_len(int64_t n);
int gcl_stride_map(const int32_t* coords_in, int64_t n_in, const int32_t* n_in_dev, int32_t t_out,
// ... 271 lines not shown
int gcl_mutual_match(const int32_t* nn01, int32_t m0, const int32_t* nn10, int32_t m1, const float* kp0, const float* kp1,
                     const float* T, float tau, int32_t* pairs, int32_t* stats, void* stream);
int gcl_mutual_correspondences(const int32_t* nn01, int32_t m0, const int32_t* nn10, int32_t m1, const float* xyz0,
                               const float* xyz1, int32_t min_count, float* src, float* tgt, int32_t* count, void* stream);
typedef struct gcl_mutual_job {
  const int32_t* nn01;
  const int32_t* nn10;
  const float* xyz0;
  const float* xyz1;
  const float* T;
  int32_t* pairs;
  float* src;
  float* tgt;
  int32_t* count;
  int32_t m0, m1;
} gcl_mutual_job;
int gcl_mutual_match_batch(const gcl_mutual_job* jobs_host, const gcl_mutual_job* jobs, int32_t n_pairs, float tau,
                           void* stream);
int gcl_mutual_correspondences_batch(const gcl_mutual_job* jobs_host, const gcl_mutual_job* jobs, int32_t n_pairs,
                                     int32_t min_count, void* stream);

int gcl_neg_mask(const int64_t* sel1, const int64_t* sel2, const int32_t* arg, int32_t m,
                 const int64_t* index, const int64_t* goff, int64_t n_groups, int64_t n_index,
                 int64_t* table, int64_t cap, uint8_t* keep, void* stream);
int gcl_neg_loss_fwd(const float* dmin, const uint8_t* keep, int32_t m, float thresh, float* out, void* stream);
int gcl_neg_loss_bwd(const float* f, int32_t c, const int64_t* sel1, const int64_t* sel2, const int32_t* arg,
                     const float* dmin, const uint8_t* keep, int32_t m, float thresh, const float* out,
                     const float* gneg, float* df, void* stream);
int gcl_loss_combine(const float* pos, const float* fin, int32_t n_sel, const float* neg, float w_pos, float w_fin,
                     float w_neg, float* out, void* stream);
int gcl_loss_seed(const float* g_total, float w_pos, float w_fin, float w_neg, int32_t n_sel, float* gpos, float* gfin,
                  float* gneg, void* stream);

int32_t gcl_sc2_chunks(void);
int32_t gcl_sc2_refine_partial_len(void);
int gcl_sc2_confidence(const float* src, const float* tgt, int32_t n, float d_thre, int32_t num_iterations,
                       float* partial, float* x, int32_t* done, void* stream);
int64_t gcl_sc2_confidence_scratch_bytes(int32_t n);
int gcl_sc2_confidence_sparse(const float* src, const float* tgt, int32_t n, float d_thre, int32_t num_iterations,
                              float* partial, float* x, int32_t* done, void* scratch, void* stream);
int64_t gcl_sc2_register_scratch_bytes(int32_t n);
int gcl_sc2_register(const float* src, const float* tgt, int32_t n, float d_thre, int32_t num_iterations, float nms_radius,
                     int32_t n_seeds, int32_t k1, int32_t k2, float inlier_thresh, float refine_thr, int32_t refine_iters,
                     void* scratch, float* conf, int64_t* seeds, int32_t* knn, float* seed_trans, float* fitness,
                     int32_t* best, float* trans16, float* labels, void* stream);
int64_t gcl_sc2_register_batch_scratch_bytes(int32_t batch, int32_t n_cap);
int gcl_sc2_register_batch(const float* src, const float* tgt, int32_t batch, int32_t n_cap, const int32_t* counts,
                           const int32_t* n_seeds, float d_thre, int32_t num_iterations, float nms_radius, int32_t k1,
                           int32_t k2, float inlier_thresh, float refine_thr, int32_t refine_iters, void* scratch, float* conf,
                           int64_t* seeds, int32_t* knn, float* seed_trans, float* fitness, int32_t* best, float* trans16,
                           float* labels, void* stream);
int gcl_sc2_local_max(const float* src, const float* conf, int32_t n, float radius, int32_t* is_max, void* stream);
int gcl_sc2_seed_knn(const float* src, const float* tgt, int32_t n, const int64_t* seeds, int32_t n_seeds,
                     float d_thre, int32_t k1, uint64_t* bits, int32_t* knn, void* stream);
int gcl_sc2_seed_trans(const float* src, const float* tgt, int32_t n, const int32_t* knn, int32_t n_seeds, int32_t k1,
                       int32_t k2, float d_thre, int32_t num_iterations, float inlier_thresh, float* trans,
                       float* fitness, void* stream);
int gcl_sc2_refine(const float* src, const float* tgt, int32_t n, float thr, int32_t iterations, double* partial,
                   int32_t* state, float* T, void* stream);

int64_t gcl_ransac_scratch_bytes(int32_t n, int32_t chunk);
int32_t gcl_ransac_default_chunk(void);
int gcl_ransac_register(const float* src, const float* tgt, int32_t n, int32_t ransac_n, float edge_similarity,
                        float check_distance, float max_corr_distance, int32_t max_iteration, float confidence,
                        uint64_t seed, int32_t chunk, void* scratch, float* trans16, int32_t* info, float* fit,
                        float* labels, int32_t* hyp_status, void* stream);
int64_t gcl_ransac_batch_scratch_bytes(int32_t batch, int32_t n_cap, int32_t chunk);
int gcl_ransac_register_batch(const float* src, const float* tgt, int32_t batch, int32_t n_cap, const int32_t* n_dev,
                              int32_t ransac_n, float edge_similarity, float check_distance, float max_corr_distance,
                              int32_t max_iteration, float confidence, const uint64_t* seeds, int32_t chunk, void* scratch,
                              float* trans16, int32_t* info, float* fit, float* labels, int32_t* hyp_status, void* stream);

int gcl_registration_stats(const float* src_corr, const float* tgt_corr, int32_t batch, int32_t n_cap, const int32_t* counts,
                           const float* pred_trans, const float* gt_trans, float inlier_threshold, float re_thre,
                           float te_thre, double* stats, float* pred_labels, float* gt_labels, void* stream);

#define GCL_MAX_LEVELS 8
#define GCL_MAX_MAPS 16
#define GCL_ERR_ARENA (-4)
#define GCL_MAPS_PINNED_BYTES (512 * (GCL_MAX_MAPS + 1))

typedef struct gcl_map_spec {
  int32_t t_in, kernel_size, stride, tables, pairs;
} gcl_map_spec;

typedef struct gcl_map_desc {
  int32_t t_in, kernel_size, stride, K;
  int32_t level_in, level_out;
  int64_t n_in, n_out, n_pairs;
  int32_t *nbr, *nbr_t, *counts;
  int32_t *tbl_n, *order_n, *mask_n;
  int32_t *tbl_t, *order_t, *mask_t;
  int32_t *pair_in, *pair_out;
  uint32_t* presence;
  int32_t* dw_bounds;
  int64_t seg_off[128];
  int32_t counts_host[128];
} gcl_map_desc;

typedef struct gcl_maps_desc {
  int32_t n_levels, n_maps;
  int64_t n_rows[GCL_MAX_LEVELS];
  int32_t* coords[GCL_MAX_LEVELS];
  int64_t* table[GCL_MAX_LEVELS];
  int64_t cap[GCL_MAX_LEVELS];
  int32_t status[4];
  int64_t arena_used;
  void* ready_event;
  int32_t late_mask;
  int32_t reserved;
  gcl_map_desc maps[GCL_MAX_MAPS];
} gcl_maps_desc;

int64_t gcl_maps_arena_bytes(int64_t n, const gcl_map_spec* specs_host, int32_t n_specs, int32_t n_levels);
int gcl_maps_build(const int32_t* coords, int64_t n, const gcl_map_spec* specs_host, int32_t n_specs, int32_t n_levels,
                   void* arena, int64_t arena_bytes, void* pinned_host, gcl_maps_desc* out_host, void* stream);
int gcl_maps_build_split(const int32_t* coords, int64_t n, const gcl_map_spec* specs_host, int32_t n_specs, int32_t n_levels,
                         void* arena, int64_t arena_bytes, void* pinned_host, gcl_maps_desc* out_host, void* stream,
                         void* side_stream);

#define GCL_OP_CONVBN 1
#define GCL_OP_CONV 2
#define GCL_OP_RELU 3
#define GCL_OP_CAT 4
#define GCL_OP_ROWNORM 5
typedef struct gcl_plan_op {
  int32_t kind;
  int32_t x, x2, y;
  int32_t level_in, level_out, cin, cout;
  int32_t map, transpose, K;
  int32_t w, bias;
  int32_t bn_w, bn_b, bn;
  int32_t relu;
  float momentum, eps;
} gcl_plan_op;

void* gcl_plan_create(const gcl_plan_op* ops_host, int32_t n_ops, int32_t n_tensors, int32_t n_params,
                      const int32_t* weight_order_host, int32_t n_weights, int32_t presplit_min_c);
void gcl_plan_destroy(void* plan);
int64_t gcl_plan_state_bytes(const void* plan);
int64_t gcl_plan_arena_bytes(void* plan, const gcl_maps_desc* maps_host);
int gcl_plan_forward(void* plan, const gcl_maps_desc* maps_host, const float* x, void* const* params_host,
                     void* const* bn_stats_host, void* state, void* arena, int64_t arena_bytes, float** y_out_host,
                     void* stream);
int64_t gcl_plan_eval_state_bytes(const void* plan);
int64_t gcl_plan_eval_arena_bytes(void* plan, const gcl_maps_desc* maps_host);
int gcl_plan_forward_eval(void* plan, const gcl_maps_desc* maps_host, const float* x, void* const* params_host,
                          void* const* bn_eval_host, int32_t repack, void* state, void* arena, int64_t arena_bytes,
                          float** y_out_host, void* stream);
int gcl_plan_backward(void* plan, void* arena, const float* dy, void* const* grads_host, int32_t first_op,
                      int32_t last_op, void* stream);
int gcl_plan_release(void* plan, void* arena);
int gcl_plan_set_aux_stream(void* plan, void* stream);
int gcl_plan_touched_suffix(const void* plan);
int gcl_plan_set_touched_rows(void* plan, const int32_t* rows, int64_t cap);
int64_t gcl_plan_suffix_rows_used(const void* plan);
int64_t gcl_plan_suffix_fwd_rows_used(const void* plan);
int64_t gcl_touched_rows_scratch_len(int64_t n_rows);
int gcl_touched_rows(const int64_t* index, int64_t n_index, const int64_t* goff, int64_t n_groups, const int64_t* sel,
                     int32_t n_sel, const int64_t* rows_a, int32_t n_a, const int64_t* rows_b, int32_t n_b, int64_t n_rows,
                     int32_t* scratch, int32_t* rows, int64_t cap, int32_t* n_touched, void* stream);
int gcl_gather_rows(const float* src, int32_t ld, int64_t n_src, const int32_t* rows, int64_t cap, int32_t c, float pad,
                    float* out, void* stream);
int gcl_scatter_rows(const float* src, const int32_t* rows, int64_t cap, int32_t c, int64_t n_dst, float* dst, int32_t ld,
                     void* stream);
int gcl_scatter_add_rows(const float* src, int32_t src_ld, const int32_t* rows, int64_t cap, int32_t c, int64_t n_dst,
                         float* dst, int32_t ld, void* stream);
int gcl_row_slots(const int32_t* rows, int64_t cap, int64_t n, int32_t* slots, void* stream);
int gcl_stream_create_cu_share(int32_t percent, int32_t low_priority, void** stream_out);
int gcl_stream_destroy(void* stream);
int gcl_plan_profile(void* plan, int32_t enable);
int gcl_plan_profile_read(void* plan, double* records_host, int32_t max_records);

int gcl_col_sum(const float* x, int64_t n, int32_t c, double* scratch, float* out, void* stream);

int gcl_pair_key_table(const int64_t* pos_pairs, int64_t n_pos, int64_t seed, int64_t* table, int64_t cap, void* stream);
int gcl_pair_key_mask(const int64_t* ap, int32_t col, const int64_t* b, const int32_t* b_arg, int64_t nb, int32_t m,
                      int64_t seed, const int64_t* table, int64_t cap, int64_t* b_out, uint8_t* keep, void* stream);
#define GCL_TRIPLET_OUT 20
int64_t gcl_triplet_scratch_len(int32_t m);
int gcl_triplet_fwd(const float* f0, int64_t n0, const float* f1, int64_t n1, int32_t c, const int64_t* ap,
                    const int64_t* neg, const uint8_t* tag, const uint8_t* keep, int32_t m, float margin, float* work,
                    float* out, void* stream);
int gcl_triplet_bwd(const float* f0, int64_t n0, const float* f1, int64_t n1, int32_t c, const int64_t* ap,
                    const int64_t* neg, const uint8_t* tag, const uint8_t* keep, int32_t m, const float* work,
                    const float* out, const float* g, float* df0, float* df1, void* stream);
#define GCL_PAIR_SQ 0
#define GCL_PAIR_SQ_POS 1
#define GCL_PAIR_NEG 2
#define GCL_PAIR_DIST 3
int64_t gcl_pair_terms_scratch_len(int32_t m);
int gcl_pair_terms_fwd(const float* f0, int64_t n0, const float* f1, int64_t n1, int32_t c, const int64_t* pairs,
                       const uint8_t* keep, int32_t m, int32_t mode, float thresh, float eps, float* work, float* out,
                       void* stream);
int gcl_pair_terms_bwd(const float* f0, int64_t n0, const float* f1, int64_t n1, int32_t c, const int64_t* pairs,
                       const uint8_t* keep, int32_t m, int32_t mode, float thresh, float eps, const float* work,
                       const float* out, const float* g, float* df0, float* df1, void* stream);

#define GCL_FPFH_MAX_NN 128
#define GCL_FPFH_MAX_CLOUDS 32767
#define GCL_FPFH_BINS 33
int gcl_fpfh_cell_keys(const float* xyz, int64_t n, const int64_t* offsets, int32_t n_clouds, float radius, int64_t* keys,
                       void* stream);
int gcl_fpfh_neighbours(const float* xyz, int64_t n, const int64_t* offsets, int32_t n_clouds, const int64_t* sorted_keys,
                        const int64_t* order, float radius, int32_t max_nn, int32_t* idx, int32_t* cnt, void* stream);
int gcl_fpfh_normals(const float* xyz, int64_t n, const int32_t* idx, const int32_t* cnt, int32_t max_nn,
                     const float* viewpoint, const int64_t* offsets, int32_t n_clouds, float* normals, void* stream);
int gcl_fpfh_spfh(const float* xyz, const float* normals, int64_t n, const int32_t* idx, const int32_t* cnt, int32_t max_nn,
                  float* spfh, void* stream);
int gcl_fpfh_combine(const float* xyz, const float* spfh, int64_t n, const int32_t* idx, const int32_t* cnt, int32_t max_nn,
                     int32_t normalize, float* fpfh, void* stream);

int64_t gcl_irls_pose_scratch_len(int64_t total);
int gcl_irls_pose_batch(const float* src, const float* tgt, int64_t total, const int64_t* offsets, int32_t B,
                        const float* weight, int32_t n_iter, double par0, int32_t halve_every, double* scratch, double* T,
                        int32_t* status, void* stream);
int gcl_val_stats_batch(const float* src, const float* tgt, int64_t total, const int64_t* offsets, const float* xyz0,
                        int64_t total0, const int64_t* offsets0, int32_t B, const double* T_est, const double* T_gt,
                        const int32_t* status, double max_dist, double thresh, double* out, void* stream);

int64_t gcl_icp_scratch_bytes(int64_t total0, int64_t total1, int32_t n_pairs);
int gcl_icp_register_batch(const float* xyz0, const int64_t* offsets0_host, const int64_t* offsets0, const float* xyz1,
                           const int64_t* offsets1_host, const int64_t* offsets1, int32_t n_pairs,
                           const int64_t* sorted_keys, const int64_t* order, double max_correspondence_distance,
                           const double* init, int32_t max_iteration, double relative_fitness, double relative_rmse,
                           void* scratch, double* T, double* stats, int32_t* status, int32_t* corr, void* stream);

#ifdef __cplusplus
}
#endif
#endif
```

Measured before the change: 47.42 million active voxels/s.

## Skip fp32 twin of BN outputs whose only readers consume plane images

Adds a plan-time reader analysis that marks BatchNorm forward outputs and backward input-gradients whose consumers only read the split plane image, and skips allocating and storing the fp32 copy for them. The BN apply kernels now accept a null fp32 destination when a plane image is written instead. This removes a full-tensor write and its arena footprint for many layers. It adds guard checks that fail if any path later needs the missing fp32 tensor, plus a keep_fp32 switch to disable it.

```diff
diff --git a/gcl_amd/MinkowskiEngine/native.py b/gcl_amd/MinkowskiEngine/native.py
--- a/gcl_amd/MinkowskiEngine/native.py
+++ b/gcl_amd/MinkowskiEngine/native.py
@@ -429,6 +429,16 @@
         n, s = len(self.records), _lib.load().gcl_plan_touched_suffix(self.handle)
         return all(last <= s or (first <= s and last == n) for first, last, _ in self._segments())
 
+    def set_keep_fp32(self, keep):
+        _lib.check(_lib.load().gcl_plan_set_keep_fp32(self.handle, int(bool(keep))), "gcl_plan_set_keep_fp32")
+
+    def plane_only(self):
+        n = len(self.records)
+        flags = (ctypes.c_int32 * n)()
+        if _lib.load().gcl_plan_plane_only(self.handle, flags, n) < 0:
+            raise RuntimeError("gcl_plan_plane_only: " + _lib.load().gcl_last_error().decode())
+        return [i for i in range(n) if flags[i] & 1], [i for i in range(n) if flags[i] & 2]
+
     def output_rows(self, maps):
         return int(maps.desc.n_rows[self.records[-1]["level_out"]])
 
diff --git a/gcl_amd/_lib.py b/gcl_amd/_lib.py
--- a/gcl_amd/_lib.py
+++ b/gcl_amd/_lib.py
@@ -160,6 +160,8 @@
     "gcl_plan_backward": (_i32, [_vp, _vp, _vp, _vp, _i32, _i32, _vp]),
     "gcl_plan_release": (_i32, [_vp, _vp]),
     "gcl_plan_set_aux_stream": (_i32, [_vp, _vp]),
+    "gcl_plan_set_keep_fp32": (_i32, [_vp, _i32]),
+    "gcl_plan_plane_only": (_i32, [_vp, _vp, _i32]),
     "gcl_plan_touched_suffix": (_i32, [_vp]),
     "gcl_plan_set_touched_rows": (_i32, [_vp, _vp, _i64]),
     "gcl_plan_suffix_rows_used": (_i64, [_vp]),
diff --git a/gcl_amd/csrc/norm.hip b/gcl_amd/csrc/norm.hip
--- a/gcl_amd/csrc/norm.hip
+++ b/gcl_amd/csrc/norm.hip
@@ -419,8 +419,8 @@
     }
     const float4 oa = bn_fwd_one(xa, ra, residual != nullptr, relu, ka);
     const float4 ob = bn_fwd_one(xb, rb, residual != nullptr, relu, kb);
-    if (oka) { BN_Y(e, row_e) = oa; am = amax4(am, oa); }
-    if (okb) { BN_Y(f, row_e + rstep) = ob; am = amax4(am, ob); }
+    if (oka) { if (y) BN_Y(e, row_e) = oa; am = amax4(am, oa); }
+    if (okb) { if (y) BN_Y(f, row_e + rstep) = ob; am = amax4(am, ob); }
     if (planes) {
       const long long pld = yld4 * 4;
       if (oka) store_planes4(planes, HOIST ? row_e : e / cq_n, pld, HOIST ? q0 * 4 : (int)(e % cq_n) * 4, oa, pscale);
@@ -518,13 +518,13 @@
       relu_gate(gb, yb);
     }
     const float4 oa = bn_bwd_one(xa, ga, inv_n, ka);
-    reinterpret_cast<float4*>(dx)[e] = oa;
+    if (dx) reinterpret_cast<float4*>(dx)[e] = oa;
     am = amax4(am, oa);
     if (planes) store_planes4(planes, e / cq_n, c, (int)(e % cq_n) * 4, oa, pscale);
     BN_DRES(e, sa, ga)
     if (okb) {
       const float4 ob = bn_bwd_one(xb, gb, inv_n, kb);
-      reinterpret_cast<float4*>(dx)[f] = ob;
+      if (dx) reinterpret_cast<float4*>(dx)[f] = ob;
       am = amax4(am, ob);
       if (planes) store_planes4(planes, f / cq_n, c, (int)(f % cq_n) * 4, ob, pscale);
       BN_DRES(f, sb, gb)
@@ -676,7 +676,8 @@
 int gcl_bn_apply_planes(const float* x, int64_t n, int32_t c, const float* mean, const float* rstd, const float* weight,
                         const float* bias, const float* residual, int32_t relu, float* y, int32_t y_ld, uint64_t* relu_mask,
                         int32_t* y_amax, void* planes, void* stream) {
-  GCL_CHECK_ARG(x && mean && rstd && weight && bias && y, "gcl_bn_apply: null pointer");
+  GCL_CHECK_ARG(x && mean && rstd && weight && bias, "gcl_bn_apply: null pointer");
+  GCL_CHECK_ARG(y || planes, "gcl_bn_apply_planes: y may be NULL only when a plane image is written in its place");
   GCL_CHECK_ARG(n > 0 && c >= 4 && c % 4 == 0, "gcl_bn_apply: unsupported shape");
   GCL_CHECK_ARG(y_ld == 0 || (y_ld >= c && y_ld % 4 == 0), "gcl_bn_apply_ld: y_ld must be 0 or a multiple of 4 >= c");
   GCL_CHECK_ARG(!planes || (y_amax && c % 32 == 0 && (y_ld % 32) == 0),
@@ -750,7 +751,8 @@
                             const float* sum_gx, int32_t relu, float* dx, float* dres, int32_t* dx_amax, void* planes,
                             void* stream) {
   GCL_CHECK_ARG(dy_ld == 0 || (dy_ld >= c && dy_ld % 4 == 0), "gcl_bn_bwd_apply: dy_ld must be 0 or a multiple of 4 >= c");
-  GCL_CHECK_ARG(x && dy && mean && rstd && weight && sum_g && sum_gx && dx, "gcl_bn_bwd_apply: null pointer");
+  GCL_CHECK_ARG(x && dy && mean && rstd && weight && sum_g && sum_gx, "gcl_bn_bwd_apply: null pointer");
+  GCL_CHECK_ARG(dx || planes, "gcl_bn_bwd_apply_planes: dx may be NULL only when a plane image is written in its place");
   GCL_CHECK_ARG(!relu || y || relu_mask, "gcl_bn_bwd_apply: y or relu_mask is required when relu is set");
   GCL_CHECK_ARG(n > 0 && c >= 4 && c % 4 == 0, "gcl_bn_bwd_apply: unsupported shape");
   GCL_CHECK_ARG(!planes || (dx_amax && c % 32 == 0),
diff --git a/gcl_amd/csrc/plan.hip b/gcl_amd/csrc/plan.hip
--- a/gcl_amd/csrc/plan.hip
+++ b/gcl_amd/csrc/plan.hip
@@ -459,7 +459,12 @@
   int32_t* amax = nullptr;
   void* planes = nullptr;
   int ld = 0;
+  bool plane_only = false;
 };
+
+#define NEED_F32(ts, rec, what)                                                                                          \
+  GCL_CHECK_ARG(!(ts).plane_only, "gcl_plan: record %d reads %s in fp32, but the plan keeps that tensor as a plane image " \
+                                  "only (reader analysis of gcl_plan_create)", (int)(rec), what)
 
 struct OpSaved {
   float* conv_out = nullptr;
@@ -496,6 +501,7 @@
   void* key = nullptr;
   const int32_t* fwd_rows = nullptr;
   long long fwd_cap = 0;
+  bool keep_twins = false;
 };
 
 struct Plan : PassState {
@@ -512,6 +518,8 @@
   std::vector<char> fuse_relu;
   std::vector<int> cat_left;
   std::vector<int> mask_from;
+  std::vector<char> po_fwd, po_bwd;
+  bool keep_fp32 = false;
   std::vector<long long> host_tables, uploaded;
   bool eval = false;
   void* const* bn_eval = nullptr;
@@ -541,17 +549,19 @@
   return P.slot_pool + (P.next_slot++) * GCL_AMAX_WORDS;
 }
 
-static int ensure_amax(Plan& P, TState& ts, long long numel, hipStream_t st) {
+static int ensure_amax(Plan& P, TState& ts, long long numel, hipStream_t st, int rec) {
   Arena& A = P.A;
   if (ts.amax) return GCL_OK;
+  NEED_F32(ts, rec, "a tensor whose max-abs slot is missing");
   ts.amax = new_slot(P);
   PLAN_CALL(gcl_amax(ts.ptr, numel, ts.amax, 1, (void*)st));
   return GCL_OK;
 }
 
-static int ensure_planes(Plan& P, TState& ts, long long n, int c, hipStream_t st) {
+static int ensure_planes(Plan& P, TState& ts, long long n, int c, hipStream_t st, int rec) {
   Arena& A = P.A;
   if (ts.planes) return GCL_OK;
+  NEED_F32(ts, rec, "a tensor whose plane image is missing");
   ts.planes = A.take(n * c * 4);
   PLAN_CALL(gcl_split_planes(ts.ptr, n, c, ts.amax, ts.planes, (void*)st));
   return GCL_OK;
@@ -639,6 +649,7 @@
   *relu_amax_out = nullptr;
   const float* W = (const float*)P.params[op.w];
   if (is_stem(op, m)) {
+    NEED_F32(x, i, "its input (first layer)");
     int rcs = stem_flag(P, op, m, x, n_in, st);
     if (rcs) return rcs;
     PLAN_CALL(gcl_stem_fwd(x.ptr, W, m.nbr, n_out, op.K, op.cin, op.cout, y, m.presence, m.presence ? P.not_ones : nullptr,
@@ -650,11 +661,12 @@
     GCL_CHECK_HIP(hipStreamWaitEvent(st, P.fwd_packs, 0));
     P.fwd_packs_pending = false;
   }
-  int rc = ensure_amax(P, x, n_in * op.cin, st);
+  int rc = ensure_amax(P, x, n_in * op.cin, st, i);
   if (rc) return rc;
   P.saved[i].x_amax = x.amax;
   const bool pl = op.cin >= P.presplit;
-  if (pl && (rc = ensure_planes(P, x, n_in, op.cin, st))) return rc;
+  if (pl && (rc = ensure_planes(P, x, n_in, op.cin, st, i))) return rc;
+  if (!pl) NEED_F32(x, i, "its input");
   float* stats = nullptr;
   if (op.kind == GCL_OP_CONVBN) stats = A.take_n<float>(cdiv(n_out, 128) * 4 * op.cout);
   *stats_out = stats;
@@ -778,6 +790,7 @@
     const long long n_out = compact ? P.fwd_cap : M.n_rows[op.level_out];
     if (compact && (int)i == P.suffix_first) {
       TState& xs = P.t[op.x];
+      NEED_F32(xs, i, "the input of the touched-row suffix");
       float* cx = A.take_n<float>(P.fwd_cap * op.cin);
       PLAN_CALL(gcl_gather_rows(xs.ptr, xs.ld ? xs.ld : op.cin, M.n_rows[op.level_in], P.fwd_rows, P.fwd_cap, op.cin, 0.f, cx,
                                 (void*)st));
@@ -800,6 +813,8 @@
           TState& x = P.t[op.x];
           const int c = op.cout;
           const float* res = op.x2 >= 0 ? P.t[op.x2].ptr : nullptr;
+          NEED_F32(x, i, "its input (inference)");
+          if (op.x2 >= 0) NEED_F32(P.t[op.x2], i, "its residual operand");
           y.ptr = A.take_n<float>(n_out * c);
           y.amax = new_slot(P);
           void* const* be = P.bn_eval ? P.bn_eval + 4 * op.bn : nullptr;
@@ -814,7 +829,7 @@
             break;
           }
           const int wi = P.widx[op.w];
-          if ((rc = ensure_amax(P, x, n_in * op.cin, st))) return rc;
+          if ((rc = ensure_amax(P, x, n_in * op.cin, st, (int)i))) return rc;
           const SortedTable T = sorted_table(m, op.transpose);
           GCL_CHECK_ARG(A.dry || m.kernel_size == 1 || T.tbl,
                         "gcl_plan_forward_eval: record %d needs a sorted table the maps do not carry", (int)i);
@@ -865,12 +880,14 @@
           y.amax = cty.amax;
           y.planes = nullptr;
         } else {
-          y.ptr = A.take_n<float>(n_out * c);
+          y.plane_only = bound && !P.keep_twins && P.po_fwd[i];
+          y.ptr = y.plane_only ? nullptr : A.take_n<float>(n_out * c);
           y.ld = 0;
           y.amax = bound ? bound_slot : new_slot(P);
           if (bound) y.planes = A.take(n_out * c * 4);
         }
         if (op.relu) sv.mask = A.take_n<unsigned long long>(gcl_bn_mask_len(n_out, c));
+        if (op.x2 >= 0) NEED_F32(P.t[op.x2], i, "its residual operand");
         const float* res = op.x2 >= 0 ? P.t[op.x2].ptr : nullptr;
         void* img = !bound ? nullptr : (P.cat_left[i] >= 0 ? P.t[P.ops[P.cat_left[i]].y].planes : y.planes);
         PLAN_CALL(gcl_bn_apply_planes(cy, n_out, c, sv.mean, sv.rstd, (const float*)P.params[op.bn_w],
@@ -895,6 +912,7 @@
           break;
         }
         const long long n4 = n_out * op.cout / 4;
+        NEED_F32(P.t[op.x], i, "its input");
         y.ptr = A.take_n<float>(n_out * op.cout);
         y.amax = new_slot(P);
         if (!A.dry) {
@@ -906,6 +924,8 @@
       }
       case GCL_OP_CAT: {
         const int ca = op.cin, cb = op.cout - op.cin;
+        NEED_F32(P.t[op.x], i, "its left input");
+        NEED_F32(P.t[op.x2], i, "its right input");
         if (P.t[op.x].ld == op.cout && P.t[op.x].ptr == y.ptr && y.ptr) {
           if (!A.dry) {
             hipLaunchKernelGGL(k_cat_right, dim3(grid_for(n_out * cb / 4)), dim3(256), 0, st, (const float4*)P.t[op.x2].ptr,
@@ -927,6 +947,7 @@
         break;
       }
       case GCL_OP_ROWNORM: {
+        NEED_F32(P.t[op.x], i, "its input");
         y.ptr = A.take_n<float>(n_out * op.cout);
         P.saved[i].norm = A.take_n<float>(n_out);
         PLAN_CALL(gcl_row_normalize_fwd(P.t[op.x].ptr, n_out, op.cout, y.ptr, P.saved[i].norm, (void*)st));
@@ -938,6 +959,7 @@
     }
   }
   if (late_pending) GCL_CHECK_HIP(hipStreamWaitEvent(st, (hipEvent_t)M.ready_event, 0));
+  NEED_F32(P.t[P.ops.back().y], P.ops.size() - 1, "its output (the caller's)");
   *y_out = P.t[P.ops.back().y].ptr;
   if (P.fwd_cap > 0) {
     const gcl_plan_op& last = P.ops.back();
@@ -1041,7 +1063,8 @@
   *out = rows;
   return GCL_OK;
 }
-static int saved_rows(Plan& P, RowView& V, const TState& t, int c, hipStream_t st, const float** out) {
+static int saved_rows(Plan& P, RowView& V, const TState& t, int c, hipStream_t st, const float** out, int rec) {
+  if (V.cap > 0 && !V.parked) NEED_F32(t, rec, "a saved operand it gathers onto a row list");
   return saved_rows(P, V, t.ptr, t.ld ? t.ld : c, c, 0.f, st, out);
 }
 
@@ -1063,6 +1086,8 @@
   float* dW = (float*)grads[op.w];
   int rc;
   if (is_stem(op, m)) {
+    NEED_F32(x, i, "its input (first layer)");
+    NEED_F32(dy, i, "its output gradient (first layer)");
     float* scratch = A.take_n<float>(gcl_stem_bwd_weight_scratch_len(op.K, op.cin, op.cout, n_out));
     hipStream_t ws = fork_aux(P, st);
     ProfScope ps(P, ws, 2, (double)m.n_pairs, op.cin, op.cout, n_in, n_out, op.K);
@@ -1071,19 +1096,24 @@
     return GCL_OK;
   }
   const int wi = P.widx[op.w];
-  if ((rc = ensure_amax(P, dy, n_out * op.cout, st))) return rc;
+  if ((rc = ensure_amax(P, dy, n_out * op.cout, st, i))) return rc;
   const int32_t* w_amax = P.w_amax + (long long)wi * GCL_AMAX_WORDS;
   const double pairs = (double)(m.kernel_size > 1 ? m.n_pairs : n_out);
   const long long rows_len = m.kernel_size == 1 ? gcl_conv_bwd_weight_rows_scratch_len(op.cin, op.cout, 4, n_in) : 0;
   const bool pl_w = rows_len <= 0 && op.cin >= P.presplit && op.cout >= P.presplit;
   const bool pl_x = op.cout >= P.presplit;
-  if ((pl_w || (pl_x && P.made[op.x])) && (rc = ensure_planes(P, dy, n_out, op.cout, st))) return rc;
+  if ((pl_w || (pl_x && P.made[op.x])) && (rc = ensure_planes(P, dy, n_out, op.cout, st, i))) return rc;
   if (pl_w) {
     x.amax = P.saved[i].x_amax;
-    if ((rc = ensure_planes(P, x, n_in, op.cin, st))) return rc;
-  }
+    if ((rc = ensure_planes(P, x, n_in, op.cin, st, i))) return rc;
+  }
+  if (!pl_w) NEED_F32(x, i, "its input (weight gradient)");
+  if (!pl_w) NEED_F32(dy, i, "its output gradient (weight gradient)");
+  if (!pl_x && P.made[op.x]) NEED_F32(dy, i, "its output gradient (input gradient)");
+  if (P.made[op.x] && !P.g[op.x].ptr && P.mask_from[i] >= 0) NEED_F32(x, i, "its input (ReLU mask of the input-gradient epilogue)");
+  if (op.bias >= 0) NEED_F32(dy, i, "its output gradient (bias gradient)");
   const float* xr;
-  if ((rc = saved_rows(P, V, x, op.cin, st, &xr))) return rc;
+  if ((rc = saved_rows(P, V, x, op.cin, st, &xr, i))) return rc;
   hipStream_t ws = fork_aux(P, st);
   if (P.made[op.x]) {
     const int mode = (m.kernel_size > 1 && !op.transpose && m.stride == 1) ? 2 : 1;
@@ -1172,7 +1202,10 @@
       double* scratch = A.take_n<double>(gcl_bn_scratch_len(n_out, c));
       const bool bound = sv.xrange && c >= P.presplit && !is_stem(op, M.maps[op.map]);
       TState d;
-      d.ptr = A.take_n<float>(n_out * c);
+      d.plane_only = bound && !P.keep_twins && P.po_bwd[i];
+      GCL_CHECK_ARG(!(d.plane_only && rv), "gcl_plan_backward: record %d: a compact gradient reached a BatchNorm whose input "
+                                           "gradient the plan keeps as a plane image only", i);
+      d.ptr = d.plane_only ? nullptr : A.take_n<float>(n_out * c);
       d.amax = new_slot(P);
       if (rv) {
         if ((rc = row_slots(P, *rv, st))) return rc;
@@ -1208,7 +1241,8 @@
       }
       if ((rc = contiguous(P, g, n_out, op.cout, st))) return rc;
       const float* y;
-      if ((rc = saved_rows(P, V, P.t[op.y], op.cout, st, &y))) return rc;
+      NEED_F32(P.t[op.y], i, "its saved output");
+      if ((rc = saved_rows(P, V, P.t[op.y], op.cout, st, &y, i))) return rc;
       const long long numel = n_out * op.cout;
       float* gx = A.take_n<float>(numel);
       int32_t* slot = new_slot(P);
@@ -1229,7 +1263,8 @@
     case GCL_OP_ROWNORM: {
       if ((rc = contiguous(P, g, n_out, op.cout, st))) return rc;
       const float *y, *norm;
-      if ((rc = saved_rows(P, V, P.t[op.y], op.cout, st, &y))) return rc;
+      NEED_F32(P.t[op.y], i, "its saved output");
+      if ((rc = saved_rows(P, V, P.t[op.y], op.cout, st, &y, i))) return rc;
       if ((rc = saved_rows(P, V, P.saved[i].norm, 1, 1, 1.f, st, &norm))) return rc;
       float* dx = A.take_n<float>(n_in * op.cin);
       int32_t* slot = new_slot(P);
@@ -1347,6 +1382,45 @@
   return join_aux(P, st);
 }
 
+static void plane_only_analysis(Plan& P) {
+  const int n_ops = (int)P.ops.size();
+  P.po_fwd.assign(n_ops, 0);
+  P.po_bwd.assign(n_ops, 0);
+  auto stem_shape = [](const gcl_plan_op& o) { return o.cin <= 4 && (o.cout % 32) == 0 && !o.transpose && o.K > 1 && o.bias < 0; };
+  auto conv = [](const gcl_plan_op& o) { return o.kind == GCL_OP_CONVBN || o.kind == GCL_OP_CONV; };
+  std::vector<int> maker(P.n_tensors, -1);
+  for (int i = 0; i < n_ops; ++i) maker[P.ops[i].y] = i;
+  std::vector<char> may_rv(P.n_tensors, 0);
+  if (P.suffix_first < n_ops) may_rv[P.ops[P.suffix_first].x] = 1;
+  for (int i = n_ops - 1; i >= 0; --i) {
+    const gcl_plan_op& o = P.ops[i];
+    if (!may_rv[o.y]) continue;
+    if (o.kind == GCL_OP_CAT) may_rv[o.x] = may_rv[o.x2] = 1;
+    if (o.kind == GCL_OP_CONVBN && o.x2 >= 0) may_rv[o.x2] = 1;
+  }
+  for (int i = 0; i < n_ops && i < P.suffix_first; ++i) {
+    const gcl_plan_op& o = P.ops[i];
+    bool bound = o.kind == GCL_OP_CONVBN && !stem_shape(o) && o.cout >= P.presplit && (o.cout % 32) == 0;
+    if (bound && o.x2 >= 0) {
+      const int k = maker[o.x2] >= 0 ? P.ops[maker[o.x2]].kind : 0;
+      bound = k == GCL_OP_CONVBN || k == GCL_OP_RELU || k == GCL_OP_CAT;
+    }
+    if (!bound) continue;
+    P.po_bwd[i] = o.K > 1 && o.cin >= P.presplit && o.bias < 0 && !may_rv[o.y];
+    bool ok = P.cat_left[i] < 0 && o.y != P.ops.back().y;
+    int readers = 0;
+    for (int j = 0; j < n_ops && ok; ++j) {
+      const gcl_plan_op& r = P.ops[j];
+      if (r.x2 == o.y) ok = false;
+      if (r.x != o.y) continue;
+      ++readers;
+      ok = ok && j < P.suffix_first && conv(r) && !stem_shape(r) && r.K > 1 && r.cin >= P.presplit && r.cout >= P.presplit &&
+           P.mask_from[j] < 0;
+    }
+    P.po_fwd[i] = ok && readers > 0;
+  }
+}
+
 static int check_maps(const Plan& P, const gcl_maps_desc* M) {
   GCL_CHECK_ARG(M && M->n_levels >= 1 && M->n_levels <= GCL_MAX_LEVELS && M->n_maps >= 0 && M->n_maps <= GCL_MAX_MAPS,
                 "gcl_plan: bad maps descriptor");
@@ -1571,6 +1645,7 @@
       ++P->n_bwd;
     }
   }
+  plane_only_analysis(*P);
   return P;
 }
 
@@ -1596,6 +1671,7 @@
   if (!P || check_maps(*P, maps_host) != GCL_OK) return -1;
   P->maps = maps_host;
   P->params.assign(P->n_params, nullptr);
+  P->keep_twins = P->keep_fp32;
   long long need = 0;
   const int rc = dry_pass(*P, nullptr, nullptr, true, &need);
   P->forward_done = false;
@@ -1615,6 +1691,7 @@
   P->state = state;
   P->A = Arena{(char*)arena, arena_bytes, 0, false};
   P->forward_done = false;
+  P->keep_twins = P->keep_fp32;
   long long need = 0;
   if ((rc = dry_pass(*P, x, bn_stats_host, true, &need))) return rc;
   if (need > arena_bytes) {
@@ -1774,6 +1851,24 @@
   GCL_CHECK_ARG(P, "gcl_plan_set_aux_stream: null plan");
   P->aux = (hipStream_t)stream;
   return GCL_OK;
+}
+
+int gcl_plan_set_keep_fp32(void* plan, int32_t keep) {
+  Plan* P = (Plan*)plan;
+  GCL_CHECK_ARG(P, "gcl_plan_set_keep_fp32: null plan");
+  P->keep_fp32 = keep != 0;
+  return GCL_OK;
+}
+
+int gcl_plan_plane_only(const void* plan, int32_t* flags_host, int32_t n_ops) {
+  const Plan* P = (const Plan*)plan;
+  GCL_CHECK_ARG(P && flags_host && n_ops == (int32_t)P->ops.size(), "gcl_plan_plane_only: flags_host must hold one word per record");
+  int n = 0;
+  for (int i = 0; i < n_ops; ++i) {
+    flags_host[i] = P->keep_fp32 ? 0 : (P->po_fwd[i] ? 1 : 0) | (P->po_bwd[i] ? 2 : 0);
+    n += (flags_host[i] & 1) + (flags_host[i] >> 1);
+  }
+  return n;
 }
 
 int gcl_plan_touched_suffix(const void* plan) {
diff --git a/include/gcl_amd.h b/include/gcl_amd.h
--- a/include/gcl_amd.h
+++ b/include/gcl_amd.h
@@ -447,6 +447,8 @@
                       int32_t last_op, void* stream);
 int gcl_plan_release(void* plan, void* arena);
 int gcl_plan_set_aux_stream(void* plan, void* stream);
+int gcl_plan_set_keep_fp32(void* plan, int32_t keep);
+int gcl_plan_plane_only(const void* plan, int32_t* flags_host, int32_t n_ops);
 int gcl_plan_touched_suffix(const void* plan);
 int gcl_plan_set_touched_rows(void* plan, const int32_t* rows, int64_t cap);
 int64_t gcl_plan_suffix_rows_used(const void* plan);
```

Measured after the change: 47.96 million active voxels/s (median of 6 runs). 1.01x the previous value.
